# Electron-Labs/eth-lc-plonky2

Measured on AMD Instinct MI355X. Metric: lc_proofs_per_hour, higher is better.
Workload: dtype u64

## Files before the change

### eth-lc-plonky2_amd/binding.py

```python
import ctypes
import os

import numpy as np

from . import build as _build

u64p = ctypes.POINTER(ctypes.c_uint64)
u32p = ctypes.POINTER(ctypes.c_uint32)
u8p = ctypes.POINTER(ctypes.c_uint8)
MEM_HOST, MEM_DEVICE = 0, 1
VERIFY_HEADS = {"host": 0, "device": 1}
E_UNSAT = -5
SECTION_OPENINGS, SECTION_FRI_CAP0, SECTION_AFTER_CAPS = 0, 1, 2

K_INTT, K_LDE, K_LEAF_HASH, K_MERKLE, K_PERM_Z, K_QUOTIENT, K_OPENINGS, K_FRI, K_POW, K_SHA256, K_OTHER = range(11)
KERNEL_FAMILIES = ["intt", "lde", "leaf_hash", "merkle", "perm_z", "quotient", "openings", "fri", "pow", "sha256", "other"]

GOLDILOCKS_P = 0xFFFFFFFF00000001


class Lcp2Error(RuntimeError):
    def __init__(self, status, message):
        super().__init__(f"lcp2 status {status}: {message}")
        self.status = status


class Params(ctypes.Structure):
    _fields_ = [(n, ctypes.c_uint32) for n in (
        "degree_bits", "num_wires", "num_routed_wires", "num_constants", "rate_bits", "cap_height",
        "num_challenges", "quotient_degree_factor", "proof_of_work_bits", "num_query_rounds", "num_fri_layers")]
    _fields_.append(("fri_arity_bits", ctypes.c_uint32 * 8))


class CircuitDesc(ctypes.Structure):
    _fields_ = [("params", Params), ("constants_sigmas", ctypes.c_void_p), ("constants_sigmas_mem", ctypes.c_int),
                ("k_is", ctypes.c_void_p), ("num_selectors", ctypes.c_uint32), ("num_gates", ctypes.c_uint32),
                ("gates", ctypes.c_void_p), ("code", ctypes.c_void_p), ("code_words", ctypes.c_size_t),
                ("imm", ctypes.c_void_p), ("num_imm", ctypes.c_size_t), ("num_public_inputs", ctypes.c_uint32),
                ("num_regs", ctypes.c_uint32)]


class CircuitRows(ctypes.Structure):
    _fields_ = [("gate_of_row", ctypes.c_void_p), ("num_rows", ctypes.c_size_t), ("pad_gate", ctypes.c_uint32), ("row_constants", ctypes.c_void_p),
                ("bindings", ctypes.c_void_p), ("num_bindings", ctypes.c_size_t), ("bindings_mem", ctypes.c_int), ("num_classes", ctypes.c_uint32)]


BINDING_DTYPE = np.dtype([("row", "<u4"), ("col", "<u4"), ("cls", "<u4")])
assert BINDING_DTYPE.itemsize == 12


class ProofLayout(ctypes.Structure):
    _fields_ = ([(n, ctypes.c_uint64) for n in ("cap_words", "wires_cap", "zs_cap", "quot_cap", "op_constants", "op_sigmas", "op_wires", "op_zs",
                                                "op_zs_next", "op_partial_products", "op_quotient", "fri_caps", "queries", "query_words")]
                + [("q_init_off", ctypes.c_uint64 * 4), ("q_init_cols", ctypes.c_uint64 * 4), ("q_init_sib", ctypes.c_uint64),
                   ("q_step_off", ctypes.c_uint64 * 8), ("q_step_sib", ctypes.c_uint64 * 8)]
                + [(n, ctypes.c_uint64) for n in ("final_poly", "final_len", "pow_witness", "total")])


class U32Job(ctypes.Structure):
    _fields_ = [("row", ctypes.c_uint32), ("kind", ctypes.c_uint16), ("op", ctypes.c_uint16), ("inputs", ctypes.c_uint32 * 4)]


U32_ARITHMETIC, U32_ADD_MANY, U32_SUBTRACTION, U32_RANGE_CHECK, U32_COMPARISON = range(5)
U32_JOB_DTYPE = np.dtype([("row", "<u4"), ("kind", "<u2"), ("op", "<u2"), ("in", "<u4", (4,))])
assert U32_JOB_DTYPE.itemsize == ctypes.sizeof(U32Job) == 24
POSEIDON_ROW_DTYPE = np.dtype([("row", "<u4"), ("swap", "<u4"), ("in", "<u8", (12,))])
assert POSEIDON_ROW_DTYPE.itemsize == 104
SHA_JOB_DTYPE = np.dtype([("first_row", "<u4"), ("in_src", "<i4", (16,))])
CELL_DTYPE = np.dtype([("row", "<u4"), ("col", "<u4"), ("value", "<u8")])
CELL_REF_DTYPE = np.dtype([("row", "<u4"), ("col", "<u4")])
assert SHA_JOB_DTYPE.itemsize == 68 and CELL_DTYPE.itemsize == 16 and CELL_REF_DTYPE.itemsize == 8
SHA_ROWS, SHA_ROW_COLUMNS = 310, 108

class RecOperand(ctypes.Structure):
    _fields_ = [("v", ctypes.c_uint64), ("col", ctypes.c_uint32), ("src", ctypes.c_uint32)]


class RecJob(ctypes.Structure):
    _fields_ = [("row", ctypes.c_uint32), ("kind", ctypes.c_uint16), ("op", ctypes.c_uint16), ("first_operand", ctypes.c_uint32),
                ("reserved", ctypes.c_uint32)]


(REC_ARITHMETIC, REC_BASE_SUM, REC_ARITHMETIC_EXT, REC_MUL_EXT, REC_REDUCING, REC_REDUCING_EXT, REC_POSEIDON_MDS, REC_RANDOM_ACCESS,
 REC_EXPONENTIATION, REC_COSET_INTERPOLATION, REC_KINDS) = range(11)
REC_IMM, REC_CELL = 0, 1
REC_OPERAND_DTYPE = np.dtype([("v", "<u8"), ("col", "<u4"), ("src", "<u4")])
REC_JOB_DTYPE = np.dtype([("row", "<u4"), ("kind", "<u2"), ("op", "<u2"), ("first_operand", "<u4"), ("reserved", "<u4")])
assert REC_OPERAND_DTYPE.itemsize == ctypes.sizeof(RecOperand) == 16 and REC_JOB_DTYPE.itemsize == ctypes.sizeof(RecJob) == 16
PLAN_IMM, PLAN_CELL, PLAN_PREV = 0, 1, 2
POS_JOB_DTYPE = np.dtype([("row", "<u4"), ("first_operand", "<u4")])
assert POS_JOB_DTYPE.itemsize == 8


class WitnessPlan(ctypes.Structure):
    _fields_ = [("rec_jobs", ctypes.c_void_p), ("nrec", ctypes.c_size_t), ("rec_level_ends", ctypes.c_void_p),
                ("pos_jobs", ctypes.c_void_p), ("npos", ctypes.c_size_t), ("chain_ends", ctypes.c_void_p), ("nchains", ctypes.c_size_t),
                ("pos_level_ends", ctypes.c_void_p), ("operands", ctypes.c_void_p), ("noperands", ctypes.c_size_t), ("nlevels", ctypes.c_size_t)]


class U32PlanJob(ctypes.Structure):
    _fields_ = [("row", ctypes.c_uint32), ("kind", ctypes.c_uint16), ("op", ctypes.c_uint16), ("first_operand", ctypes.c_uint32),
                ("reserved", ctypes.c_uint32)]


U32_PLAN_JOB_DTYPE = REC_JOB_DTYPE
U32_PLAN_OPERANDS = {U32_ARITHMETIC: 3, U32_ADD_MANY: 4, U32_SUBTRACTION: 3, U32_RANGE_CHECK: 1, U32_COMPARISON: 2}
assert ctypes.sizeof(U32PlanJob) == U32_PLAN_JOB_DTYPE.itemsize == 16


class WitnessPlanU32(ctypes.Structure):
    _fields_ = [("base", WitnessPlan), ("u32_jobs", ctypes.c_void_p), ("nu32", ctypes.c_size_t), ("u32_level_ends", ctypes.c_void_p)]


_lib = None


class WitnessReport(ctypes.Structure):
    _fields_ = [("gate_violations", ctypes.c_uint64), ("gate_row", ctypes.c_uint64), ("gate_index", ctypes.c_uint32), ("gate_constraint", ctypes.c_uint32),
                ("copy_violations", ctypes.c_uint64), ("copy_row", ctypes.c_uint64), ("copy_wire", ctypes.c_uint32),
                ("copy_to_row", ctypes.c_uint64), ("copy_to_wire", ctypes.c_uint32), ("noncanonical_cells", ctypes.c_uint64)]
    per_gate = None

    @property
    def ok(self):
        return self.gate_violations == 0 and self.copy_violations == 0

    def __repr__(self):
        return "WitnessReport(%s)" % ", ".join("%s=%d" % (f, getattr(self, f)) for f, _ in self._fields_)


class FillReport(ctypes.Structure):
    _fields_ = [(f, ctypes.c_uint64) for f in ("num_classes", "classes_set", "cells_filled", "conflicts", "conflict_index", "owner_index")]
    unsat = False
    message = ""

    def __repr__(self):
        return "FillReport(%s, unsat=%s)" % (", ".join("%s=%d" % (f, getattr(self, f)) for f, _ in self._fields_), self.unsat)


class ChallengerState(ctypes.Structure):
    _fields_ = [("sponge", ctypes.c_uint64 * 12), ("input", ctypes.c_uint64 * 8), ("output", ctypes.c_uint64 * 8),
                ("input_len", ctypes.c_uint32), ("output_len", ctypes.c_uint32)]


def _share_torch_hip_runtime():
    import importlib.util
    spec = importlib.util.find_spec("torch")
    if spec is None or not spec.submodule_search_locations:
        return
    libdir = os.path.join(list(spec.submodule_search_locations)[0], "lib")
    for name in ("libhsa-runtime64.so", "libamdhip64.so"):
        cand = os.path.join(libdir, name)
        if os.path.exists(cand):
            try:
                ctypes.CDLL(cand, mode=ctypes.RTLD_GLOBAL)
            except OSError:
                return


def load_library():
    global _lib
    if _lib is not None:
        return _lib
    path = _build.LIB
    if not os.path.exists(path):
        path = _build.build_native()
    _share_torch_hip_runtime()
    lib = ctypes.CDLL(path)
    c = ctypes
    sigs = {
        "lcp2_status_str": (c.c_char_p, [c.c_int]),
        "lcp2_abi_version": (c.c_int, []),
        "lcp2_device_count": (c.c_int, []),
        "lcp2_params_standard": (c.c_int, [c.c_uint32, c.c_uint32, c.POINTER(Params)]),
        "lcp2_params_config": (c.c_int, [c.c_uint32] * 8 + [c.POINTER(Params)]),
        "lcp2_ctx_create": (c.c_int, [c.c_int, c.c_void_p, c.POINTER(c.c_void_p)]),
        "lcp2_ctx_create_ex": (c.c_int, [c.c_int, c.c_void_p, c.c_uint32, c.POINTER(c.c_void_p)]),
        "lcp2_ctx_destroy": (None, [c.c_void_p]),
        "lcp2_ctx_sync": (c.c_int, [c.c_void_p]),
        "lcp2_ctx_stream": (c.c_void_p, [c.c_void_p]),
        "lcp2_last_error": (c.c_char_p, [c.c_void_p]),
        "lcp2_poseidon_permute_batch": (c.c_int, [c.c_void_p, c.c_void_p, c.c_void_p, c.c_size_t, c.c_int]),
        "lcp2_field_op_batch": (c.c_int, [c.c_void_p, c.c_void_p, c.c_void_p, c.c_void_p, c.c_size_t, c.c_uint32, c.c_int]),
        "lcp2_merkle_cap": (c.c_int, [c.c_void_p, c.c_void_p, c.c_size_t, c.c_size_t, c.c_uint32, c.c_int, c.c_void_p]),
        "lcp2_ntt_batch": (c.c_int, [c.c_void_p, c.c_void_p, c.c_size_t, c.c_uint32, c.c_int, c.c_uint64, c.c_int]),
        "lcp2_lde_batch": (c.c_int, [c.c_void_p, c.c_void_p, c.c_void_p, c.c_size_t, c.c_uint32, c.c_uint32, c.c_int]),
        "lcp2_sha256_tree": (c.c_int, [c.c_void_p, c.c_void_p, c.c_uint32, c.c_size_t, c.c_void_p, c.c_void_p, c.c_int]),
        "lcp2_sha256_witness": (c.c_int, [c.c_void_p, c.c_void_p, c.c_size_t, c.c_void_p, c.c_uint32, c.c_void_p, c.c_size_t, c.c_void_p, c.c_uint64, c.c_void_p]),
        "lcp2_scatter_cells": (c.c_int, [c.c_void_p, c.c_void_p, c.c_size_t, c.c_void_p, c.c_uint64]),
        "lcp2_poseidon_gate_rows": (c.c_int, [c.c_void_p, c.c_void_p, c.c_size_t, c.c_void_p, c.c_uint64]),
        "lcp2_u32_gate_rows": (c.c_int, [c.c_void_p, c.c_void_p, c.c_size_t, c.c_int, c.c_void_p, c.c_uint64]),
        "lcp2_rec_gate_rows": (c.c_int, [c.c_void_p, c.c_void_p, c.c_size_t, c.c_void_p, c.c_size_t, c.c_void_p, c.c_size_t, c.c_int, c.c_void_p,
                                         c.c_uint32, c.c_uint64]),
        "lcp2_witness_plan_rows": (c.c_int, [c.c_void_p, c.POINTER(WitnessPlan), c.c_int, c.c_void_p, c.c_uint32, c.c_uint64]),
        "lcp2_witness_plan_rows_u32": (c.c_int, [c.c_void_p, c.POINTER(WitnessPlanU32), c.c_int, c.c_void_p, c.c_uint32, c.c_uint64]),
        "lcp2_commit_wires_rows_begin": (c.c_int, [c.c_void_p, c.c_void_p]),
        "lcp2_commit_wires_chunk": (c.c_int, [c.c_void_p, c.c_void_p, c.c_uint32, c.c_uint32]),
        "lcp2_commit_wires_rows_finish": (c.c_int, [c.c_void_p, c.c_void_p]),
        "lcp2_host_register": (c.c_int, [c.c_void_p, c.c_void_p, c.c_size_t]),
        "lcp2_host_unregister": (c.c_int, [c.c_void_p, c.c_void_p]),
        "lcp2_witness_stage": (c.c_int, [c.c_void_p, c.c_void_p, c.c_uint32]),
        "lcp2_prove_staged": (c.c_int, [c.c_void_p, c.c_uint32, c.c_void_p, c.c_size_t, c.c_void_p, c.c_size_t]),
        "lcp2_buffer_alloc": (c.c_int, [c.c_void_p, c.c_size_t, c.POINTER(c.c_void_p)]),
        "lcp2_buffer_free": (c.c_int, [c.c_void_p, c.c_void_p]),
        "lcp2_buffer_zero": (c.c_int, [c.c_void_p, c.c_void_p, c.c_size_t]),
        "lcp2_buffer_read": (c.c_int, [c.c_void_p, c.c_void_p, c.c_void_p, c.c_size_t]),
        "lcp2_buffer_write": (c.c_int, [c.c_void_p, c.c_void_p, c.c_void_p, c.c_size_t]),
        "lcp2_buffer_copy": (c.c_int, [c.c_void_p, c.c_void_p, c.c_void_p, c.c_size_t]),
        "lcp2_buffer_copy_2d": (c.c_int, [c.c_void_p, c.c_void_p, c.c_size_t, c.c_void_p, c.c_size_t, c.c_size_t, c.c_size_t]),
        "lcp2_commit_values": (c.c_int, [c.c_void_p, c.c_void_p, c.c_size_t, c.c_uint32, c.c_uint32, c.c_uint32, c.c_int, c.POINTER(c.c_void_p), c.c_void_p]),
        "lcp2_commit_coeffs": (c.c_int, [c.c_void_p, c.c_void_p, c.c_size_t, c.c_uint32, c.c_uint32, c.c_uint32, c.c_int, c.POINTER(c.c_void_p), c.c_void_p]),
        "lcp2_commit_cosets": (c.c_int, [c.c_void_p, c.c_void_p, c.c_size_t, c.c_uint32, c.c_uint32, c.c_uint32, c.c_uint32, c.c_uint32, c.c_int, c.POINTER(c.c_void_p), c.c_void_p]),
        "lcp2_oracle_destroy": (None, [c.c_void_p]),
        "lcp2_oracle_open": (c.c_int, [c.c_void_p, c.c_void_p, c.c_size_t, c.c_void_p, c.c_void_p]),
        "lcp2_oracle_read": (c.c_int, [c.c_void_p, c.c_void_p, c.c_void_p]),
        "lcp2_circuit_create": (c.c_int, [c.c_void_p, c.POINTER(CircuitDesc), c.POINTER(c.c_void_p)]),
        "lcp2_circuit_rows_expand": (c.c_int, [c.c_void_p, c.POINTER(CircuitDesc), c.POINTER(CircuitRows), c.c_void_p]),
        "lcp2_circuit_create_from_rows": (c.c_int, [c.c_void_p, c.POINTER(CircuitDesc), c.POINTER(CircuitRows), c.POINTER(c.c_void_p)]),
        "lcp2_verifier_create": (c.c_int, [c.POINTER(CircuitDesc), c.c_void_p, c.c_void_p, c.POINTER(c.c_void_p)]),
        "lcp2_circuit_destroy": (None, [c.c_void_p]),
        "lcp2_circuit_digest": (c.c_int, [c.c_void_p, c.c_void_p, c.c_void_p]),
        "lcp2_proof_words": (c.c_size_t, [c.POINTER(Params)]),
        "lcp2_proof_layout_of": (c.c_int, [c.POINTER(Params), c.POINTER(ProofLayout)]),
        "lcp2_prove": (c.c_int, [c.c_void_p, c.c_void_p, c.c_int, c.c_void_p, c.c_size_t, c.c_void_p, c.c_size_t]),
        "lcp2_witness_fill_copies": (c.c_int, [c.c_void_p, c.c_void_p, c.c_size_t, c.c_int, c.c_void_p, c.POINTER(FillReport)]),
        "lcp2_circuit_copy_classes": (c.c_int, [c.c_void_p, c.c_void_p, c.POINTER(c.c_uint64)]),
        "lcp2_witness_settle_copies": (c.c_int, [c.c_void_p, c.c_void_p, c.c_size_t, c.c_int, c.c_void_p, c.POINTER(FillReport)]),
        "lcp2_check_witness": (c.c_int, [c.c_void_p, c.c_void_p, c.c_int, c.c_void_p, c.c_size_t, c.POINTER(WitnessReport), c.c_void_p, c.c_uint32]),
        "lcp2_commit_wires": (c.c_int, [c.c_void_p, c.c_void_p, c.c_int, c.c_void_p]),
        "lcp2_commit_wires_coeffs": (c.c_int, [c.c_void_p, c.c_void_p, c.c_void_p, c.c_void_p]),
        "lcp2_commit_wires_rows": (c.c_int, [c.c_void_p, c.c_void_p, c.c_void_p, c.c_void_p]),
        "lcp2_perm_zs_rows_begin": (c.c_int, [c.c_void_p, c.c_void_p, c.c_void_p, c.c_void_p]),
        "lcp2_perm_zs_rows_finish": (c.c_int, [c.c_void_p, c.c_void_p, c.POINTER(c.c_void_p), c.POINTER(c.c_size_t)]),
        "lcp2_perm_zs_commit": (c.c_int, [c.c_void_p, c.c_void_p]),
        "lcp2_perm_zs": (c.c_int, [c.c_void_p, c.c_void_p, c.c_void_p, c.c_void_p]),
        "lcp2_quotient": (c.c_int, [c.c_void_p, c.c_void_p, c.c_void_p, c.c_void_p]),
        "lcp2_fri_open": (c.c_int, [c.c_void_p, c.c_void_p, c.POINTER(ChallengerState), c.c_void_p]),
        "lcp2_fri_open_begin": (c.c_int, [c.c_void_p, c.c_void_p, c.POINTER(ChallengerState), c.c_void_p]),
        "lcp2_fri_open_commit": (c.c_int, [c.c_void_p, c.c_void_p]),
        "lcp2_fri_open_finish": (c.c_int, [c.c_void_p, c.POINTER(ChallengerState), c.c_void_p]),
        "lcp2_proof_section": (c.c_int, [c.c_void_p, c.c_int, c.POINTER(c.c_size_t), c.POINTER(c.c_size_t)]),
        "lcp2_challenger_init": (None, [c.POINTER(ChallengerState)]),
        "lcp2_challenger_observe": (c.c_int, [c.POINTER(ChallengerState), c.c_void_p, c.c_size_t]),
        "lcp2_challenger_get": (c.c_int, [c.POINTER(ChallengerState), c.c_void_p, c.c_size_t]),
        "lcp2_hash_no_pad": (c.c_int, [c.c_void_p, c.c_size_t, c.c_void_p]),
        "lcp2_circuit_create_sharded": (c.c_int, [c.c_void_p, c.POINTER(CircuitDesc), c.c_uint32, c.c_uint32, c.POINTER(c.c_void_p)]),
        "lcp2_circuit_set_constants_cap": (c.c_int, [c.c_void_p, c.c_void_p]),
        "lcp2_quotient_values": (c.c_int, [c.c_void_p, c.c_void_p, c.c_void_p]),
        "lcp2_quotient_buffer": (c.c_int, [c.c_void_p, c.POINTER(c.c_void_p), c.POINTER(c.c_size_t)]),
        "lcp2_quotient_commit": (c.c_int, [c.c_void_p, c.c_void_p]),
        "lcp2_verify": (c.c_int, [c.c_void_p, c.c_void_p, c.c_size_t, c.c_void_p, c.c_size_t, c.POINTER(c.c_int)]),
        "lcp2_verify_batch": (c.c_int, [c.c_void_p, c.c_void_p, c.c_void_p, c.c_size_t, c.c_size_t, c.c_int, c.c_void_p, c.c_size_t, c.c_void_p]),
        "lcp2_verify_batch_ex": (c.c_int, [c.c_void_p, c.c_void_p, c.c_void_p, c.c_size_t, c.c_size_t, c.c_int, c.c_void_p, c.c_size_t, c.c_void_p,
                                           c.c_uint32]),
        "lcp2_last_challenges": (c.c_int, [c.c_void_p, c.c_void_p]),
        "lcp2_gate_program_degree": (c.c_int, [c.c_void_p, c.c_size_t, c.c_uint32, c.POINTER(c.c_uint32)]),
        "lcp2_circuit_gate_tiers": (c.c_int, [c.c_void_p, c.c_uint32, c.c_void_p, c.c_void_p]),
        "lcp2_proof_bytes": (c.c_size_t, [c.POINTER(Params), c.c_size_t, c.c_uint32]),
        "lcp2_proof_to_bytes": (c.c_int, [c.POINTER(Params), c.c_void_p, c.c_size_t, c.c_void_p, c.c_size_t, c.c_uint32, c.c_void_p, c.c_size_t]),
        "lcp2_proof_from_bytes": (c.c_int, [c.POINTER(Params), c.c_void_p, c.c_size_t, c.c_uint32, c.c_void_p, c.c_size_t, c.c_void_p, c.c_size_t]),
        "lcp2_verifier_data_to_bytes": (c.c_int, [c.c_void_p, c.c_void_p, c.c_size_t]),
        "lcp2_prof_enable": (c.c_int, [c.c_void_p, c.c_int]),
        "lcp2_prof_reset": (c.c_int, [c.c_void_p]),
        "lcp2_prof_get": (c.c_int, [c.c_void_p, c.c_int, c.POINTER(c.c_double), c.POINTER(c.c_uint64), c.POINTER(c.c_double)]),
    }
    for name, (res, args) in sigs.items():
        fn = getattr(lib, name)
        fn.restype = res
        fn.argtypes = args
    _lib = lib
    return lib


EXPORTED_SYMBOLS = None


def _np_u64(a):
    a = np.ascontiguousarray(a, dtype=np.uint64)
    return a


def _ptr(a):
    return a.ctypes.data_as(ctypes.c_void_p) if a is not None else None


def standard_params(degree_bits, num_constants=4):
    lib = load_library()
    p = Params()
    rc = lib.lcp2_params_standard(degree_bits, num_constants, ctypes.byref(p))
    if rc:
        raise Lcp2Error(rc, lib.lcp2_status_str(rc).decode())
    return p


def params_config(degree_bits, num_constants=4, rate_bits=3, cap_height=4, proof_of_work_bits=16, num_query_rounds=28,
                  arity_bits=4, final_poly_bits=5):
    lib = load_library()
    p = Params()
    rc = lib.lcp2_params_config(degree_bits, num_constants, rate_bits, cap_height, proof_of_work_bits, num_query_rounds,
                                arity_bits, final_poly_bits, ctypes.byref(p))
    if rc:
        raise Lcp2Error(rc, lib.lcp2_status_str(rc).decode())
    return p


class Oracle:

    def __init__(self, ctx, handle, ncols, log_n, rate_bits, cap_height, cap):
        self.ctx, self.handle = ctx, handle
        self.ncols, self.log_n, self.rate_bits, self.cap_height = ncols, log_n, rate_bits, cap_height
        self.cap = cap
        self.block_first, self.block_count = 0, 1 << rate_bits

    def open(self, indices):
        idx = _np_u64(indices)
        k = idx.size
        nsib = self.log_n + self.rate_bits - self.cap_height
        leaves = np.zeros((k, self.ncols), dtype=np.uint64)
        sib = np.zeros((k, max(nsib, 0), 4), dtype=np.uint64)
        self.ctx._check(self.ctx.lib.lcp2_oracle_open(self.handle, _ptr(idx), k, _ptr(leaves), _ptr(sib)))
        return leaves, sib

    def read(self, coeffs=True, lde=True):
        n = 1 << self.log_n
        c = np.zeros((self.ncols, n), dtype=np.uint64) if coeffs else None
        l = np.zeros((self.ncols, n * self.block_count), dtype=np.uint64) if lde else None
        self.ctx._check(self.ctx.lib.lcp2_oracle_read(self.handle, _ptr(c), _ptr(l)))
        return c, l

    def close(self):
        if self.handle:
            self.ctx.lib.lcp2_oracle_destroy(self.handle)
            self.handle = None

    def __del__(self):
        try:
            self.close()
        except Exception:
            pass


class Context:

    def __init__(self, device=0, stream=None, order_with_default_stream=False):
        self.lib = load_library()
        h = ctypes.c_void_p()
        rc = self.lib.lcp2_ctx_create_ex(device, stream, 1 if order_with_default_stream else 0, ctypes.byref(h))
        if rc:
            raise Lcp2Error(rc, self.lib.lcp2_status_str(rc).decode())
        self.handle = h

    def _check(self, rc):
        if rc:
            msg = self.lib.lcp2_status_str(rc).decode()
            detail = self.lib.lcp2_last_error(self.handle)
            raise Lcp2Error(rc, msg + (": " + detail.decode() if detail else ""))

    def close(self):
        if getattr(self, "handle", None):
            self.lib.lcp2_ctx_destroy(self.handle)
            self.handle = None

    def __del__(self):
        try:
            self.close()
        except Exception:
            pass

    def sync(self):
        self._check(self.lib.lcp2_ctx_sync(self.handle))

    def stream_ptr(self):
        return self.lib.lcp2_ctx_stream(self.handle) or 0

    def poseidon_permute_batch(self, states):
        s = _np_u64(states).reshape(-1, 12)
        out = np.empty_like(s)
        self._check(self.lib.lcp2_poseidon_permute_batch(self.handle, _ptr(s), _ptr(out), s.shape[0], MEM_HOST))
        return out

    FIELD_OPS = {"mul": 0, "pow7": 1, "add": 2, "sub": 3, "canon": 4, "add_lazy": 5, "sub_lazy": 6, "shl32_lazy": 24, "mul_u32": 25,
                 **{"shl%d" % (12 * k): 16 + k for k in range(1, 8)}}

    def field_op_batch(self, op, a, b=None):
        a = _np_u64(a).reshape(-1)
        out = np.empty_like(a)
        if b is not None:
            b = _np_u64(b).reshape(-1)
            assert a.shape == b.shape
        self._check(self.lib.lcp2_field_op_batch(self.handle, _ptr(a), _ptr(b) if b is not None else None, _ptr(out), a.shape[0],
                                                 self.FIELD_OPS[op], MEM_HOST))
        return out

    def merkle_cap(self, leaves, cap_height):
        l = _np_u64(leaves)
        assert l.ndim == 2
        cap = np.zeros((1 << cap_height, 4), dtype=np.uint64)
        self._check(self.lib.lcp2_merkle_cap(self.handle, _ptr(l), l.shape[0], l.shape[1], cap_height, MEM_HOST, _ptr(cap)))
        return cap

    def ntt_batch(self, cols, inverse=False, shift=1):
        c = _np_u64(cols).copy()
        assert c.ndim == 2
        log_n = int(c.shape[1]).bit_length() - 1
        assert 1 << log_n == c.shape[1]
        self._check(self.lib.lcp2_ntt_batch(self.handle, _ptr(c), c.shape[0], log_n, int(inverse), shift, MEM_HOST))
        return c

    def lde_batch(self, coeffs, rate_bits=3):
        c = _np_u64(coeffs)
        log_n = int(c.shape[1]).bit_length() - 1
        out = np.zeros((c.shape[0], c.shape[1] << rate_bits), dtype=np.uint64)
        self._check(self.lib.lcp2_lde_batch(self.handle, _ptr(c), _ptr(out), c.shape[0], log_n, rate_bits, MEM_HOST))
        return out

    def sha256_tree(self, leaves, height, trees=1, trace=False):
        l = np.ascontiguousarray(leaves, dtype=np.uint8).reshape(trees, 1 << height, 32)
        nodes = np.zeros((trees, (2 << height) - 1, 32), dtype=np.uint8)
        tr = np.zeros((trees, (1 << height) - 1, 2, 176), dtype=np.uint32) if trace else None
        self._check(self.lib.lcp2_sha256_tree(self.handle, _ptr(l), height, trees, _ptr(nodes), _ptr(tr), MEM_HOST))
        return (nodes, tr) if trace else nodes

    def _commit(self, fn, cols, rate_bits, cap_height, mem, shape):
        if mem == MEM_HOST:
            c = _np_u64(cols)
            ncols, n = c.shape
            p = _ptr(c)
        else:
            ncols, n = shape
            p = ctypes.c_void_p(cols)
        log_n = int(n).bit_length() - 1
        cap = np.zeros((1 << cap_height, 4), dtype=np.uint64)
        h = ctypes.c_void_p()
        self._check(fn(self.handle, p, ncols, log_n, rate_bits, cap_height, mem, ctypes.byref(h), _ptr(cap)))
        return Oracle(self, h, ncols, log_n, rate_bits, cap_height, cap)

    def commit_values(self, cols, rate_bits=3, cap_height=4, mem=MEM_HOST, shape=None):
        return self._commit(self.lib.lcp2_commit_values, cols, rate_bits, cap_height, mem, shape)

    def commit_coeffs(self, cols, rate_bits=3, cap_height=4, mem=MEM_HOST, shape=None):
        return self._commit(self.lib.lcp2_commit_coeffs, cols, rate_bits, cap_height, mem, shape)

    def commit_cosets(self, coeffs, block_first, block_count, rate_bits=3, cap_height=4, mem=MEM_HOST, shape=None):
        if mem == MEM_HOST:
            c = _np_u64(coeffs)
            ncols, n = c.shape
            p = _ptr(c)
        else:
            ncols, n = shape
            p = ctypes.c_void_p(coeffs)
        log_n = int(n).bit_length() - 1
        cap = np.zeros((block_count << (cap_height - rate_bits), 4), dtype=np.uint64)
        h = ctypes.c_void_p()
        self._check(self.lib.lcp2_commit_cosets(self.handle, p, ncols, log_n, rate_bits, cap_height, block_first, block_count, mem,
                                                ctypes.byref(h), _ptr(cap)))
        o = Oracle(self, h, ncols, log_n, rate_bits, cap_height, cap)
        o.block_first, o.block_count = block_first, block_count
        return o

    def buffer_zero(self, dev_ptr, words):
        self._check(self.lib.lcp2_buffer_zero(self.handle, ctypes.c_void_p(dev_ptr), int(words) * 8))

    def sha256_witness(self, jobs, level_start, words_in, wires_dev, n, digests=True):
        if not isinstance(jobs, np.ndarray) or jobs.dtype != SHA_JOB_DTYPE:
            raise Lcp2Error(-1, "jobs must be an array of SHA_JOB_DTYPE records")
        j = np.ascontiguousarray(jobs).ravel()
        levels = np.ascontiguousarray(level_start, dtype=np.uint32).ravel()
        words = np.ascontiguousarray(words_in, dtype=np.uint32).ravel()
        out = np.zeros((j.size, 8), dtype=np.uint32) if digests else None
        self._check(self.lib.lcp2_sha256_witness(self.handle, _ptr(j) if j.size else None, j.size, _ptr(levels) if levels.size else None,
                                                 max(levels.size, 1) - 1, _ptr(words) if words.size else None, words.size,
                                                 ctypes.c_void_p(wires_dev), int(n), _ptr(out) if digests and j.size else None))
        return out

    def scatter_cells(self, cells, wires_dev, n):
        if not isinstance(cells, np.ndarray) or cells.dtype != CELL_DTYPE:
            raise Lcp2Error(-1, "cells must be an array of CELL_DTYPE records")
        c = np.ascontiguousarray(cells).ravel()
        self._check(self.lib.lcp2_scatter_cells(self.handle, _ptr(c) if c.size else None, c.size, ctypes.c_void_p(wires_dev), int(n)))

    def poseidon_gate_rows(self, rows, wires_dev, n):
        if not isinstance(rows, np.ndarray) or rows.dtype != POSEIDON_ROW_DTYPE:
            raise Lcp2Error(-1, "rows must be an array of POSEIDON_ROW_DTYPE records")
        r = np.ascontiguousarray(rows).ravel()
        self._check(self.lib.lcp2_poseidon_gate_rows(self.handle, _ptr(r), r.size, ctypes.c_void_p(wires_dev), n))

    def u32_gate_rows(self, jobs, wires_dev, n, njobs=None):
        if isinstance(jobs, np.ndarray):
            if jobs.dtype != U32_JOB_DTYPE:
                raise Lcp2Error(-1, "jobs must be an array of U32_JOB_DTYPE records")
            j = np.ascontiguousarray(jobs).ravel()
            count, p, mem = j.size, _ptr(j), MEM_HOST
        else:
            if njobs is None:
                raise Lcp2Error(-1, "a device job list needs njobs")
            count, p, mem = int(njobs), ctypes.c_void_p(jobs), MEM_DEVICE
        self._check(self.lib.lcp2_u32_gate_rows(self.handle, p, count, mem, ctypes.c_void_p(wires_dev), n))

    def rec_gate_rows(self, jobs, operands, level_ends, wires_dev, ncols, n, njobs=None, noperands=None):
        ends = np.ascontiguousarray(level_ends, dtype=np.uint32).ravel()
        if isinstance(jobs, np.ndarray) != isinstance(operands, np.ndarray):
            raise Lcp2Error(-1, "jobs and operands must both be host arrays or both be device pointers")
        if isinstance(jobs, np.ndarray):
            if jobs.dtype != REC_JOB_DTYPE or operands.dtype != REC_OPERAND_DTYPE:
                raise Lcp2Error(-1, "jobs / operands must be arrays of REC_JOB_DTYPE / REC_OPERAND_DTYPE records")
            j, o = np.ascontiguousarray(jobs).ravel(), np.ascontiguousarray(operands).ravel()
            nj, no, pj, po, mem = j.size, o.size, _ptr(j), _ptr(o), MEM_HOST
        else:
            if njobs is None or noperands is None:
                raise Lcp2Error(-1, "device lists need njobs and noperands")
            nj, no, pj, po, mem = int(njobs), int(noperands), ctypes.c_void_p(jobs), ctypes.c_void_p(operands), MEM_DEVICE
        self._check(self.lib.lcp2_rec_gate_rows(self.handle, pj, nj, po, no, _ptr(ends) if ends.size else None, ends.size, mem,
                                                ctypes.c_void_p(wires_dev), int(ncols), int(n)))

    def witness_plan_rows(self, rec_jobs, pos_jobs, chain_ends, operands, rec_level_ends, pos_level_ends, wires_dev, ncols, n,
                          nrec=None, npos=None, nchains=None, noperands=None):
        rends = np.ascontiguousarray(rec_level_ends, dtype=np.uint32).ravel()
        pends = np.ascontiguousarray(pos_level_ends, dtype=np.uint32).ravel()
        if rends.size != pends.size:
            raise Lcp2Error(-1, "rec_level_ends and pos_level_ends must have one entry per level each")
        lists = (rec_jobs, pos_jobs, chain_ends, operands)
        on_host = [isinstance(a, np.ndarray) for a in lists]
        if any(on_host) != all(on_host):
            raise Lcp2Error(-1, "the four lists must all be host arrays or all be device pointers")
        if all(on_host):
            if (rec_jobs.dtype, pos_jobs.dtype, chain_ends.dtype, operands.dtype) != (REC_JOB_DTYPE, POS_JOB_DTYPE, np.dtype(np.uint32), REC_OPERAND_DTYPE):
                raise Lcp2Error(-1, "the lists must be arrays of REC_JOB_DTYPE / POS_JOB_DTYPE / uint32 / REC_OPERAND_DTYPE records")
            keep = [np.ascontiguousarray(a).ravel() for a in lists]
            counts, ptrs, mem = [a.size for a in keep], [a.ctypes.data if a.size else None for a in keep], MEM_HOST
        else:
            if None in (nrec, npos, nchains, noperands):
                raise Lcp2Error(-1, "device lists need nrec, npos, nchains and noperands")
            counts, ptrs, mem = [int(nrec), int(npos), int(nchains), int(noperands)], [a or None for a in lists], MEM_DEVICE
        plan = WitnessPlan(ptrs[0], counts[0], rends.ctypes.data if rends.size else None, ptrs[1], counts[1], ptrs[2], counts[2],
                           pends.ctypes.data if pends.size else None, ptrs[3], counts[3], rends.size)
        self._check(self.lib.lcp2_witness_plan_rows(self.handle, ctypes.byref(plan), mem, ctypes.c_void_p(wires_dev), int(ncols), int(n)))

    def witness_plan_rows_u32(self, u32_jobs, rec_jobs, pos_jobs, chain_ends, operands, u32_level_ends, rec_level_ends, pos_level_ends,
                              wires_dev, ncols, n, nu32=None, nrec=None, npos=None, nchains=None, noperands=None):
        ends = [np.ascontiguousarray(e, dtype=np.uint32).ravel() for e in (u32_level_ends, rec_level_ends, pos_level_ends)]
        if len({e.size for e in ends}) != 1:
            raise Lcp2Error(-1, "u32_level_ends, rec_level_ends and pos_level_ends must have one entry per level each")
        lists = (u32_jobs, rec_jobs, pos_jobs, chain_ends, operands)
        on_host = [isinstance(a, np.ndarray) for a in lists]
        if any(on_host) != all(on_host):
            raise Lcp2Error(-1, "the five lists must all be host arrays or all be device pointers")
        if all(on_host):
            if [a.dtype for a in lists] != [U32_PLAN_JOB_DTYPE, REC_JOB_DTYPE, POS_JOB_DTYPE, np.dtype(np.uint32), REC_OPERAND_DTYPE]:
                raise Lcp2Error(-1, "the lists must be arrays of U32_PLAN_JOB_DTYPE / REC_JOB_DTYPE / POS_JOB_DTYPE / uint32 / REC_OPERAND_DTYPE records")
            keep = [np.ascontiguousarray(a).ravel() for a in lists]
            counts, ptrs, mem = [a.size for a in keep], [a.ctypes.data if a.size else None for a in keep], MEM_HOST
        else:
            if None in (nu32, nrec, npos, nchains, noperands):
                raise Lcp2Error(-1, "device lists need nu32, nrec, npos, nchains and noperands")
            counts, ptrs, mem = [int(nu32), int(nrec), int(npos), int(nchains), int(noperands)], [a or None for a in lists], MEM_DEVICE
        end_ptrs = [e.ctypes.data if e.size else None for e in ends]
        base = WitnessPlan(ptrs[1], counts[1], end_ptrs[1], ptrs[2], counts[2], ptrs[3], counts[3], end_ptrs[2], ptrs[4], counts[4], ends[0].size)
        plan = WitnessPlanU32(base, ptrs[0], counts[0], end_ptrs[0])
        self._check(self.lib.lcp2_witness_plan_rows_u32(self.handle, ctypes.byref(plan), mem, ctypes.c_void_p(wires_dev), int(ncols), int(n)))

    def verify_batch(self, circuit_data, proofs, public_inputs, mem=MEM_HOST, count=None, head="host"):
        if head not in VERIFY_HEADS:
            raise Lcp2Error(-1, "head is 'host' or 'device'")
        words = circuit_data.proof_words
        if mem == MEM_HOST:
            pr = _np_u64(proofs)
            if pr.size % words:
                raise Lcp2Error(-1, "proofs is not a whole number of this circuit's proofs")
            count, ptr = pr.size // words, _ptr(pr)
        else:
            if count is None:
                raise Lcp2Error(-1, "device proofs need count")
            ptr = ctypes.c_void_p(proofs)
        if count == 0:
            return np.zeros(0, dtype=np.int32)
        pis = _np_u64(public_inputs).ravel()
        npi = pis.size // count
        if npi * count != pis.size:
            raise Lcp2Error(-1, "public_inputs is not count rows")
        checks = np.zeros(count, dtype=np.int32)
        if head == "host":
            rc = self.lib.lcp2_verify_batch(self.handle, circuit_data.handle, ptr, words, count, mem, _ptr(pis), npi, _ptr(checks))
        else:
            rc = self.lib.lcp2_verify_batch_ex(self.handle, circuit_data.handle, ptr, words, count, mem, _ptr(pis), npi, _ptr(checks), VERIFY_HEADS[head])
        if rc != -7:
            self._check(rc)
        return checks

    def expand_rows(self, circ, rows, bindings_ptr=None, num_bindings=None):
        d, keep = _describe(circ, 0)
        r, keep_rows = _describe_rows(rows, bindings_ptr, num_bindings)
        shape = (circ.params.num_constants + circ.params.num_routed_wires, 1 << circ.params.degree_bits)
        ptr = self.buffer_alloc(shape[0] * shape[1])
        try:
            self._check(self.lib.lcp2_circuit_rows_expand(self.handle, ctypes.byref(d), ctypes.byref(r), ctypes.c_void_p(ptr)))
            return self.buffer_read(ptr, shape[0] * shape[1]).reshape(shape)
        finally:
            self.buffer_free(ptr)

    def buffer_alloc(self, words):
        p = ctypes.c_void_p()
        self._check(self.lib.lcp2_buffer_alloc(self.handle, int(words) * 8, ctypes.byref(p)))
        return p.value

    def buffer_free(self, dev_ptr):
        self._check(self.lib.lcp2_buffer_free(self.handle, ctypes.c_void_p(dev_ptr)))

    def buffer_read(self, dev_ptr, words):
        out = np.zeros(words, dtype=np.uint64)
        self._check(self.lib.lcp2_buffer_read(self.handle, _ptr(out), ctypes.c_void_p(dev_ptr), words * 8))
        return out

    def buffer_write(self, dev_ptr, arr):
        a = _np_u64(arr)
        self._check(self.lib.lcp2_buffer_write(self.handle, ctypes.c_void_p(dev_ptr), _ptr(a), a.size * 8))

    def buffer_copy(self, dst_ptr, src_ptr, words):
        self._check(self.lib.lcp2_buffer_copy(self.handle, ctypes.c_void_p(dst_ptr), ctypes.c_void_p(src_ptr), words * 8))

    def buffer_copy_2d(self, dst_ptr, dst_pitch_words, src_ptr, src_pitch_words, width_words, height):
        self._check(self.lib.lcp2_buffer_copy_2d(self.handle, ctypes.c_void_p(dst_ptr), dst_pitch_words * 8, ctypes.c_void_p(src_ptr),
                                                 src_pitch_words * 8, width_words * 8, height))

    def prof_enable(self, on=True):
        self._check(self.lib.lcp2_prof_enable(self.handle, int(on)))

    def prof_reset(self):
        self._check(self.lib.lcp2_prof_reset(self.handle))

    def prof_get(self):
        out = {}
        for i, name in enumerate(KERNEL_FAMILIES):
            ms, n, b = ctypes.c_double(), ctypes.c_uint64(), ctypes.c_double()
            self._check(self.lib.lcp2_prof_get(self.handle, i, ctypes.byref(ms), ctypes.byref(n), ctypes.byref(b)))
            out[name] = {"ms": ms.value, "launches": n.value, "bytes": b.value}
        return out


class Challenger:

    def __init__(self):
        self.lib = load_library()
        self.state = ChallengerState()
        self.lib.lcp2_challenger_init(ctypes.byref(self.state))

    def observe(self, values):
        v = np.ascontiguousarray(np.asarray(values, dtype=np.uint64).ravel())
        rc = self.lib.lcp2_challenger_observe(ctypes.byref(self.state), _ptr(v), v.size)
        if rc:
            raise Lcp2Error(rc, self.lib.lcp2_status_str(rc).decode())

    def get(self, count=1):
        out = np.zeros(count, dtype=np.uint64)
        rc = self.lib.lcp2_challenger_get(ctypes.byref(self.state), _ptr(out), count)
        if rc:
            raise Lcp2Error(rc, self.lib.lcp2_status_str(rc).decode())
        return out


def hash_no_pad(values):
    lib = load_library()
    v = np.ascontiguousarray(np.asarray(values, dtype=np.uint64).ravel())
    out = np.zeros(4, dtype=np.uint64)
    rc = lib.lcp2_hash_no_pad(_ptr(v) if v.size else None, v.size, _ptr(out))
    if rc:
        raise Lcp2Error(rc, lib.lcp2_status_str(rc).decode())
    return out


SER_PUBLIC_INPUT_COUNT = 1


def proof_layout(params):
    lib, out = load_library(), ProofLayout()
    rc = lib.lcp2_proof_layout_of(ctypes.byref(params), ctypes.byref(out))
    if rc:
        raise Lcp2Error(rc, lib.lcp2_status_str(rc).decode())
    return out


def proof_to_bytes(params, proof, public_inputs, flags=SER_PUBLIC_INPUT_COUNT):
    lib = load_library()
    pr, pis = _np_u64(proof).ravel(), _np_u64(public_inputs).ravel()
    out = np.zeros(lib.lcp2_proof_bytes(ctypes.byref(params), pis.size, flags), dtype=np.uint8)
    rc = lib.lcp2_proof_to_bytes(ctypes.byref(params), _ptr(pr), pr.size, _ptr(pis), pis.size, flags, _ptr(out), out.size)
    if rc:
        raise Lcp2Error(rc, lib.lcp2_status_str(rc).decode())
    return out.tobytes()


def proof_from_bytes(params, data, num_public_inputs, flags=SER_PUBLIC_INPUT_COUNT):
    lib = load_library()
    buf = np.frombuffer(bytes(data), dtype=np.uint8)
    proof = np.zeros(lib.lcp2_proof_words(ctypes.byref(params)), dtype=np.uint64)
    pis = np.zeros(num_public_inputs, dtype=np.uint64)
    rc = lib.lcp2_proof_from_bytes(ctypes.byref(params), _ptr(buf) if buf.size else None, buf.size, flags, _ptr(proof), proof.size, _ptr(pis), pis.size)
    if rc:
        raise Lcp2Error(rc, lib.lcp2_status_str(rc).decode())
    return proof, pis


class ProofRejected(Lcp2Error):

    def __init__(self, check):
        super().__init__(-7, f"proof rejected (check {check})")
        self.check = check


def _describe(circ, constants_sigmas_ptr=None, mem=MEM_HOST):
    gs = circ.gateset
    gates = circ.gates_array
    d = CircuitDesc()
    d.params = circ.params
    d.constants_sigmas = constants_sigmas_ptr if constants_sigmas_ptr is not None else circ.constants_sigmas.ctypes.data
    d.constants_sigmas_mem = mem
    d.k_is = circ.k_is.ctypes.data
    d.num_selectors, d.num_gates = gs.num_selectors, len(gs.gates)
    d.gates = ctypes.cast(gates, ctypes.c_void_p)
    d.code, d.code_words = gs.code.ctypes.data, gs.code_len
    d.imm, d.num_imm = gs.imm.ctypes.data, gs.imm.size
    d.num_public_inputs, d.num_regs = circ.num_public_inputs, gs.max_regs
    return d, (gates, gs, circ)


def _describe_rows(rows, bindings_ptr=None, num_bindings=None):
    gate_of_row = np.ascontiguousarray(rows.gate_of_row, dtype=np.uint32).ravel()
    consts = None if rows.row_constants is None else np.ascontiguousarray(rows.row_constants, dtype=np.uint64)
    r = CircuitRows()
    r.gate_of_row, r.num_rows, r.pad_gate = (gate_of_row.ctypes.data if gate_of_row.size else None), gate_of_row.size, rows.pad_gate
    r.row_constants = consts.ctypes.data if consts is not None and consts.size else None
    r.num_classes = rows.num_classes
    if bindings_ptr is not None:
        r.bindings, r.num_bindings, r.bindings_mem, b = bindings_ptr, int(num_bindings), MEM_DEVICE, None
    else:
        if not isinstance(rows.bindings, np.ndarray) or rows.bindings.dtype != BINDING_DTYPE:
            raise Lcp2Error(-1, "bindings must be an array of BINDING_DTYPE records")
        b = np.ascontiguousarray(rows.bindings).ravel()
        r.bindings, r.num_bindings, r.bindings_mem = (b.ctypes.data if b.size else None), b.size, MEM_HOST
    return r, (gate_of_row, consts, b)


class CircuitData:

    def __init__(self, ctx, circ, handle, keep):
        self.ctx, self.circ, self.handle, self._keep = ctx, circ, handle, keep
        self.lib = load_library()
        self.proof_words = self.lib.lcp2_proof_words(ctypes.byref(circ.params))

    @classmethod
    def build(cls, ctx, circ, constants_sigmas_ptr=None, mem=MEM_HOST):
        d, keep = _describe(circ, constants_sigmas_ptr, mem)
        h = ctypes.c_void_p()
        ctx._check(ctx.lib.lcp2_circuit_create(ctx.handle, ctypes.byref(d), ctypes.byref(h)))
        return cls(ctx, circ, h, keep)

    @classmethod
    def build_from_rows(cls, ctx, circ, rows, bindings_ptr=None, num_bindings=None):
        d, keep = _describe(circ, 0)
        r, keep_rows = _describe_rows(rows, bindings_ptr, num_bindings)
        h = ctypes.c_void_p()
        ctx._check(ctx.lib.lcp2_circuit_create_from_rows(ctx.handle, ctypes.byref(d), ctypes.byref(r), ctypes.byref(h)))
        return cls(ctx, circ, h, keep)

    @classmethod
    def build_sharded(cls, ctx, circ, block_first, block_count, constants_sigmas_ptr=None, mem=MEM_HOST):
        d, keep = _describe(circ, constants_sigmas_ptr, mem)
        h = ctypes.c_void_p()
        ctx._check(ctx.lib.lcp2_circuit_create_sharded(ctx.handle, ctypes.byref(d), block_first, block_count, ctypes.byref(h)))
        return cls(ctx, circ, h, keep)

    def set_constants_cap(self, cap):
        cp = _np_u64(cap)
        self._check(self.lib.lcp2_circuit_set_constants_cap(self.handle, _ptr(cp)))

    def quotient_values(self, alphas, public_inputs_hash):
        a, h = _np_u64(alphas), _np_u64(public_inputs_hash)
        assert h.size == 4
        self._check(self.lib.lcp2_quotient_values(self.handle, _ptr(a), _ptr(h)))

    def quotient_buffer(self):
        ptr, words = ctypes.c_void_p(), ctypes.c_size_t()
        self._check(self.lib.lcp2_quotient_buffer(self.handle, ctypes.byref(ptr), ctypes.byref(words)))
        return ptr.value, words.value

    def quotient_commit(self):
        cap = self._cap()
        self._check(self.lib.lcp2_quotient_commit(self.handle, _ptr(cap)))
        return cap

    @classmethod
    def verifier_only(cls, circ, digest, cap):
        lib = load_library()
        d, keep = _describe(circ, 0)
        h = ctypes.c_void_p()
        dg, cp = _np_u64(digest), _np_u64(cap)
        rc = lib.lcp2_verifier_create(ctypes.byref(d), _ptr(dg), _ptr(cp), ctypes.byref(h))
        if rc:
            raise Lcp2Error(rc, lib.lcp2_status_str(rc).decode())
        return cls(None, circ, h, keep)

    def _check(self, rc):
        if rc:
            if self.ctx is not None:
                self.ctx._check(rc)
            raise Lcp2Error(rc, self.lib.lcp2_status_str(rc).decode())

    def digest(self):
        d = np.zeros(4, dtype=np.uint64)
        cap = np.zeros((1 << self.circ.params.cap_height, 4), dtype=np.uint64)
        self._check(self.lib.lcp2_circuit_digest(self.handle, _ptr(d), _ptr(cap)))
        return d, cap

    def prove(self, wires, public_inputs, mem=MEM_HOST):
        pis = _np_u64(public_inputs).ravel()
        proof = np.zeros(self.proof_words, dtype=np.uint64)
        if mem == MEM_HOST:
            w = _np_u64(wires)
            if w.shape != (self.circ.params.num_wires, 1 << self.circ.params.degree_bits):
                raise Lcp2Error(-1, "witness must be [num_wires][n]")
            wp = _ptr(w)
        else:
            wp = ctypes.c_void_p(wires)
        self._check(self.lib.lcp2_prove(self.handle, wp, mem, _ptr(pis), pis.size, _ptr(proof), proof.size))
        return proof

    def check_witness(self, wires, public_inputs, per_gate=False, mem=MEM_HOST):
        pis = _np_u64(public_inputs).ravel()
        if mem == MEM_HOST:
            w = _np_u64(wires)
            if w.shape != (self.circ.params.num_wires, 1 << self.circ.params.degree_bits):
                raise Lcp2Error(-1, "witness must be [num_wires][n]")
            wp = _ptr(w)
        else:
            wp = ctypes.c_void_p(wires)
        report = WitnessReport()
        ng = len(self.circ.gateset.gates)
        counts = np.zeros(ng, dtype=np.uint64) if per_gate else None
        self._check(self.lib.lcp2_check_witness(self.handle, wp, mem, _ptr(pis), pis.size, ctypes.byref(report), _ptr(counts), ng))
        report.per_gate = counts
        return report

    def fill_copies(self, cells, wires_ptr, mem=MEM_HOST, ncells=None):
        return self._copies_call(self.lib.lcp2_witness_fill_copies, cells, CELL_DTYPE, "cells must be an array of CELL_DTYPE records", wires_ptr, mem, ncells)

    def settle_copies(self, sources, wires_ptr, mem=MEM_HOST, nsources=None):
        return self._copies_call(self.lib.lcp2_witness_settle_copies, sources, CELL_REF_DTYPE, "sources must be an array of CELL_REF_DTYPE records", wires_ptr, mem,
                                 nsources)

    def _copies_call(self, call, records, dtype, dtype_message, wires_ptr, mem, count):
        if mem == MEM_HOST:
            if not isinstance(records, np.ndarray) or records.dtype != dtype:
                raise Lcp2Error(-1, dtype_message)
            c = np.ascontiguousarray(records).ravel()
            p, count = (_ptr(c) if c.size else None), c.size
        else:
            p, count = ctypes.c_void_p(records), int(count)
        report = FillReport()
        rc = call(self.handle, p, count, mem, ctypes.c_void_p(wires_ptr), ctypes.byref(report))
        if rc == E_UNSAT:
            report.unsat = True
            report.message = self.lib.lcp2_last_error(self.ctx.handle).decode()
        else:
            self._check(rc)
        return report

    def copy_classes(self):
        NR, n = self.circ.params.num_routed_wires, 1 << self.circ.params.degree_bits
        class_of, count = np.zeros((NR, n), dtype=np.uint32), ctypes.c_uint64()
        self._check(self.lib.lcp2_circuit_copy_classes(self.handle, _ptr(class_of), ctypes.byref(count)))
        return class_of, count.value

    def stage_witness(self, wires, slot):
        w = _np_u64(wires)
        if w.shape != (self.circ.params.num_wires, 1 << self.circ.params.degree_bits):
            raise Lcp2Error(-1, "witness must be [num_wires][n]")
        if not hasattr(self, "_staged"):
            self._staged = {}
        self._staged[slot] = w
        self._check(self.lib.lcp2_witness_stage(self.handle, _ptr(w), slot))

    def prove_staged(self, slot, public_inputs):
        pis = _np_u64(public_inputs).ravel()
        proof = np.zeros(self.proof_words, dtype=np.uint64)
        self._check(self.lib.lcp2_prove_staged(self.handle, slot, _ptr(pis), pis.size, _ptr(proof), proof.size))
        self._staged.pop(slot, None)
        return proof

    def host_witness_benchmark(self, wires, public_inputs, steps=4, reference_proof=None):
        import time
        ctx = self.ctx
        bufs = [np.ascontiguousarray(wires, dtype=np.uint64), np.array(wires, dtype=np.uint64, order="C")]
        for b in bufs:
            ctx._check(ctx.lib.lcp2_host_register(ctx.handle, _ptr(b), b.nbytes))
        try:
            ctx.sync()
            t0 = time.perf_counter()
            plain = self.prove(bufs[0], public_inputs, mem=MEM_HOST)
            t_plain = time.perf_counter() - t0
            self.stage_witness(bufs[0], 0)
            times = []
            for i in range(steps):
                t0 = time.perf_counter()
                if i + 1 < steps:
                    self.stage_witness(bufs[(i + 1) % 2], (i + 1) % 2)
                proof = self.prove_staged(i % 2, public_inputs)
                times.append(time.perf_counter() - t0)
            ok = bool((proof == plain).all()) and (reference_proof is None or bool((proof == reference_proof).all()))
        finally:
            ctx.sync()
            for b in bufs:
                ctx.lib.lcp2_host_unregister(ctx.handle, _ptr(b))
        steady = times[1:-1] if len(times) > 2 else times
        return {"workload": "lcp2_prove from HOST witnesses (%.2f GB each, pinned with lcp2_host_register): upload of witness i + 1 on the copy stream while "
                            "proof i runs (lcp2_witness_stage / lcp2_prove_staged)" % (bufs[0].nbytes / 1e9),
                "ms_per_proof_steady_state": 1e3 * min(steady), "ms_per_proof_all": [round(1e3 * t, 2) for t in times],
                "ms_plain_host_prove": 1e3 * t_plain, "proofs_equal_device_resident_proof": ok}

    def _cap(self):
        return np.zeros((1 << self.circ.params.cap_height, 4), dtype=np.uint64)

    def commit_wires(self, wires, mem=MEM_HOST):
        cap = self._cap()
        if mem == MEM_HOST:
            self._staged_wires = _np_u64(wires)
            wp = _ptr(self._staged_wires)
        else:
            wp = ctypes.c_void_p(wires)
        self._check(self.lib.lcp2_commit_wires(self.handle, wp, mem, _ptr(cap)))
        return cap

    def commit_wires_coeffs(self, wires_ptr, coeffs_ptr):
        cap = self._cap()
        self._check(self.lib.lcp2_commit_wires_coeffs(self.handle, ctypes.c_void_p(wires_ptr), ctypes.c_void_p(coeffs_ptr), _ptr(cap)))
        return cap

    def commit_wires_rows(self, rows_ptr, coeffs_ptr):
        cap = self._cap()
        self._check(self.lib.lcp2_commit_wires_rows(self.handle, ctypes.c_void_p(rows_ptr), ctypes.c_void_p(coeffs_ptr), _ptr(cap)))
        return cap

    def commit_wires_rows_begin(self, rows_ptr):
        self._check(self.lib.lcp2_commit_wires_rows_begin(self.handle, ctypes.c_void_p(rows_ptr)))

    def commit_wires_chunk(self, coeffs_ptr, first_col, ncols):
        self._check(self.lib.lcp2_commit_wires_chunk(self.handle, ctypes.c_void_p(coeffs_ptr), first_col, ncols))

    def commit_wires_rows_finish(self):
        cap = self._cap()
        self._check(self.lib.lcp2_commit_wires_rows_finish(self.handle, _ptr(cap)))
        return cap

    def perm_zs_rows_begin(self, betas, gammas, world):
        out, b, g = np.zeros(world * self.circ.params.num_challenges, dtype=np.uint64), _np_u64(betas), _np_u64(gammas)
        self._check(self.lib.lcp2_perm_zs_rows_begin(self.handle, _ptr(b), _ptr(g), _ptr(out)))
        return out

    def perm_zs_rows_finish(self, block_products):
        bp = _np_u64(block_products)
        ptr, words = ctypes.c_void_p(), ctypes.c_size_t()
        self._check(self.lib.lcp2_perm_zs_rows_finish(self.handle, _ptr(bp), ctypes.byref(ptr), ctypes.byref(words)))
        return ptr.value, words.value

    def perm_zs_commit(self):
        cap = self._cap()
        self._check(self.lib.lcp2_perm_zs_commit(self.handle, _ptr(cap)))
        return cap

    def perm_zs(self, betas, gammas):
        cap, b, g = self._cap(), _np_u64(betas), _np_u64(gammas)
        self._check(self.lib.lcp2_perm_zs(self.handle, _ptr(b), _ptr(g), _ptr(cap)))
        return cap

    def quotient(self, alphas, public_inputs_hash):
        cap, a, h = self._cap(), _np_u64(alphas), _np_u64(public_inputs_hash)
        assert h.size == 4
        self._check(self.lib.lcp2_quotient(self.handle, _ptr(a), _ptr(h), _ptr(cap)))
        return cap

    def fri_open(self, zeta, challenger_state, proof):
        z = _np_u64(zeta)
        assert proof.dtype == np.uint64 and proof.size == self.proof_words and proof.flags.c_contiguous
        self._check(self.lib.lcp2_fri_open(self.handle, _ptr(z), ctypes.byref(challenger_state), _ptr(proof)))

    def fri_open_begin(self, zeta, challenger_state, proof):
        z = _np_u64(zeta)
        assert proof.dtype == np.uint64 and proof.size == self.proof_words and proof.flags.c_contiguous
        self._check(self.lib.lcp2_fri_open_begin(self.handle, _ptr(z), ctypes.byref(challenger_state), _ptr(proof)))

    def fri_open_commit(self, proof):
        assert proof.dtype == np.uint64 and proof.size == self.proof_words and proof.flags.c_contiguous
        self._check(self.lib.lcp2_fri_open_commit(self.handle, _ptr(proof)))

    def fri_open_finish(self, proof, challenger_state=None):
        assert proof.dtype == np.uint64 and proof.size == self.proof_words and proof.flags.c_contiguous
        self._check(self.lib.lcp2_fri_open_finish(self.handle, ctypes.byref(challenger_state) if challenger_state is not None else None, _ptr(proof)))

    def proof_section(self, section):
        first, count = ctypes.c_size_t(0), ctypes.c_size_t(0)
        self._check(self.lib.lcp2_proof_section(self.handle, section, ctypes.byref(first), ctypes.byref(count)))
        return first.value, count.value

    def verify(self, proof, public_inputs):
        failed = ctypes.c_int(0)
        pr, pis = _np_u64(proof).ravel(), _np_u64(public_inputs).ravel()
        rc = self.lib.lcp2_verify(self.handle, _ptr(pr), pr.size, _ptr(pis), pis.size, ctypes.byref(failed))
        if rc == -7:
            raise ProofRejected(failed.value)
        self._check(rc)

    def verifier_data_bytes(self):
        out = np.zeros(((4 << self.circ.params.cap_height) + 4) * 8, dtype=np.uint8)
        self._check(self.lib.lcp2_verifier_data_to_bytes(self.handle, _ptr(out), out.size))
        return out.tobytes()

    def last_challenges(self):
        out = np.zeros(97, dtype=np.uint64)
        self._check(self.lib.lcp2_last_challenges(self.handle, _ptr(out)))
        return {"betas": out[0:4], "gammas": out[4:8], "alphas": out[8:12], "zeta": out[12:14], "fri_alpha": out[14:16],
                "fri_betas": out[16:32].reshape(8, 2), "pow_witness": int(out[32]), "query_indices": out[33:97]}

    def gate_tiers(self):
        ng = len(self.circ.gateset.gates)
        deg, bun = np.zeros(ng, dtype=np.uint32), np.zeros(ng, dtype=np.int32)
        self._check(self.lib.lcp2_circuit_gate_tiers(self.handle, ng, _ptr(deg), _ptr(bun)))
        return deg, bun

    def close(self):
        if self.handle:
            self.lib.lcp2_circuit_destroy(self.handle)
            self.handle = None

    def __del__(self):
        try:
            self.close()
        except Exception:
            pass
```

### eth-lc-plonky2_amd/csrc/kernels_gates.hpp

```cpp
#pragma once
#include <utility>
#include "quotient_common.hpp"

namespace lcp2 {

enum GeneratedMode : u32 { GEN_QUOTIENT = 0, GEN_ROW_CHECK = 1, GEN_CLAIM_CHECK = 2 };

#if defined(__HIP_DEVICE_COMPILE__)
template <u32 K> struct QGenerated {
  static __device__ __forceinline__ void run(const QuotientArgs &a, const GateDev &, u64 i, u64 *, u32, u32, QEmit &emit) { q_generated<K>(a, i, emit); }
};
#else
template <u32 K> struct QGenerated;
#endif

template <u32 K, bool CHECK>
__global__ __launch_bounds__(QUOTIENT_THREADS, Q_GENERATED_WAVES[K]) void k_q_gen(QuotientArgs a, u32 g, u32 accumulate, unsigned long long *flag) {
#if defined(__HIP_DEVICE_COMPILE__)
  extern __shared__ __attribute__((aligned(16))) u64 lds[];
  const u32 T = QUOTIENT_THREADS, tid = threadIdx.x;
  u64 i;
  const bool live = q_point<CHECK>(a, i);
  q_stage_limbs(a, lds, T, tid);
  if (!live) return;
  const GateDev G = q_load_gate(a, g);
  if (!q_wave_holds<CHECK>(a, G, i)) return;
  u64 val[QUOTIENT_MAX_CH];
  q_gate_value<QGenerated<K>>(a, g, G, i, lds, T, tid, val);
  q_gate_store<CHECK>(a, i, val, accumulate, flag);
#endif
}

template <class EVAL>
__global__ __launch_bounds__(QUOTIENT_THREADS, 2) void k_claim_check(QuotientArgs a, u32 g, unsigned long long *flag) {
  extern __shared__ __attribute__((aligned(16))) u64 lds[];
  const u32 T = QUOTIENT_THREADS, tid = threadIdx.x;
  const u64 i = (u64)blockIdx.x * T + tid;
  q_stage_limbs(a, lds, T, tid);
  if (i >= a.count) return;
  q_claim_check<EVAL>(a, g, i, lds, T, tid, flag);
}
template <class EVAL>
void launch_claim_check(hipStream_t s, const QuotientArgs &a, u32 g, unsigned long long *flag) {
  QuotientArgs ag = a;
  ag.limbs_lds_word = (a.num_regs + QUOTIENT_STAGE) * QUOTIENT_THREADS;
  hipLaunchKernelGGL((k_claim_check<EVAL>), q_grid(a), dim3(QUOTIENT_THREADS), q_interp_lds_bytes(a) + Q_LIMB_WORDS32 * 4, s, ag, g, flag);
}

template <u32 K>
void launch_generated_one(hipStream_t s, const QuotientArgs &a, u32 g, u32 accumulate, unsigned long long *flag, u32 mode) {
  if (mode == GEN_CLAIM_CHECK) { launch_claim_check<QGenerated<K>>(s, a, g, flag); return; }
  const dim3 block(QUOTIENT_THREADS);
  const size_t limbs = Q_LIMB_WORDS32 * 4;
  QuotientArgs ag = a;
  ag.limbs_lds_word = 0;
  if (mode == GEN_ROW_CHECK) hipLaunchKernelGGL((k_q_gen<K, true>), q_grid(a), block, limbs, s, ag, g, accumulate, flag);
  else hipLaunchKernelGGL((k_q_gen<K, false>), q_grid(a), block, limbs, s, ag, g, accumulate, flag);
}

template <u32 FIRST, size_t... I>
bool launch_generated_unit(std::index_sequence<I...>, hipStream_t s, const QuotientArgs &a, u32 k, u32 g, u32 accumulate, unsigned long long *flag, u32 mode) {
  bool hit = false;
  ((k == FIRST + I ? (launch_generated_one<FIRST + (u32)I>(s, a, g, accumulate, flag, mode), hit = true) : false), ...);
  return hit;
}

#define LCP2_DEFINE_GENERATED_UNIT(name, FIRST, COUNT)                                                                                          \
  bool launch_generated_##name(hipStream_t s, const QuotientArgs &a, u32 k, u32 g, u32 accumulate, unsigned long long *flag, u32 mode) {       \
    return launch_generated_unit<FIRST>(std::make_index_sequence<COUNT>{}, s, a, k, g, accumulate, flag, mode);                                 \
  }

bool launch_generated_sha(hipStream_t s, const QuotientArgs &a, u32 k, u32 g, u32 accumulate, unsigned long long *flag, u32 mode);
bool launch_generated_u32a(hipStream_t s, const QuotientArgs &a, u32 k, u32 g, u32 accumulate, unsigned long long *flag, u32 mode);
bool launch_generated_u32b(hipStream_t s, const QuotientArgs &a, u32 k, u32 g, u32 accumulate, unsigned long long *flag, u32 mode);
bool launch_generated_reca(hipStream_t s, const QuotientArgs &a, u32 k, u32 g, u32 accumulate, unsigned long long *flag, u32 mode);
bool launch_generated_recb(hipStream_t s, const QuotientArgs &a, u32 k, u32 g, u32 accumulate, unsigned long long *flag, u32 mode);

}
```

### eth-lc-plonky2_amd/csrc/kernels_quotient.hip

```cpp
#include <algorithm>
#include "gate_program.hpp"
#include "kernels_gates.hpp"
#include "light_gates.hpp"

namespace lcp2 {

void stage_gate_programs(const std::vector<uint32_t> &code, std::vector<GateDev> &gates, u32 num_wires, u32 num_selectors,
                         std::vector<uint32_t> &out, std::vector<uint32_t> &lists) {
  stage_programs(code, gates, num_wires, num_selectors, out, lists);
}

#if defined(__HIP_DEVICE_COMPILE__)
__device__ __forceinline__ void q_poseidon_native(const QuotientArgs &a, u64 i, u64 *lds, u32 T, u32 tid, QEmit &emit) {
  const_as<u64> rc = konst(a.rc);
  QEmit &E = emit;
  E.begin_terms();
  auto emit_term = [&](u64 x) { E.term(a, E.emitted++, x); };
  const u64 *W = a.wires + i;
  const u64 st = a.stride;
  u64 in[12], dl[4], swap;
#pragma unroll
  for (int j = 0; j < 12; j++) in[j] = W[(u64)j * st];
  swap = W[24 * st];
#pragma unroll
  for (int j = 0; j < 4; j++) dl[j] = W[(u64)(25 + j) * st];
  emit_term(gl_mul_nc(swap, gl_sub(swap, 1)));
#pragma unroll
  for (int j = 0; j < 4; j++) emit_term(gl_sub_nc(gl_mul_nc(swap, gl_sub(in[j + 4], in[j])), dl[j]));
  u32 lo[12], hi[12];
#pragma unroll
  for (int j = 0; j < 12; j++) {
    u64 v = j < 4 ? gl_add(in[j], dl[j]) : j < 8 ? gl_sub(in[j], dl[j - 4]) : in[j];
    v = gl_add_nc(v, rc[j]);
    lo[j] = (u32)v; hi[j] = (u32)(v >> 32);
  }
  auto constrain12 = [&](u32 first_wire) {
    u64 w[12];
#pragma unroll
    for (int j = 0; j < 12; j++) w[j] = W[(u64)(first_wire + j) * st];
#pragma unroll
    for (int j = 0; j < 12; j++) {
      emit_term(gl_sub_nc(((u64)hi[j] << 32) | lo[j], w[j]));
      lo[j] = (u32)w[j]; hi[j] = (u32)(w[j] >> 32);
    }
  };
  u32 round = 0;
#pragma unroll 1
  for (u32 r = 0; r < POS_FULL_HALF; r++, round++) {
    if (r) constrain12(29 + 12 * (r - 1));
#pragma unroll
    for (int j = 0; j < 12; j++) pos_sbox_h(lo[j], hi[j]);
    u64 nxt[12];
#pragma unroll
    for (int j = 0; j < 12; j++) nxt[j] = rc[(round + 1) * 12 + j];
    pos_mds_h(lo, hi, nxt);
  }
  static_assert(QUOTIENT_STAGE % POS_GROUP == 0, "a group of partial rounds must not straddle two staging batches");
  auto stage_sbox_wires = [&](u32 r) {
    u64 pw[QUOTIENT_STAGE];
#pragma unroll
    for (u32 j = 0; j < QUOTIENT_STAGE; j++) pw[j] = W[(u64)(65 + min(r + j, (u32)POS_PARTIAL - 1)) * st];
#pragma unroll
    for (u32 j = 0; j < QUOTIENT_STAGE; j++) lds[j * T + tid] = pw[j];
  };
  auto constrain0 = [&](u32 r, u32 &ul, u32 &uh) {
    const u64 w = lds[(r % QUOTIENT_STAGE) * T + tid];
    emit_term(gl_sub_nc(((u64)uh << 32) | ul, w));
    ul = (u32)w; uh = (u32)(w >> 32);
  };
  u32 r = 0;
#pragma unroll 1
  for (u32 g = 0; g < POS_GROUPS; g++, r += POS_GROUP, round += POS_GROUP) {
    if (r % QUOTIENT_STAGE == 0) stage_sbox_wires(r);
    constrain0(r, lo[0], hi[0]);
    pos_partial3_core(lo, hi, &rc[POS_ROUNDS * POS_W + POS_GROUP_CONSTS * g], [&](int i, u32 &ul, u32 &uh) {
      constrain0(r + i, ul, uh);
      pos_sbox_h(ul, uh);
    });
  }
#pragma unroll 1
  for (; r < POS_PARTIAL; r++, round++) {
    if (r % QUOTIENT_STAGE == 0) stage_sbox_wires(r);
    constrain0(r, lo[0], hi[0]);
    pos_sbox_h(lo[0], hi[0]);
    u64 nxt[12];
#pragma unroll
    for (int j = 0; j < 12; j++) nxt[j] = rc[(round + 1) * 12 + j];
    pos_mds_h(lo, hi, nxt);
  }
#pragma unroll 1
  for (u32 r = 0; r < POS_FULL_HALF; r++, round++) {
    constrain12(87 + 12 * r);
#pragma unroll
    for (int j = 0; j < 12; j++) pos_sbox_h(lo[j], hi[j]);
    u64 nxt[12];
#pragma unroll
    for (int j = 0; j < 12; j++) nxt[j] = round + 1 < POS_ROUNDS ? rc[(round + 1) * 12 + j] : 0;
    pos_mds_h(lo, hi, nxt);
  }
  u64 out[12];
#pragma unroll
  for (int j = 0; j < 12; j++) out[j] = W[(u64)(12 + j) * st];
#pragma unroll
  for (int j = 0; j < 12; j++) emit_term(gl_sub_nc(((u64)hi[j] << 32) | lo[j], out[j]));
  E.finish_terms();
}
#endif

#if defined(__HIP_DEVICE_COMPILE__)
struct QPoseidon {
  static __device__ __forceinline__ void run(const QuotientArgs &a, const GateDev &, u64 i, u64 *lds, u32 T, u32 tid, QEmit &emit) { q_poseidon_native(a, i, lds, T, tid, emit); }
};
struct QArithmetic {
  static __device__ __forceinline__ void run(const QuotientArgs &a, const GateDev &G, u64 i, u64 *, u32, u32, QEmit &emit) { q_arith_base_walk<true, false>(a, i, G.num_constraints, 0, emit, emit); }
};
struct QBaseSum2 {
  static __device__ __forceinline__ void run(const QuotientArgs &a, const GateDev &G, u64 i, u64 *, u32, u32, QEmit &emit) { q_arith_base_walk<false, true>(a, i, 0, G.num_constraints - 1, emit, emit); }
};
__device__ __forceinline__ void q_pair_values(const QuotientArgs &a, u32 gA, u32 gB, const GateDev &GA, const GateDev &GB, u64 i, u64 valA[QUOTIENT_MAX_CH], u64 valB[QUOTIENT_MAX_CH]) {
  QEmit eA, eB;
  q_emit_begin(a, GA, eA); q_emit_begin(a, GB, eB);
  q_arith_base_walk<true, true>(a, i, GA.num_constraints, GB.num_constraints - 1, eA, eB);
  q_gate_finish(a, gA, GA, i, eA, valA); q_gate_finish(a, gB, GB, i, eB, valB);
}
#else
struct QPoseidon; struct QArithmetic; struct QBaseSum2;
#endif
struct QArithBasePair;
template <>
__device__ __forceinline__ void q_claim_check<QArithBasePair>(const QuotientArgs &a, u32 g, u64 i, u64 *lds, u32 T, u32 tid, unsigned long long *flag) {
#if defined(__HIP_DEVICE_COMPILE__)
  const u32 gA = g & 0xFFFFu, gB = g >> 16;
  const GateDev GA = q_load_gate(a, gA), GB = q_load_gate(a, gB);
  u64 pA[QUOTIENT_MAX_CH], pB[QUOTIENT_MAX_CH], vA[QUOTIENT_MAX_CH], vB[QUOTIENT_MAX_CH];
  q_gate_value<QInterpreted>(a, gA, GA, i, lds, T, tid, pA); q_gate_value<QInterpreted>(a, gB, GB, i, lds, T, tid, pB);
  q_pair_values(a, gA, gB, GA, GB, i, vA, vB);
  q_claim_compare(a, i, pA, vA, flag); q_claim_compare(a, i, pB, vB, flag);
#endif
}

template <u32 NATIVE, bool CHECK>
__global__ __launch_bounds__(QUOTIENT_THREADS, 2) void k_q_gate(QuotientArgs a, u32 g, u32 accumulate, unsigned long long *flag) {
  static_assert(NATIVE == LCP2_GATE_NATIVE_POSEIDON, "k_q_gate is the PoseidonGate kernel");
#if defined(__HIP_DEVICE_COMPILE__)
  extern __shared__ __attribute__((aligned(16))) u64 lds[];
  u64 i;
  if (!q_point<CHECK>(a, i)) return;
  const GateDev G = q_load_gate(a, g);
  if (!q_wave_holds<CHECK>(a, G, i)) return;
  u64 val[QUOTIENT_MAX_CH];
  q_gate_value<QPoseidon>(a, g, G, i, lds, QUOTIENT_THREADS, threadIdx.x, val);
  q_gate_store<CHECK>(a, i, val, accumulate, flag);
#endif
}

__device__ __forceinline__ u64 q_mul7_nc(u64 x) {
#if defined(__HIP_DEVICE_COMPILE__)
  const u64 p0 = (u64)(u32)x * 7u, p1 = (u64)(u32)(x >> 32) * 7u + (p0 >> 32);
  u64 lo = (p1 << 32) | (u32)p0;
  const u32 hi = (u32)(p1 >> 32);
  u32 c;
  asm("v_mad_u64_u32 %0, vcc, %2, -1, %0\n\t"
      "s_nop 1\n\t"
      "v_cndmask_b32_e64 %1, 0, 1, vcc\n\t"
      "v_mad_u64_u32 %0, vcc, %1, -1, %0"
      : "+v"(lo), "=&v"(c) : "v"(hi) : "vcc");
  return lo;
#else
  return gl_mul_u32_nc(x, 7u);
#endif
}

__global__ __launch_bounds__(QUOTIENT_THREADS, 2) void k_q_perm(QuotientArgs a, u32 have_gates) {
  const u32 T = QUOTIENT_THREADS, tid = threadIdx.x;
  const u64 i = (u64)blockIdx.x * T + tid;
  if (i >= a.count) return;
  const u64 ig = a.leaf0 + i;
  const u32 CH = a.num_challenges;
  u64 res[QUOTIENT_MAX_CH];
#pragma unroll
  for (u32 c = 0; c < QUOTIENT_MAX_CH; c++) res[c] = (c < CH && have_gates) ? a.out[(u64)c * a.N + ig] : 0;

  const u32 lgN = a.lgN;
  const u64 jnat = bitrev32((u32)ig, lgN);
  const u64 x = two_level(a.points, jnat);
  const u64 inext = bitrev32((u32)((jnat + (1u << a.rate_bits)) & (a.N - 1)), lgN) - a.leaf0;
  const u32 npp = a.nchunks - 1;
  u64 beta[QUOTIENT_MAX_CH], gamma[QUOTIENT_MAX_CH], bx[QUOTIENT_MAX_CH], prev[QUOTIENT_MAX_CH], z0[QUOTIENT_MAX_CH];
  u64 bxk[QUOTIENT_MAX_CH];
  u64 hh[QUOTIENT_MAX_CH][QUOTIENT_MAX_CH];
  u64 ainv[QUOTIENT_MAX_CH];
#pragma unroll
  for (u32 c = 0; c < QUOTIENT_MAX_CH; c++) {
    beta[c] = c < CH ? konst(a.betas)[c] : 0; gamma[c] = c < CH ? konst(a.gammas)[c] : 0;
    ainv[c] = c < CH ? konst(a.alpha_inv)[c] : 0;
    bx[c] = gl_mul(beta[c], x);
    bxk[c] = bx[c];
    z0[c] = c < CH ? a.zs[(u64)c * a.stride + i] : 0;
    prev[c] = z0[c];
#pragma unroll
    for (u32 d = 0; d < QUOTIENT_MAX_CH; d++) hh[c][d] = 0;
  }
  for (u32 k = 0; k < a.nchunks; k++) {
    u64 pn[QUOTIENT_MAX_CH], pd[QUOTIENT_MAX_CH], nx[QUOTIENT_MAX_CH];
#pragma unroll
    for (u32 c = 0; c < QUOTIENT_MAX_CH; c++) {
      pn[c] = 1; pd[c] = 1;
      nx[c] = c < CH ? (k < npp ? a.zs[((u64)CH + (u64)c * npp + k) * a.stride + i] : a.zs[(u64)c * a.stride + inext]) : 0;
    }
    const u32 jend = min((k + 1) * a.chunk, a.num_routed);
    for (u32 j0 = k * a.chunk; j0 < jend; j0 += 8) {
      u64 w[8], sg[8];
#pragma unroll
      for (u32 jj = 0; jj < 8; jj++) {
        const u32 j = min(j0 + jj, jend - 1);
        w[jj] = a.wires[(u64)j * a.stride + i];
        sg[jj] = a.consts[(u64)(a.num_constants + j) * a.stride + i];
      }
#pragma unroll
      for (u32 jj = 0; jj < 8; jj++) {
        if (j0 + jj < jend) {
          const u64 kj = konst(a.k_is)[j0 + jj];
#pragma unroll
          for (u32 c = 0; c < QUOTIENT_MAX_CH; c++)
            if (c < CH) {
              const u64 wg = gl_add(w[jj], gamma[c]);
              const u64 bk = a.kis_pow7 ? bxk[c] : gl_mul_nc(bx[c], kj);
              if (a.kis_pow7) bxk[c] = q_mul7_nc(bxk[c]);
              pn[c] = gl_mul_nc(pn[c], gl_add_nc(bk, wg));
              pd[c] = gl_mul_nc(pd[c], gl_add_nc(gl_mul_nc(beta[c], sg[jj]), wg));
            }
        }
      }
    }
#pragma unroll
    for (u32 c2 = 0; c2 < QUOTIENT_MAX_CH; c2++)
      if (c2 < CH) {
        const u64 term = gl_sub(gl_mul(prev[c2], pn[c2]), gl_mul(nx[c2], pd[c2]));
        prev[c2] = nx[c2];
#pragma unroll
        for (u32 c = 0; c < QUOTIENT_MAX_CH; c++)
          if (c < CH) hh[c2][c] = gl_add(gl_mul(hh[c2][c], ainv[c]), term);
      }
  }
  const u64 l0 = a.l0[ig];
#pragma unroll
  for (u32 c = 0; c < QUOTIENT_MAX_CH; c++)
    if (c < CH) {
      const_as<u64> pw = konst(a.alpha_pow) + c * QUOTIENT_ALPHA_POWS;
      u64 l0t[QUOTIENT_MAX_CH];
#pragma unroll
      for (u32 c2 = 0; c2 < QUOTIENT_MAX_CH; c2++) l0t[c2] = c2 < CH ? gl_mul(l0, gl_sub(z0[c2], 1)) : 0;
      if (ainv[c] == 0) { res[c] = l0t[0]; continue; }
      u64 r = gl_mul(res[c], pw[CH + CH * a.nchunks]);
#pragma unroll
      for (u32 c2 = 0; c2 < QUOTIENT_MAX_CH; c2++)
        if (c2 < CH) {
          r = gl_add(r, gl_mul(hh[c2][c], pw[CH + c2 * a.nchunks + a.nchunks - 1]));
          r = gl_add(r, gl_mul(l0t[c2], pw[c2]));
        }
      res[c] = r;
    }
  const u64 zhi = a.zh_inv[ig >> (lgN - a.rate_bits)];
#pragma unroll
  for (u32 c = 0; c < QUOTIENT_MAX_CH; c++)
    if (c < CH) a.out[(u64)c * a.N + ig] = gl_mul(res[c], zhi);
}

constexpr u32 LIGHT_NO_PAIR = ~0u;
struct LightGates { u32 count; u32 g[8]; u32 pair_a, pair_b; };
template <bool CHECK>
__global__ __launch_bounds__(QUOTIENT_THREADS, 2) void k_q_light(QuotientArgs a, LightGates L, u32 accumulate, unsigned long long *flag) {
#if defined(__HIP_DEVICE_COMPILE__)
  extern __shared__ __attribute__((aligned(16))) u64 lds[];
  const u32 T = QUOTIENT_THREADS, tid = threadIdx.x;
  u64 i;
  if (!q_point<CHECK>(a, i)) return;
  u64 sum[QUOTIENT_MAX_CH];
#pragma unroll
  for (u32 c = 0; c < QUOTIENT_MAX_CH; c++) sum[c] = 0;
  const u32 ka = L.pair_a, kb = L.pair_b;
  const bool pair = ka != LIGHT_NO_PAIR;
  if (pair) {
    const GateDev GA = q_load_gate(a, L.g[ka]), GB = q_load_gate(a, L.g[kb]);
    if (q_wave_holds<CHECK>(a, GA, i) || q_wave_holds<CHECK>(a, GB, i)) {
      u64 va[QUOTIENT_MAX_CH], vb[QUOTIENT_MAX_CH];
      q_pair_values(a, L.g[ka], L.g[kb], GA, GB, i, va, vb);
#pragma unroll
      for (u32 c = 0; c < QUOTIENT_MAX_CH; c++)
        if (c < a.num_challenges) sum[c] = gl_add(va[c], vb[c]);
    }
  }
  for (u32 k = 0; k < L.count; k++) {
    if (pair && (k == ka || k == kb)) continue;
    const u32 g = L.g[k];
    const GateDev G = q_load_gate(a, g);
    if (!q_wave_holds<CHECK>(a, G, i)) continue;
    u64 val[QUOTIENT_MAX_CH];
    switch (G.flags & LCP2_GATE_NATIVE_MASK) {
      case LCP2_GATE_NATIVE_ARITHMETIC: q_gate_value<QArithmetic>(a, g, G, i, lds, T, tid, val); break;
      case LCP2_GATE_NATIVE_BASE_SUM2: q_gate_value<QBaseSum2>(a, g, G, i, lds, T, tid, val); break;
      default: q_gate_value<QInterpreted>(a, g, G, i, lds, T, tid, val); break;
    }
#pragma unroll
    for (u32 c = 0; c < QUOTIENT_MAX_CH; c++)
      if (c < a.num_challenges) sum[c] = gl_add(sum[c], val[c]);
  }
  q_gate_store<CHECK>(a, i, sum, accumulate, flag);
#endif
}

static bool launch_generated(hipStream_t s, const QuotientArgs &a, u32 k, u32 g, u32 accumulate, unsigned long long *flag, u32 mode) {
  return launch_generated_sha(s, a, k, g, accumulate, flag, mode) || launch_generated_u32a(s, a, k, g, accumulate, flag, mode) ||
         launch_generated_u32b(s, a, k, g, accumulate, flag, mode) || launch_generated_reca(s, a, k, g, accumulate, flag, mode) ||
         launch_generated_recb(s, a, k, g, accumulate, flag, mode);
}
namespace {
template <bool CHECK>
void launch_gate(hipStream_t s, const QuotientArgs &a, const GateDev &G, u32 g, u32 accumulate, unsigned long long *flag) {
  const u32 kind = G.flags & LCP2_GATE_NATIVE_MASK;
  if (kind & 0x8000u) {
    launch_generated(s, a, (kind >> 8) & 0x7Fu, g, accumulate, flag, CHECK ? GEN_ROW_CHECK : GEN_QUOTIENT);
    return;
  }
  const size_t stage = (size_t)QUOTIENT_STAGE * QUOTIENT_THREADS * sizeof(u64);
  hipLaunchKernelGGL((k_q_gate<LCP2_GATE_NATIVE_POSEIDON, CHECK>), q_grid(a), dim3(QUOTIENT_THREADS), stage, s, a, g, accumulate, flag);
}
bool is_light(const GateDev &G) {
  const u32 k = G.flags & LCP2_GATE_NATIVE_MASK;
  return k == 0 || k == LCP2_GATE_NATIVE_ARITHMETIC || k == LCP2_GATE_NATIVE_BASE_SUM2;
}
bool pairable(u32 g) { return g < (1u << 16); }
template <bool CHECK>
u32 launch_gates(hipStream_t s, const QuotientArgs &a, const std::vector<GateDev> &host_gates, unsigned long long *flag, const int *tier = nullptr, int want = -1) {
  u32 launched = 0;
  const LightGates none{0, {}, LIGHT_NO_PAIR, LIGHT_NO_PAIR};
  LightGates L = none;
  auto flush = [&] {
    if (!L.count) return;
    if (L.pair_a == LIGHT_NO_PAIR || L.pair_b == LIGHT_NO_PAIR) L.pair_a = L.pair_b = LIGHT_NO_PAIR;
    hipLaunchKernelGGL((k_q_light<CHECK>), q_grid(a), dim3(QUOTIENT_THREADS), q_interp_lds_bytes(a), s, a, L, launched ? 1u : 0u, flag);
    launched++;
    L = none;
  };
  for (u32 g = 0; g < host_gates.size(); g++) {
    if (host_gates[g].num_constraints == 0 || (tier && tier[g] != want)) continue;
    if (is_light(host_gates[g])) {
      const u32 kind = host_gates[g].flags & LCP2_GATE_NATIVE_MASK;
      if (kind == LCP2_GATE_NATIVE_ARITHMETIC && L.pair_a == LIGHT_NO_PAIR && pairable(g)) L.pair_a = L.count;
      if (kind == LCP2_GATE_NATIVE_BASE_SUM2 && L.pair_b == LIGHT_NO_PAIR && pairable(g)) L.pair_b = L.count;
      L.g[L.count++] = g;
      if (L.count == 8) flush();
      continue;
    }
    launch_gate<CHECK>(s, a, host_gates[g], g, launched ? 1u : 0u, flag);
    launched++;
  }
  flush();
  return launched;
}
}

void launch_quotient(hipStream_t s, const QuotientArgs &a, const std::vector<GateDev> &host_gates) {
  const u32 launched = launch_gates<false>(s, a, host_gates, nullptr);
  launch_quotient_perm(s, a, launched ? 1u : 0u);
}
void launch_quotient_perm(hipStream_t s, const QuotientArgs &a, u32 have_gates) {
  hipLaunchKernelGGL(k_q_perm, q_grid(a), dim3(QUOTIENT_THREADS), 0, s, a, have_gates);
}
u32 launch_quotient_full_tier(hipStream_t s, const QuotientArgs &a, const std::vector<GateDev> &host_gates, const QuotientTiers &t) {
  return launch_gates<false>(s, a, host_gates, nullptr, t.bundle_of.data(), -1);
}
void launch_quotient_half_tier(hipStream_t s, const QuotientArgs &a, const std::vector<GateDev> &host_gates, const QuotientTiers &t, u64 *planes) {
  for (size_t b = 0; b < t.bundles.size(); b++) {
    QuotientArgs ab = a;
    ab.out = planes + (u64)b * a.num_challenges * a.N;
    launch_gates<false>(s, ab, host_gates, nullptr, t.bundle_of.data(), (int)b);
  }
}

struct TierCombine { u32 count; u32 selector_index[8], group_start[8], group_end[8]; u64 mask[8]; };
__global__ __launch_bounds__(256) void k_q_tier_combine(QuotientArgs a, const u64 *__restrict__ planes, TierCombine T, u32 accumulate) {
  const u64 i = (u64)blockIdx.x * 256 + threadIdx.x;
  if (i >= a.count) return;
  const u32 CH = a.num_challenges;
  const u64 ig = a.leaf0 + i;
  u64 acc[QUOTIENT_MAX_CH];
#pragma unroll
  for (u32 c = 0; c < QUOTIENT_MAX_CH; c++) acc[c] = (c < CH && accumulate) ? a.out[(u64)c * a.N + ig] : 0;
  for (u32 b = 0; b < T.count; b++) {
    const u32 gs = T.group_start[b], ge = T.group_end[b];
    const u64 mask = T.mask[b];
    const u64 s = a.consts[(u64)T.selector_index[b] * a.stride + i];
    u64 v[QUOTIENT_MAX_CH];
#pragma unroll
    for (u32 c = 0; c < QUOTIENT_MAX_CH; c++) v[c] = c < CH ? planes[((u64)b * CH + c) * a.N + ig] : 0;
    u64 f = 1;
    for (u32 j = gs; j < ge; j++) {
      const bool in_bundle = (mask >> ((j - gs) & 63)) & 1;
      if (!in_bundle) f = gl_mul(f, gl_sub((u64)j, s));
    }
    if (a.num_selectors > 1) f = gl_mul(f, gl_sub(0xFFFFFFFFull, s));
#pragma unroll
    for (u32 c = 0; c < QUOTIENT_MAX_CH; c++)
      if (c < CH) acc[c] = gl_add(acc[c], gl_mul(f, v[c]));
  }
#pragma unroll
  for (u32 c = 0; c < QUOTIENT_MAX_CH; c++)
    if (c < CH) a.out[(u64)c * a.N + ig] = acc[c];
}
void launch_tier_combine(hipStream_t s, const QuotientArgs &a, const QuotientTiers &t, const u64 *planes, u32 accumulate) {
  for (size_t b0 = 0; b0 < t.bundles.size(); b0 += 8) {
    TierCombine T{};
    T.count = (u32)std::min<size_t>(8, t.bundles.size() - b0);
    for (u32 k = 0; k < T.count; k++) {
      const QuotientBundle &B = t.bundles[b0 + k];
      T.selector_index[k] = B.selector_index; T.group_start[k] = B.group_start; T.group_end[k] = B.group_end; T.mask[k] = B.mask;
    }
    hipLaunchKernelGGL(k_q_tier_combine, dim3((unsigned)((a.count + 255) / 256)), dim3(256), 0, s, a, planes + (u64)b0 * a.num_challenges * a.N, T, b0 ? 1u : accumulate);
  }
}
void launch_gate_check(hipStream_t s, const QuotientArgs &a, const std::vector<GateDev> &host_gates, unsigned long long *flag) {
  launch_gates<true>(s, a, host_gates, flag);
}
void launch_native_check(hipStream_t s, const QuotientArgs &a, const std::vector<GateDev> &host_gates, unsigned long long *flag) {
  auto kind_of = [&](u32 g) { return host_gates[g].flags & LCP2_GATE_NATIVE_MASK; };
  for (u32 g = 0; g < host_gates.size(); g++) {
    const u32 kind = kind_of(g);
    if (kind & 0x8000u) { launch_generated(s, a, (kind >> 8) & 0x7Fu, g, 0, flag, GEN_CLAIM_CHECK); continue; }
    switch (kind) {
      case LCP2_GATE_NATIVE_POSEIDON: launch_claim_check<QPoseidon>(s, a, g, flag); break;
      case LCP2_GATE_NATIVE_ARITHMETIC: launch_claim_check<QArithmetic>(s, a, g, flag);
        for (u32 gB = 0; gB < host_gates.size() && pairable(g) && pairable(gB); gB++)
          if (kind_of(gB) == LCP2_GATE_NATIVE_BASE_SUM2) launch_claim_check<QArithBasePair>(s, a, g | gB << 16, flag);
        break;
      case LCP2_GATE_NATIVE_BASE_SUM2: launch_claim_check<QBaseSum2>(s, a, g, flag); break;
      default: break;
    }
  }
}

__global__ __launch_bounds__(256) void k_quotient_setup(QuotientSetupArgs a) {
  const u32 t = threadIdx.x, CH = a.num_challenges;
  if (t < QUOTIENT_TERM_POWS) {
    for (u32 c = 0; c < QUOTIENT_MAX_CH; c++) {
      const u64 pw = c < CH ? gl_pow(a.alphas[c], t) : 0;
      u32 *w = a.limbs + ((size_t)c * QUOTIENT_TERM_POWS + t) * 4;
      w[0] = (u32)(pw & 0x3FFFFF); w[1] = (u32)((pw >> 22) & 0x3FFFFF); w[2] = (u32)(pw >> 44); w[3] = 0;
      if (t < QUOTIENT_ALPHA_POWS) a.small[SMALL_ALPHA_POW + (size_t)c * QUOTIENT_ALPHA_POWS + t] = pw;
    }
  } else if (t < 255) {
    for (u32 g = t - QUOTIENT_TERM_POWS; g < a.num_gates; g += 255 - QUOTIENT_TERM_POWS) {
      const u32 m = konst((const u32 *)a.gates)[(size_t)g * GW_WORDS + GW_NUM_CONSTRAINTS];
      for (u32 c = 0; c < QUOTIENT_MAX_CH; c++) a.small[SMALL_GATE_SCALE + (size_t)g * QUOTIENT_MAX_CH + c] = c < CH ? (m ? gl_pow(a.alphas[c], m - 1) : 1) : 0;
    }
  } else {
    for (u32 c = 0; c < 4; c++) {
      const u64 al = c < CH ? a.alphas[c] : 0;
      a.small[SMALL_ALPHAS + c] = al;
      a.small[SMALL_ALPHA_INV + c] = al ? gl_inv(al) : 0;
      a.small[SMALL_PI_HASH + c] = a.pi_hash[c];
    }
    a.small[SMALL_CHECK] = ~0ull;
  }
}
void launch_quotient_setup(hipStream_t s, const QuotientSetupArgs &a) {
  static_assert(QUOTIENT_TERM_POWS < 255 && QUOTIENT_MAX_CH <= 4 && QUOTIENT_ALPHA_POWS <= QUOTIENT_TERM_POWS, "k_quotient_setup's thread map");
  hipLaunchKernelGGL(k_quotient_setup, dim3(1), dim3(256), 0, s, a);
}

__global__ __launch_bounds__(256) void k_quotient_combine(const u64 *__restrict__ in, u64 *__restrict__ out, const u64 *__restrict__ m, u64 n, u32 R, u64 plane) {
  const u64 l = (u64)blockIdx.x * 256 + threadIdx.x;
  if (l >= n) return;
  const u64 base = (u64)blockIdx.y * plane + l;
  u64 r[8];
#pragma unroll
  for (u32 b = 0; b < 8; b++) r[b] = b < R ? in[base + (u64)b * n] : 0;
  for (u32 k = 0; k < R; k++) {
    u64 acc = 0;
#pragma unroll
    for (u32 b = 0; b < 8; b++)
      if (b < R) acc = gl_add(acc, gl_mul(m[k * R + b], r[b]));
    out[base + (u64)k * n] = acc;
  }
}
void launch_quotient_combine(hipStream_t s, const u64 *in, u64 *out, const u64 *m, u64 n, u32 R, u64 plane, u32 num_challenges) {
  hipLaunchKernelGGL(k_quotient_combine, dim3((unsigned)((n + 255) / 256), num_challenges), dim3(256), 0, s, in, out, m, n, R, plane);
}
}
```

### eth-lc-plonky2_amd/csrc/prover_build.hip

```cpp
#include <algorithm>
#include <cstdlib>
#include "circuit_state.hpp"
#include "gate_program.hpp"

using namespace lcp2;
namespace gp = gate_program;

namespace lcp2 {
const char *params_problem(const lcp2_params &p, bool *unsupported) {
  *unsupported = false;
  if (p.degree_bits < 1 || p.rate_bits < 1 || p.rate_bits > 8 || p.degree_bits + p.rate_bits > 30) return "degree_bits / rate_bits out of range";
  if (p.num_wires == 0 || p.num_wires > 65535 || p.num_constants > 65535) return "bad column counts";
  if (p.num_routed_wires > p.num_wires || p.num_routed_wires == 0) return "bad routed wire count";
  if (p.cap_height > p.degree_bits + p.rate_bits) return "cap_height exceeds the LDE tree";
  *unsupported = true;
  if (p.quotient_degree_factor < 2 || p.quotient_degree_factor > (1u << p.rate_bits)) return "quotient_degree_factor must lie in [2, 2^rate_bits]";
  if (p.num_challenges < 1 || p.num_challenges > QUOTIENT_MAX_CH) return "num_challenges must be 1 or 2";
  if ((p.num_routed_wires + p.quotient_degree_factor - 1) / p.quotient_degree_factor > PERM_MAX_CHUNKS) return "too many routed wires";
  if (p.num_query_rounds > 64 || p.num_fri_layers > LCP2_MAX_FRI_LAYERS) return "too many queries / layers";
  if (p.proof_of_work_bits < 1 || p.proof_of_work_bits > 40) return "proof_of_work_bits out of range";
  *unsupported = false;
  u32 lg = p.degree_bits + p.rate_bits, d = p.degree_bits;
  for (u32 l = 0; l < p.num_fri_layers; l++) {
    u32 ab = p.fri_arity_bits[l];
    if (ab < 1 || ab > 5 || ab > d || lg - ab < p.cap_height) return "bad FRI arity schedule";
    lg -= ab; d -= ab;
  }
  return nullptr;
}
}

namespace {
static_assert(QUOTIENT_TERM_POWS == 128, "the limit LIGHT_GATE_LIMIT names");
const char *const LIGHT_GATE_LIMIT = "LCP2_GATE_NATIVE_ARITHMETIC / LCP2_GATE_NATIVE_BASE_SUM2: at most 128 constraints (the alpha power table holds 128 weights)";
const char *validate_programs(const lcp2_circuit_desc *d) {
  const lcp2_params &p = d->params;
  if (d->num_regs > 64 || d->num_selectors > p.num_constants) return "bad gate set";
  const gp::Limits limits{std::max(d->num_regs, 1u), p.num_wires, p.num_constants - d->num_selectors, d->num_imm, 4};
  for (u32 g = 0; g < d->num_gates; g++) {
    const lcp2_gate &G = d->gates[g];
    if (G.selector_index >= d->num_selectors || ((size_t)G.code_offset + (size_t)G.code_len) * 2 > d->code_words || G.group_end < G.group_start ||
        (G.flags & ~(LCP2_GATE_EMIT_FORWARD | LCP2_GATE_NATIVE_MASK)))
      return "gate descriptor out of range";
    switch (G.flags & LCP2_GATE_NATIVE_MASK) {
      case 0: break;
      case LCP2_GATE_NATIVE_POSEIDON:
        if (!(G.flags & LCP2_GATE_EMIT_FORWARD) || G.num_constraints != 123 || p.num_wires < 135) return "LCP2_GATE_NATIVE_POSEIDON needs 135 wires, 123 forward-emitted constraints";
        break;
      case LCP2_GATE_NATIVE_ARITHMETIC:
        if ((G.flags & LCP2_GATE_EMIT_FORWARD) || G.num_constraints == 0 || 4 * (size_t)G.num_constraints > p.num_wires || p.num_constants - d->num_selectors < 2)
          return "LCP2_GATE_NATIVE_ARITHMETIC needs 4 wires per operation and 2 gate constants";
        if (G.num_constraints > QUOTIENT_TERM_POWS) return LIGHT_GATE_LIMIT;
        break;
      case LCP2_GATE_NATIVE_BASE_SUM2:
        if ((G.flags & LCP2_GATE_EMIT_FORWARD) || G.num_constraints < 2 || G.num_constraints > p.num_wires) return "LCP2_GATE_NATIVE_BASE_SUM2 needs num_limbs + 1 wires";
        if (G.num_constraints > QUOTIENT_TERM_POWS) return LIGHT_GATE_LIMIT;
        break;
      default:
        if (!(G.flags & 0x8000u) || ((G.flags >> 8) & 0x7Fu) >= QUOTIENT_GENERATED_GATES || G.num_constraints > QUOTIENT_TERM_POWS) return "unknown native gate id";
        break;
    }
    size_t emits_seen = 0;
    for (size_t pc = G.code_offset; pc < (size_t)G.code_offset + G.code_len; pc++) {
      const gp::Insn in(d->code[2 * pc], d->code[2 * pc + 1]);
      if (const char *why = gp::insn_problem(in, limits)) return why;
      emits_seen += in.emits();
    }
    if (emits_seen != G.num_constraints) return "num_constraints does not match the program";
  }
  return nullptr;
}

constexpr u32 DEGREE_CAP = 1u << 20;
struct DegreeAlg {
  using V = u32; using S = u32;
  V wire(u32) { return 1; }    V gate_const(u32) { return 1; }    V imm(u64) { return 0; }    V pi(u32) { return 0; }    S scalar(u64) { return 0; }
  V add(V a, V b) { return std::max(a, b); }    V sub(V a, V b) { return std::max(a, b); }    V mul(V a, V b) { return std::min(a + b, DEGREE_CAP); }
  V mul_add(V a, V b, V acc) { return std::max(acc, mul(a, b)); }
  V scale_add(V x, S, V acc) { return std::max(x, acc); }
};
u32 program_degree(const uint32_t *code, size_t first, size_t len, size_t nregs) {
  std::vector<u32> reg(std::max<size_t>(nregs, 1), 0);
  DegreeAlg A;
  u32 deg = 0;
  gp::walk_program(A, code, first, len, (const u64 *)nullptr, reg.data(), [&](u32 d) { deg = std::max(deg, d); });
  return deg;
}

void form_bundles(lcp2_circuit *c) {
  QuotientTiers &t = c->tiers;
  t.bundles.clear();
  t.bundle_of.assign(c->gates.size(), -1);
  const u32 qb = c->qbits();
  if (qb == 0) return;
  const u32 half = 1u << (qb - 1);
  std::vector<u32> order;
  for (u32 g = 0; g < c->gates.size(); g++) {
    const lcp2_gate &G = c->gates[g];
    if (G.num_constraints == 0 || c->gate_degree[g] > half) continue;
    if (G.selector_value < G.group_start || G.selector_value >= G.group_end || G.group_end - G.group_start > 64) continue;
    order.push_back(g);
  }
  std::stable_sort(order.begin(), order.end(), [&](u32 x, u32 y) { return c->gate_degree[x] > c->gate_degree[y]; });
  std::vector<u32> maxdeg;
  for (u32 g : order) {
    const lcp2_gate &G = c->gates[g];
    size_t b = 0;
    for (; b < t.bundles.size(); b++) {
      const QuotientBundle &B = t.bundles[b];
      if (B.selector_index == G.selector_index && B.group_start == G.group_start && B.group_end == G.group_end &&
          maxdeg[b] + B.gates.size() <= half && !((B.mask >> (G.selector_value - G.group_start)) & 1))
        break;
    }
    if (b == t.bundles.size()) {
      t.bundles.push_back(QuotientBundle{G.selector_index, G.group_start, G.group_end, 0, {}});
      maxdeg.push_back(c->gate_degree[g]);
    }
    t.bundles[b].gates.push_back(g);
    t.bundles[b].mask |= 1ull << (G.selector_value - G.group_start);
    t.bundle_of[g] = (int)b;
  }
}

void circuit_digest(const std::vector<u64> &cs_cap, u32 degree_bits, u64 digest[4]) {
  std::vector<u64> buf(cs_cap);
  const u64 empty_padded[8] = {1, 0, 0, 0, 0, 0, 0, 1};
  u64 ds[4];
  HostPoseidon::get().hash_no_pad(empty_padded, 8, ds);
  buf.insert(buf.end(), ds, ds + 4);
  buf.push_back(degree_bits);
  HostPoseidon::get().hash_no_pad(buf.data(), buf.size(), digest);
}

int check_native_gates(lcp2_circuit *c) {
  lcp2_ctx *ctx = c->ctx;
  bool any = false;
  for (const lcp2_gate &G : c->gates) any = any || (G.flags & LCP2_GATE_NATIVE_MASK);
  if (!any) return LCP2_OK;
  const lcp2_params &p = c->p;
  const u64 cnt = 256;
  u64 seed = 0x9E3779B97F4A7C15ull;
  auto rnd = [&]() { seed += 0x9E3779B97F4A7C15ull; u64 z = seed; z = (z ^ (z >> 30)) * 0xBF58476D1CE4E5B9ull; z = (z ^ (z >> 27)) * 0x94D049BB133111EBull; return gl_canon(z ^ (z >> 31)); };
  std::vector<u64> hw((size_t)p.num_wires * cnt), hc((size_t)p.num_constants * cnt);
  for (auto &v : hw) v = rnd();
  for (auto &v : hc) v = rnd();
  DevBuf dw, dc;
  LCP2_TRY(upload(ctx, dw, hw.data(), hw.size() * 8));
  LCP2_TRY(upload(ctx, dc, hc.data(), hc.size() * 8));
  LCP2_HIP(ctx, c->alpha_limbs.ensure((size_t)QUOTIENT_MAX_CH * QUOTIENT_TERM_POWS * 16));
  u64 *d_small = c->small.u();
  QuotientSetupArgs qs{};
  for (u32 i = 0; i < 4; i++) qs.pi_hash[i] = rnd();
  qs.num_challenges = p.num_challenges; qs.num_gates = (u32)c->gates.size(); qs.gates = (const GateDev *)c->d_gates.p; qs.small = d_small;
  qs.limbs = (u32 *)c->alpha_limbs.p;
  QuotientArgs a{};
  a.wires = dw.u(); a.consts = dc.u(); a.stride = cnt; a.count = cnt;
  a.alphas = d_small + SMALL_ALPHAS; a.alpha_inv = d_small + SMALL_ALPHA_INV; a.pis = d_small + SMALL_PI_HASH; a.gate_scale = d_small + SMALL_GATE_SCALE;
  a.alpha_limbs = (const u32 *)c->alpha_limbs.p;
  a.imm = c->d_imm.u(); a.code = (const u32 *)c->d_code.p; a.gates = (const GateDev *)c->d_gates.p; a.stage_list = (const u32 *)c->d_stage.p;
  a.num_wires = p.num_wires; a.num_gates = (u32)c->gates.size(); a.num_selectors = c->num_selectors; a.num_constants = p.num_constants;
  a.num_challenges = p.num_challenges; a.num_regs = c->num_regs; a.rc = ctx->d_rc;
  u64 bad = ~0ull;
  for (int zero_alpha = 0; zero_alpha < 2 && bad == ~0ull; zero_alpha++) {
    for (u32 k = 0; k < p.num_challenges; k++) qs.alphas[k] = zero_alpha ? 0 : gl_canon(rnd() | 1);
    launch_quotient_setup(ctx->stream, qs);
    launch_native_check(ctx->stream, a, c->dev_gates, (unsigned long long *)(d_small + SMALL_CHECK));
    LCP2_HIP(ctx, hipGetLastError());
    LCP2_TRY(download(ctx, &bad, d_small + SMALL_CHECK, 8));
  }
  if (bad != ~0ull) return ctx->fail(LCP2_E_INVALID, "a gate flagged LCP2_GATE_NATIVE_* does not compute what its program computes");
  return LCP2_OK;
}

void copy_description(lcp2_circuit *c, const lcp2_circuit_desc *d) {
  const lcp2_params &p = d->params;
  c->p = p; c->npi = d->num_public_inputs; c->num_selectors = d->num_selectors; c->num_regs = std::max(d->num_regs, 1u);
  c->gates.assign(d->gates, d->gates + d->num_gates);
  c->code.assign(d->code, d->code + d->code_words);
  c->imm.resize(std::max<size_t>(d->num_imm, 1), 0);
  for (size_t i = 0; i < d->num_imm; i++) c->imm[i] = gl_canon(d->imm[i]);
  c->k_is.resize(p.num_routed_wires);
  for (u32 i = 0; i < p.num_routed_wires; i++) c->k_is[i] = gl_canon(d->k_is[i]);
  c->gate_degree.resize(c->gates.size());
  for (size_t g = 0; g < c->gates.size(); g++) c->gate_degree[g] = program_degree(c->code.data(), c->gates[g].code_offset, c->gates[g].code_len, c->num_regs);
  c->tiers.bundle_of.assign(c->gates.size(), -1);
}

int circuit_create(lcp2_ctx *ctx, const lcp2_circuit_desc *d, uint32_t bf, uint32_t bc, lcp2_circuit **out) {
  if (!ctx || !d || !out) return LCP2_E_INVALID;
  *out = nullptr;
  if (!d->constants_sigmas || !d->k_is || !d->gates || !d->code || (d->num_imm && !d->imm)) return ctx->fail(LCP2_E_INVALID, "null description field");
  LCP2_TRY(check_params(ctx, d->params));
  const lcp2_params &p = d->params;
  if (d->num_selectors > p.num_constants || d->num_regs > 64 || d->num_gates == 0) return ctx->fail(LCP2_E_INVALID, "bad gate set");
  if (d->num_public_inputs > (1u << 20)) return ctx->fail(LCP2_E_UNSUPPORTED, "too many public inputs");
  if (const char *why = validate_programs(d)) return ctx->fail(LCP2_E_INVALID, why);
  LCP2_HIP(ctx, hipSetDevice(ctx->device));
  std::unique_ptr<lcp2_circuit> c(new lcp2_circuit());
  c->ctx = ctx;
  if (bc) {
    if (p.quotient_degree_factor != (1u << p.rate_bits)) return ctx->fail(LCP2_E_UNSUPPORTED, "sharded circuit: needs quotient_degree_factor = 2^rate_bits");
    if (p.cap_height < p.rate_bits) return ctx->fail(LCP2_E_INVALID, "sharded circuit: needs cap_height >= rate_bits");
    if ((bc & (bc - 1)) || bf % bc || bf + bc > (1u << p.rate_bits)) return ctx->fail(LCP2_E_INVALID, "sharded circuit: block range must be an aligned power of two");
    c->bf = bf; c->bc = bc; c->cap_final = false;
    for (lcp2_oracle *o : c->oracles()) { o->block_first = bf; o->block_count = bc; }
  }
  copy_description(c.get(), d);
  const u64 n = 1ull << p.degree_bits, N = n << p.rate_bits;
  const u32 ncs = p.num_constants + p.num_routed_wires, CH = p.num_challenges, npp = npp_of(p), nchunks = npp + 1;
  {
    static_assert(sizeof(GateDev) == sizeof(lcp2_gate), "GateDev mirrors lcp2_gate");
    std::vector<GateDev> &dev_gates = c->dev_gates;
    dev_gates.resize(c->gates.size());
    memcpy(dev_gates.data(), c->gates.data(), c->gates.size() * sizeof(lcp2_gate));
    std::vector<uint32_t> staged, lists;
    stage_gate_programs(c->code, dev_gates, p.num_wires, c->num_selectors, staged, lists);
    c->dev_regs = 1;
    for (const lcp2_gate &G : c->gates) {
      if (G.flags & LCP2_GATE_NATIVE_MASK) continue;
      for (size_t pc = G.code_offset; pc < (size_t)G.code_offset + G.code_len; pc++)
        c->dev_regs = std::max(c->dev_regs, gp::Insn(c->code[2 * pc], c->code[2 * pc + 1]).top_reg());
    }
    staged.resize(staged.size() + 4, 0);
    LCP2_TRY(upload(ctx, c->d_gates, dev_gates.data(), dev_gates.size() * sizeof(GateDev)));
    LCP2_TRY(upload(ctx, c->d_code, staged.data(), staged.size() * 4));
    LCP2_TRY(upload(ctx, c->d_stage, lists.data(), lists.size() * 4));
    LCP2_HIP(ctx, hipStreamSynchronize(ctx->stream));
  }
  LCP2_TRY(upload(ctx, c->d_imm, c->imm.data(), c->imm.size() * 8));
  LCP2_TRY(upload(ctx, c->d_kis, c->k_is.data(), c->k_is.size() * 8));
  LCP2_HIP(ctx, c->cs_values.alloc((size_t)ncs * n * 8));
  LCP2_HIP(ctx, hipMemcpyAsync(c->cs_values.p, d->constants_sigmas, (size_t)ncs * n * 8,
                               d->constants_sigmas_mem == LCP2_MEM_DEVICE ? hipMemcpyDeviceToDevice : hipMemcpyHostToDevice, ctx->stream));
  LCP2_TRY(commit_values_dev(ctx, c->cs_values.u(), ncs, p.degree_bits, p.rate_bits, p.cap_height, &c->cs));
  const size_t capw = (size_t)4 << p.cap_height;
  c->cs_cap.resize(capw);
  {
    Download dl(ctx);
    LCP2_TRY(queue_cap(dl, c.get(), c->cs.cap_dev(), c->cs_cap.data()));
    LCP2_TRY(dl.wait());
  }
  if (!c->sharded()) circuit_digest(c->cs_cap, p.degree_bits, c->digest);
  {
    DevBuf ones;
    LCP2_HIP(ctx, ones.alloc(n * 8));
    launch_fill(ctx->stream, ones.u(), n, gl_inv(n % GL_P));
    LCP2_HIP(ctx, c->d_l0.alloc(N * 8));
    DeviceNttBackend be{ctx};
    NttHost<DeviceNttBackend> ntt(be);
    ntt.forward(ones.u(), n, c->d_l0.u(), N, p.degree_bits, 1, GL_GENERATOR, p.rate_bits);
    if (be.status) return be.status;
    LCP2_HIP(ctx, hipStreamSynchronize(ctx->stream));
  }
  const u32 qb = c->qbits();
  const u64 NQ = n << qb;
  {
    std::vector<u64> t(1u << qb);
    u64 shift_n = gl_pow(GL_GENERATOR, n), wr = gl_root_of_unity(qb);
    for (u32 top = 0; top < (1u << qb); top++) {
      u32 r = bitrev32(top, qb);
      t[top] = gl_inv(gl_sub(gl_mul(shift_n, gl_pow(wr, r)), 1));
    }
    LCP2_TRY(upload(ctx, c->d_zh_inv, t.data(), t.size() * 8));
  }
  LCP2_HIP(ctx, c->zs_vals.alloc((size_t)CH * (1 + npp) * n * 8));
  LCP2_HIP(ctx, c->chunk_q.alloc((size_t)CH * nchunks * n * 8));
  LCP2_HIP(ctx, c->row_tot.alloc((size_t)CH * n * 8));
  LCP2_HIP(ctx, c->scan_tmp.alloc(std::max(scan_scratch_words(n, 4), (u64)16) * 8));
  LCP2_HIP(ctx, c->qvals.alloc((size_t)CH * NQ * 8));
  {
    const char *sw = getenv("LCP2_QUOTIENT_TIERS");
    if (!c->sharded() && !(sw && sw[0] == '0' && !sw[1])) form_bundles(c.get());
    if (c->tiers.on()) {
      std::vector<u64> masks(c->gates.size(), 0);
      for (const QuotientBundle &B : c->tiers.bundles)
        for (u32 g : B.gates) masks[g] = B.mask;
      LCP2_TRY(upload(ctx, c->d_half_mask, masks.data(), masks.size() * 8));
      LCP2_HIP(ctx, hipStreamSynchronize(ctx->stream));
      LCP2_HIP(ctx, c->tier_planes.alloc(c->tiers.bundles.size() * (size_t)CH * NQ * 8));
      LCP2_HIP(ctx, hipMemsetAsync(c->tier_planes.p, 0, c->tiers.bundles.size() * (size_t)CH * NQ * 8, ctx->stream));
      DeviceNttBackend be{ctx};
      NttHost<DeviceNttBackend> ntt(be);
      LCP2_TRY(tier_extend(c.get(), ntt));
      if (be.status) return be.status;
      LCP2_HIP(ctx, hipStreamSynchronize(ctx->stream));
    }
  }
  LCP2_HIP(ctx, c->planes.alloc((size_t)4 * n * 8));
  LCP2_HIP(ctx, c->small.alloc((SMALL_GATE_SCALE + (size_t)QUOTIENT_MAX_CH * d->num_gates + 8) * 8));
  {
    u32 maxcols = std::max(std::max(ncs, p.num_wires), std::max(CH * (1 + npp), CH * p.quotient_degree_factor));
    u64 nchk = (n + EVAL_CHUNK - 1) / EVAL_CHUNK;
    LCP2_HIP(ctx, c->partial.alloc((size_t)maxcols * nchk * 16 + (size_t)maxcols * 16));
  }
  LCP2_HIP(ctx, c->tables.alloc(((size_t)8 * ((1ull << ((p.degree_bits + 1) / 2)) + (n >> ((p.degree_bits + 1) / 2)) + 2) + 4 * 1024 + 2 * (ncs + p.num_wires + 64) + 64) * 16));
  LCP2_HIP(ctx, c->fri_c[0].alloc((size_t)2 * n * 8));
  LCP2_HIP(ctx, c->fri_c[1].alloc((size_t)2 * n * 8));
  {
    u64 m = n;
    c->fri_vals.resize(p.num_fri_layers); c->fri_dig.resize(p.num_fri_layers);
    c->fri_level_off.resize(p.num_fri_layers); c->fri_d_level_off.resize(p.num_fri_layers);
    for (u32 l = 0; l < p.num_fri_layers; l++) {
      u64 nvals = m << p.rate_bits, nleaves = nvals >> p.fri_arity_bits[l];
      u32 h = 0;
      while ((1ull << h) < nleaves) h++;
      u32 nlev = h - p.cap_height + 1;
      if (l == 0 && c->sharded()) {
        nvals = (u64)c->bc * m;
        nleaves = nvals >> p.fri_arity_bits[0];
      }
      LCP2_HIP(ctx, c->fri_vals[l].alloc((size_t)2 * nvals * 8));
      c->fri_level_off[l].resize(nlev);
      u64 tot = 0;
      for (u32 k = 0; k < nlev; k++) { c->fri_level_off[l][k] = tot; tot += nleaves >> k; }
      LCP2_HIP(ctx, c->fri_dig[l].alloc(tot * 32));
      LCP2_TRY(upload(ctx, c->fri_d_level_off[l], c->fri_level_off[l].data(), nlev * 8));
      m >>= p.fri_arity_bits[l];
    }
  }
  LCP2_HIP(ctx, c->q_idx.alloc(64 * 8 * (3 + LCP2_MAX_FRI_LAYERS)));
  LCP2_HIP(ctx, c->q_buf.alloc((size_t)64 * (ncs + p.num_wires + CH * (1 + npp) + CH * p.quotient_degree_factor + 4 * 4 * 32 + LCP2_MAX_FRI_LAYERS * (64 + 4 * 32)) * 8));
  LCP2_HIP(ctx, hipStreamSynchronize(ctx->stream));
  LCP2_TRY(check_native_gates(c.get()));
  *out = c.release();
  return LCP2_OK;
}
}

extern "C" int lcp2_circuit_create(lcp2_ctx *ctx, const lcp2_circuit_desc *d, lcp2_circuit **out) { return circuit_create(ctx, d, 0, 0, out); }
extern "C" int lcp2_circuit_create_sharded(lcp2_ctx *ctx, const lcp2_circuit_desc *d, uint32_t block_first, uint32_t block_count,
                                           lcp2_circuit **out) {
  if (block_count == 0) return LCP2_E_INVALID;
  return circuit_create(ctx, d, block_first, block_count, out);
}
extern "C" int lcp2_circuit_set_constants_cap(lcp2_circuit *c, const uint64_t *cap) {
  if (!c || !cap) return LCP2_E_INVALID;
  if (!c->sharded()) return LCP2_E_INVALID;
  const lcp2_circuit::Range mine = c->cap_share();
  if (memcmp(cap + mine.first, c->cs_cap.data() + mine.first, mine.count * 8) != 0)
    return c->ctx->fail(LCP2_E_INVALID, "constants cap does not contain this shard's entries");
  c->cs_cap.assign((const u64 *)cap, (const u64 *)cap + c->cs_cap.size());
  circuit_digest(c->cs_cap, c->p.degree_bits, c->digest);
  c->cap_final = true;
  return LCP2_OK;
}

extern "C" int lcp2_verifier_create(const lcp2_circuit_desc *d, const uint64_t digest[4], const uint64_t *cap, lcp2_circuit **out) {
  if (!d || !digest || !cap || !out || !d->k_is || !d->gates || !d->code) return LCP2_E_INVALID;
  *out = nullptr;
  const lcp2_params &p = d->params;
  bool unsupported;
  if (params_problem(p, &unsupported)) return unsupported ? LCP2_E_UNSUPPORTED : LCP2_E_INVALID;
  if (d->num_selectors > p.num_constants || d->num_gates == 0 || (d->num_imm && !d->imm)) return LCP2_E_INVALID;
  if (validate_programs(d)) return LCP2_E_INVALID;
  lcp2_circuit *c = new lcp2_circuit();
  copy_description(c, d);
  memcpy(c->digest, digest, 32);
  c->cs_cap.assign((const u64 *)cap, (const u64 *)cap + ((size_t)4 << p.cap_height));
  *out = c;
  return LCP2_OK;
}

extern "C" void lcp2_circuit_destroy(lcp2_circuit *c) {
  if (!c) return;
  if (c->ctx) { (void)hipSetDevice(c->ctx->device); (void)hipStreamSynchronize(c->ctx->stream); }
  delete c;
}
extern "C" int lcp2_circuit_digest(const lcp2_circuit *c, uint64_t digest[4], uint64_t *cap) {
  if (!c || !digest) return LCP2_E_INVALID;
  memcpy(digest, c->digest, 32);
  if (cap) memcpy(cap, c->cs_cap.data(), c->cs_cap.size() * 8);
  return LCP2_OK;
}
extern "C" size_t lcp2_proof_words(const lcp2_params *p) {
  bool unsupported;
  if (!p || params_problem(*p, &unsupported)) return 0;
  return ProofLayout(*p).total;
}
extern "C" int lcp2_gate_program_degree(const uint32_t *code, size_t num_instructions, uint32_t num_regs, uint32_t *degree) {
  if (!code || !degree || num_regs > 64) return LCP2_E_INVALID;
  const gp::Limits registers_only{std::max(num_regs, 1u)};
  for (size_t pc = 0; pc < num_instructions; pc++)
    if (gp::insn_problem(gp::Insn(code[2 * pc], code[2 * pc + 1]), registers_only)) return LCP2_E_INVALID;
  *degree = program_degree(code, 0, num_instructions, registers_only.regs);
  return LCP2_OK;
}
extern "C" int lcp2_circuit_gate_tiers(const lcp2_circuit *c, uint32_t num_gates, uint32_t *degrees, int32_t *bundles) {
  if (!c || num_gates != c->gates.size()) return LCP2_E_INVALID;
  for (uint32_t g = 0; g < num_gates; g++) {
    if (degrees) degrees[g] = c->gate_degree[g];
    if (bundles) bundles[g] = c->tiers.bundle_of[g];
  }
  return LCP2_OK;
}
extern "C" int lcp2_last_challenges(const lcp2_circuit *c, uint64_t out[97]) {
  if (!c || !out) return LCP2_E_INVALID;
  memcpy(out, c->last_challenges, sizeof c->last_challenges);
  return LCP2_OK;
}

namespace lcp2 {
VerifierView verifier_view(const lcp2_circuit *c) {
  VerifierView v;
  v.p = &c->p; v.npi = c->npi; v.num_selectors = c->num_selectors;
  v.gates = c->gates.data(); v.num_gates = (u32)c->gates.size(); v.code = c->code.data(); v.imm = c->imm.data();
  v.k_is = c->k_is.data(); v.digest = c->digest; v.cs_cap = c->cs_cap.data();
  v.code_words = c->code.size(); v.num_imm = c->imm.size(); v.num_regs = c->num_regs;
  return v;
}
}
```

### eth-lc-plonky2_amd/csrc/prover_kernels.hpp

```cpp
#pragma once
#include <hip/hip_runtime.h>
#include <cstddef>
#include <vector>
#include "gate_staging.hpp"
#include "gl64.hpp"
#include "ntt.hpp"

namespace lcp2 {

constexpr u32 PERM_MAX_CHUNKS = 10;
constexpr u32 QUOTIENT_THREADS = 128;
constexpr u32 QUOTIENT_MAX_CH = 2;
constexpr u32 QUOTIENT_ALPHA_POWS = 32;
constexpr u32 QUOTIENT_TERM_POWS = 128;
constexpr u32 QUOTIENT_GENERATED_GATES = 17;
constexpr u32 EVAL_CHUNK = 4096;

constexpr size_t SMALL_BETAS = 0, SMALL_GAMMAS = 4, SMALL_ALPHAS = 8, SMALL_ALPHA_INV = 12, SMALL_PI_HASH = 16, SMALL_POW = 20,
                 SMALL_CHECK = 21, SMALL_NONCANON = 22, SMALL_TRIM = 23, SMALL_PERM_PREFIX = 24, SMALL_ALPHA_POW = 32, SMALL_GATE_SCALE = SMALL_ALPHA_POW + QUOTIENT_MAX_CH * QUOTIENT_ALPHA_POWS;

struct GateDev {
  u32 selector_index, selector_value, group_start, group_end, code_offset, code_len, num_constraints, flags;
};
constexpr u32 GW_NUM_CONSTRAINTS = 6, GW_FLAGS = 7, GW_WORDS = 8;
static_assert(sizeof(GateDev) == 4 * GW_WORDS && offsetof(GateDev, num_constraints) == 4 * GW_NUM_CONSTRAINTS && offsetof(GateDev, flags) == 4 * GW_FLAGS, "GateDev's words");

struct PermArgs {
  const u64 *wires;
  const u64 *sigmas;
  const u64 *k_is;
  TwoLevelTable subgroup;
  const u64 *betas, *gammas;
  const u64 *prefix;
  u64 *chunk_q;
  u64 *row_tot;
  u64 *zs_out;
  u64 n, row0;
  u64 wires_stride, sigma_stride;
  u32 num_routed, chunk, nchunks, num_challenges;
};

struct QuotientArgs {
  const u64 *wires;
  const u64 *consts;
  const u64 *zs;
  const u64 *l0;
  const u64 *zh_inv;
  TwoLevelTable points;
  const u64 *k_is, *betas, *gammas, *alphas, *pis, *imm;
  u32 kis_pow7;
  const u32 *stage_list;
  u32 num_wires;
  const u64 *rc;
  const u64 *alpha_pow;
  u32 limbs_lds_word;
  const u32 *alpha_limbs;
  const u64 *alpha_inv;
  const u64 *gate_scale;
  const u32 *code;
  const GateDev *gates;
  const u64 *half_mask;
  u64 *out;
  u64 N;
  u64 leaf0, count, stride;
  u32 lgN, rate_bits, num_gates, num_selectors, num_constants, num_routed, chunk, nchunks, num_challenges, num_regs;
};

struct EvalArgs {
  const u64 *coeffs;
  u64 col_stride;
  u32 chunk_len, items, nchunks;
  u64 zstep[2];
  const u64 *zpow_t;
  const u64 *zpow_chunk;
  u64 *partial;
};

struct ComposeArgs {
  const u64 *coeffs[4];
  u32 ncols[4];
  u32 num_challenges;
  u64 n;
  const u64 *alpha_pows;
  const u64 *z0_lo, *z0_hi, *z1_lo, *z1_hi;
  const u64 *zi0_lo, *zi0_hi, *zi1_lo, *zi1_hi;
  u32 zh;
  u64 zmask;
  u64 alpha_shift[2];
  u64 *planes;
};

struct PowArgs {
  u64 state[12];
  u32 pos, bits;
  u64 start;
  const u64 *rc;
  u64 *result;
};

void launch_scan(hipStream_t s, bool mul, const u64 *in, u64 *out, u64 *block_tot, u64 n, bool reverse, u32 batches, u64 batch_stride);
u64 scan_scratch_words(u64 n, u32 batches);
void launch_quotient_combine(hipStream_t s, const u64 *in, u64 *out, const u64 *m, u64 n, u32 R, u64 plane, u32 num_challenges);
void launch_perm_chunks(hipStream_t s, const PermArgs &a);
void launch_perm_finalize(hipStream_t s, const PermArgs &a);
void launch_quotient(hipStream_t s, const QuotientArgs &a, const std::vector<GateDev> &host_gates);
struct QuotientBundle {
  u32 selector_index, group_start, group_end;
  u64 mask;
  std::vector<u32> gates;
};
struct QuotientTiers {
  std::vector<QuotientBundle> bundles;
  std::vector<int> bundle_of;
  bool on() const { return !bundles.empty(); }
};
u32 launch_quotient_full_tier(hipStream_t s, const QuotientArgs &a, const std::vector<GateDev> &host_gates, const QuotientTiers &t);
void launch_quotient_half_tier(hipStream_t s, const QuotientArgs &a, const std::vector<GateDev> &host_gates, const QuotientTiers &t, u64 *planes);
void launch_tier_combine(hipStream_t s, const QuotientArgs &a, const QuotientTiers &t, const u64 *planes, u32 accumulate);
void launch_quotient_perm(hipStream_t s, const QuotientArgs &a, u32 have_gates);
void stage_gate_programs(const std::vector<uint32_t> &code, std::vector<GateDev> &gates, u32 num_wires, u32 num_selectors,
                         std::vector<uint32_t> &staged_code, std::vector<uint32_t> &stage_list);
void launch_gate_check(hipStream_t s, const QuotientArgs &a, const std::vector<GateDev> &host_gates, unsigned long long *flag);
void launch_native_check(hipStream_t s, const QuotientArgs &a, const std::vector<GateDev> &host_gates, unsigned long long *flag);
void launch_eval_polys(hipStream_t s, const EvalArgs &a, u32 npolys, u64 *out);
void launch_compose(hipStream_t s, const ComposeArgs &a);
void launch_divide_finalize(hipStream_t s, const ComposeArgs &a, u64 *out0, u64 *out1);
void launch_fri_fold(hipStream_t s, const u64 *c0, const u64 *c1, u64 *o0, u64 *o1, u64 nout, u32 arity, u64 b0, u64 b1);
void launch_gather_ext_leaves(hipStream_t s, const u64 *p0, const u64 *p1, u32 arity, const u64 *leaf_idx, u32 k, u64 *out);
void launch_pow_search(hipStream_t s, const PowArgs &a, u64 count);
void launch_fill(hipStream_t s, u64 *p, u64 n, u64 v);
struct U32JobDev;
void launch_u32_gate_rows(hipStream_t s, const U32JobDev *jobs, u64 njobs, u64 *wires, u64 n, u64 *flag);
struct RecJobDev;
struct RecOperandDev;
void launch_rec_gate_rows(hipStream_t s, const RecJobDev *jobs, u64 base, u64 begin, u64 end, const RecOperandDev *operands, u64 noperands,
                          u64 *wires, u32 ncols, u64 n, u64 *flag, bool check_structure);
struct PosJobDev;
void launch_pos_plan_chains(hipStream_t s, const PosJobDev *jobs, u64 npos, const u32 *chain_ends, u64 chain_begin, u64 chain_end,
                            const RecOperandDev *operands, u64 noperands, u64 *wires, u32 ncols, u64 n, const u64 *rc, u64 *flags, u64 gate,
                            u64 marker);
struct U32PlanJobDev;
void launch_u32_plan_rows(hipStream_t s, const U32PlanJobDev *jobs, u64 base, u64 begin, u64 end, const RecOperandDev *operands, u64 noperands,
                          u64 *wires, u32 ncols, u64 n, u64 *flags, u64 gate, u64 marker);
void launch_any_nonzero(hipStream_t s, const u64 *p, u64 pitch, u64 width, u32 rows, unsigned long long *flag);

struct SmallWords { u64 v[16]; };
void launch_set_words(hipStream_t s, u64 *dst, const SmallWords &w, u32 n);
struct QuotientSetupArgs {
  u64 alphas[QUOTIENT_MAX_CH], pi_hash[4];
  u32 num_challenges, num_gates;
  const GateDev *gates;
  u64 *small;
  u32 *limbs;
};
void launch_quotient_setup(hipStream_t s, const QuotientSetupArgs &a);
void launch_eval_tables(hipStream_t s, u64 z0, u64 z1, u32 chunk_len, u32 nchunks, u64 *tab);
void launch_compose_tables(hipStream_t s, u64 a0, u64 a1, u64 z0, u64 z1, u64 g, u32 total_polys, u32 h, u64 hi_count, u64 *T);

}
```

### eth-lc-plonky2_amd/csrc/quotient_common.hpp

```cpp
#pragma once
#include "internal.hpp"
#include "poseidon.hpp"
#include "prover_kernels.hpp"
#include "gate_helpers.hpp"

namespace lcp2 {

template <class T> using const_as = const T __attribute__((address_space(4))) *;
template <class T> __device__ __forceinline__ const_as<T> konst(const T *p) { return (const_as<T>)(unsigned long long)p; }

__device__ __forceinline__ u64 q_operand(const QuotientArgs &a, u32 kind, u32 idx, const u64 *lds, u32 T, u32 tid, u64 i) {
  switch (kind) {
    case 0: return lds[idx * T + tid];
    case 1: return a.wires[(u64)idx * a.stride + i];
    case 2: return a.consts[(u64)(a.num_selectors + idx) * a.stride + i];
    case 3: return konst(a.imm)[idx];
    case 4: return konst(a.pis)[idx];
    default: return lds[(a.num_regs + idx) * T + tid];
  }
}

__device__ __forceinline__ void q_stage(const QuotientArgs &a, u32 cnt, const_as<u32> lst, u64 *lds, u32 T, u32 tid, u64 i) {
  u64 v[QUOTIENT_STAGE];
#pragma unroll
  for (u32 j = 0; j < QUOTIENT_STAGE; j++) {
    const u32 e = lst[j < cnt ? j : 0];
    const u64 *col = e < a.num_wires ? a.wires + (u64)e * a.stride : a.consts + (u64)(e - a.num_wires) * a.stride;
    v[j] = col[i];
  }
#pragma unroll
  for (u32 j = 0; j < QUOTIENT_STAGE; j++)
    if (j < cnt) lds[(a.num_regs + j) * T + tid] = v[j];
}

#if defined(__HIP_DEVICE_COMPILE__)
__device__ __forceinline__ void q_pmds(u64 *lds, u32 T, u32 tid, u32 dst, u32 src, const_as<u64> add) {
  u32 lo[12], hi[12];
  u64 rc[12];
#pragma unroll
  for (int j = 0; j < 12; j++) rc[j] = add[j];
#pragma unroll
  for (int j = 0; j < 12; j++) { const u64 v = lds[(src + j) * T + tid]; lo[j] = (u32)v; hi[j] = (u32)(v >> 32); }
  pos_mds_h(lo, hi, rc);
#pragma unroll
  for (int j = 0; j < 12; j++) lds[(dst + j) * T + tid] = gl_canon(((u64)hi[j] << 32) | lo[j]);
}
__device__ __forceinline__ u64 q_sbox(u64 x) {
  u32 x0 = (u32)x, x1 = (u32)(x >> 32);
  pos_sbox_h(x0, x1);
  return gl_canon(((u64)x1 << 32) | x0);
}
#else
__device__ void q_pmds(u64 *lds, u32 T, u32 tid, u32 dst, u32 src, const_as<u64> add);
__device__ u64 q_sbox(u64 x);
#endif

#if defined(__HIP_DEVICE_COMPILE__)
struct QTermCols {
  u64 col[QUOTIENT_MAX_CH][6];
  __device__ __forceinline__ void clear() {
#pragma unroll
    for (u32 c = 0; c < QUOTIENT_MAX_CH; c++)
#pragma unroll
      for (u32 l = 0; l < 6; l++) col[c][l] = 0;
  }
  __device__ __forceinline__ void fold(u64 out[QUOTIENT_MAX_CH], u32 ch) const {
#pragma unroll
    for (u32 c = 0; c < QUOTIENT_MAX_CH; c++) {
      if (c < ch) {
        u64 v[3];
#pragma unroll
        for (u32 l = 0; l < 3; l++) {
          const u64 lo = col[c][l] + (col[c][3 + l] << 32);
          const u64 hi = (col[c][3 + l] >> 32) + (lo < col[c][l] ? 1 : 0);
          v[l] = gl_reduce128(lo, hi);
        }
        out[c] = gl_add(v[0], gl_add(gl_shl<22>(v[1]), gl_shl<44>(v[2])));
      }
    }
  }
};
struct QTerms : QTermCols {
  u32 CH;
  __device__ __forceinline__ void init(u32 ch) { CH = ch; clear(); }
  template <u32 E>
  __device__ __forceinline__ void add(const QuotientArgs &a, u64 x) {
    static_assert(E < QUOTIENT_TERM_POWS, "too many constraints for the alpha power table");
    add(a, E, x);
  }
  __device__ __forceinline__ void add(const QuotientArgs &a, u32 e , u64 x) {
    const u32 x0 = (u32)x, x1 = (u32)(x >> 32);
#pragma unroll
    for (u32 c = 0; c < QUOTIENT_MAX_CH; c++) {
      if (c < CH) {
        const_as<u32> L = konst(a.alpha_limbs) + ((size_t)c * QUOTIENT_TERM_POWS + e) * 4;
#pragma unroll
        for (u32 l = 0; l < 3; l++) {
          const u32 w = L[l];
          col[c][l] += (u64)x0 * w;
          col[c][3 + l] += (u64)x1 * w;
        }
      }
    }
  }
  __device__ __forceinline__ void fold(u64 out[QUOTIENT_MAX_CH]) const { QTermCols::fold(out, CH); }
};
typedef const __attribute__((address_space(3))) u32 *lds_u32_ptr;
struct QTermsLds : QTermCols {
  lds_u32_ptr limbs;
  __device__ __forceinline__ void init() { clear(); }
  __device__ __forceinline__ void pin() {
#pragma unroll
    for (u32 c = 0; c < QUOTIENT_MAX_CH; c++)
#pragma unroll
      for (u32 l = 0; l < 6; l++) asm volatile("" : "+v"(col[c][l]));
  }
  template <u32 E>
  __device__ __forceinline__ void add(u64 x) {
    static_assert(E < QUOTIENT_TERM_POWS, "too many constraints for the alpha power table");
    const u32 x0 = (u32)x, x1 = (u32)(x >> 32);
#pragma unroll
    for (u32 c = 0; c < QUOTIENT_MAX_CH; c++) {
      lds_u32_ptr L = limbs + ((size_t)c * QUOTIENT_TERM_POWS + E) * 4;
#pragma unroll
      for (u32 l = 0; l < 3; l++) {
        const u32 w = L[l];
        col[c][l] += (u64)x0 * w;
        col[c][3 + l] += (u64)x1 * w;
      }
    }
  }
  __device__ __forceinline__ void fold(u64 out[QUOTIENT_MAX_CH]) const { QTermCols::fold(out, QUOTIENT_MAX_CH); }
};
struct QEmit {
  u64 acc[QUOTIENT_MAX_CH], step[QUOTIENT_MAX_CH];
  u32 CH, emitted;
  bool weighted = false;
  QTerms t;
  QTermsLds tl;
  __device__ __forceinline__ void begin_terms_lds() { tl.init(); }
  __device__ __forceinline__ void finish_terms_lds() { tl.fold(acc); weighted = true; }
  __device__ __forceinline__ void begin_terms() { t.init(CH); }
  __device__ __forceinline__ void term(const QuotientArgs &a, u32 e, u64 x) { t.add(a, e, x); }
  __device__ __forceinline__ void finish_terms() { t.fold(acc); weighted = true; }
  __device__ __forceinline__ void operator()(u64 x) {
#pragma unroll
    for (u32 c = 0; c < QUOTIENT_MAX_CH; c++)
      if (c < CH) acc[c] = step[c] == 0 ? (emitted ? acc[c] : x) : gl_add_nc(gl_mul_nc(acc[c], step[c]), x);
    emitted++;
  }
  __device__ __forceinline__ void horner(u64 x) {
#pragma unroll
    for (u32 c = 0; c < QUOTIENT_MAX_CH; c++)
      if (c < CH) acc[c] = gl_add_nc(gl_mul_nc(acc[c], step[c]), x);
  }
};
#endif

}

#define Q_PIN(x) asm volatile("" : "+v"(x))
#define Q_WINDOW_BARRIER() do { asm volatile("" ::: "memory"); __builtin_amdgcn_sched_barrier(0); } while (0)
#include "generated_gates.hpp"

namespace lcp2 {
static_assert(Q_GENERATED_COUNT == QUOTIENT_GENERATED_GATES, "prover_kernels.hpp and generated_gates.hpp disagree");
#if defined(__HIP_DEVICE_COMPILE__)
template <u32 K> __device__ __forceinline__ void q_generated(const QuotientArgs &a, u64 i, QEmit &emit);
#endif

constexpr u32 Q_LIMB_WORDS32 = QUOTIENT_MAX_CH * QUOTIENT_TERM_POWS * 4;
__device__ __forceinline__ void q_stage_limbs(const QuotientArgs &a, u64 *lds, u32 T, u32 tid) {
#if defined(__HIP_DEVICE_COMPILE__)
  u32 *dst = (u32 *)(lds + a.limbs_lds_word);
  for (u32 j = tid; j < Q_LIMB_WORDS32; j += T) dst[j] = konst(a.alpha_limbs)[j];
  __syncthreads();
#endif
}

#if defined(__HIP_DEVICE_COMPILE__)
__device__ __forceinline__ void q_emit_begin(const QuotientArgs &a, const GateDev &G, QEmit &emit) {
  const u32 CH = a.num_challenges;
  const bool fwd = (G.flags & LCP2_GATE_EMIT_FORWARD) != 0;
  emit.CH = CH; emit.emitted = 0;
#pragma unroll
  for (u32 c = 0; c < QUOTIENT_MAX_CH; c++) { emit.acc[c] = 0; emit.step[c] = c < CH ? (fwd ? konst(a.alpha_inv)[c] : konst(a.alphas)[c]) : 0; }
}
__device__ __forceinline__ void q_interpret(const QuotientArgs &a, const GateDev &G, u64 i, u64 *lds, u32 T, u32 tid, QEmit &emit) {
  const bool fwd = (G.flags & LCP2_GATE_EMIT_FORWARD) != 0;
  const_as<u64> code2 = konst((const u64 *)a.code);
  u64 nxt = code2[G.code_offset];
  for (u32 pc = G.code_offset; pc < G.code_offset + G.code_len; pc++) {
    const u32 w0 = (u32)nxt, w1 = (u32)(nxt >> 32);
    nxt = code2[pc + 1];
    const u32 op = w0 & 0xF, dst = (w0 >> 8) & 0xFF, ka = (w0 >> 16) & 0xF, kb = (w0 >> 20) & 0xF, ia = w1 & 0xFFFF, ib = w1 >> 16;
    if (op == QOP_LDG) { q_stage(a, dst, konst(a.stage_list) + w1, lds, T, tid, i); continue; }
    if (op == LCP2_OP_PMDS) { q_pmds(lds, T, tid, dst, ia, konst(a.imm) + ib); continue; }
    u64 x = q_operand(a, ka, ia, lds, T, tid, i);
    if (op == LCP2_OP_EMIT || op == LCP2_OP_EMITBOOL) {
      if (op == LCP2_OP_EMITBOOL) x = gl_sub(gl_mul(x, x), x);
      if (fwd) emit(x); else emit.horner(x);
      continue;
    }
    if (op == LCP2_OP_SBOX) { lds[dst * T + tid] = q_sbox(x); continue; }
    u64 y = q_operand(a, kb, ib, lds, T, tid, i);
    u64 r;
    switch (op) {
      case LCP2_OP_ADD: r = gl_add(x, y); break;
      case LCP2_OP_SUB: r = gl_sub(x, y); break;
      case LCP2_OP_MUL: r = gl_mul(x, y); break;
      case LCP2_OP_XOR: { const u64 xy = gl_mul(x, y); r = gl_sub(gl_sub(gl_add(x, y), xy), xy); break; }
      case LCP2_OP_DBLADD: r = gl_add(gl_add(x, x), y); break;
      default: r = gl_add(lds[dst * T + tid], gl_mul(x, y)); break;
    }
    lds[dst * T + tid] = r;
  }
}
__device__ __forceinline__ u64 q_filter(const QuotientArgs &a, u32 g, const GateDev &G, u64 i) {
  const u64 s = a.consts[(u64)G.selector_index * a.stride + i];
  const bool half = a.half_mask != nullptr;
  const u64 keep = half ? konst(a.half_mask)[g] : ~0ull;
  u64 f = 1;
  for (u32 j = G.group_start; j < G.group_end; j++)
    if (j != G.selector_value && ((keep >> ((j - G.group_start) & 63)) & 1)) f = gl_mul(f, gl_sub((u64)j, s));
  if (a.num_selectors > 1 && !half) f = gl_mul(f, gl_sub(0xFFFFFFFFull, s));
  return f;
}
__device__ __forceinline__ void q_gate_finish(const QuotientArgs &a, u32 g, const GateDev &G, u64 i, const QEmit &emit, u64 val[QUOTIENT_MAX_CH]) {
  const u32 CH = a.num_challenges;
  const bool fwd = (G.flags & LCP2_GATE_EMIT_FORWARD) != 0;
  const u64 f = q_filter(a, g, G, i);
#pragma unroll
  for (u32 c = 0; c < QUOTIENT_MAX_CH; c++)
    if (c < CH) {
      const u64 sum = (fwd && !emit.weighted && emit.step[c] != 0) ? gl_mul(emit.acc[c], konst(a.gate_scale)[g * QUOTIENT_MAX_CH + c]) : emit.acc[c];
      val[c] = gl_mul(f, sum);
    }
}
struct QInterpreted {
  static __device__ __forceinline__ void run(const QuotientArgs &a, const GateDev &G, u64 i, u64 *lds, u32 T, u32 tid, QEmit &emit) { q_interpret(a, G, i, lds, T, tid, emit); }
};
template <class EVAL>
__device__ __forceinline__ void q_gate_value(const QuotientArgs &a, u32 g, const GateDev &G, u64 i, u64 *lds, u32 T, u32 tid, u64 val[QUOTIENT_MAX_CH]) {
  QEmit emit;
  q_emit_begin(a, G, emit);
  emit.tl.limbs = (lds_u32_ptr)(lds + a.limbs_lds_word);
  EVAL::run(a, G, i, lds, T, tid, emit);
  q_gate_finish(a, g, G, i, emit, val);
}
#endif
__device__ __forceinline__ GateDev q_load_gate(const QuotientArgs &a, u32 g) {
  GateDev G;
  const_as<u32> gw = konst((const u32 *)a.gates) + (size_t)g * GW_WORDS;
  G.selector_index = gw[0]; G.selector_value = gw[1]; G.group_start = gw[2]; G.group_end = gw[3];
  G.code_offset = gw[4]; G.code_len = gw[5]; G.num_constraints = gw[GW_NUM_CONSTRAINTS]; G.flags = gw[GW_FLAGS];
  return G;
}

template <bool CHECK>
__device__ __forceinline__ bool q_point(const QuotientArgs &a, u64 &i) {
  const u64 i0 = (u64)blockIdx.x * QUOTIENT_THREADS + threadIdx.x;
  i = !CHECK || i0 < a.count ? i0 : a.count - 1;
  return CHECK || i0 < a.count;
}
template <bool CHECK>
__device__ __forceinline__ bool q_wave_holds(const QuotientArgs &a, const GateDev &G, u64 i) {
  if (!CHECK) return true;
  const u64 sel = a.consts[(u64)G.selector_index * a.stride + i];
  return __any(sel == G.selector_value);
}
template <bool CHECK>
__device__ __forceinline__ void q_gate_store(const QuotientArgs &a, u64 i, const u64 (&val)[QUOTIENT_MAX_CH], u32 accumulate, unsigned long long *flag) {
  if (CHECK) {
    bool bad = false;
#pragma unroll
    for (u32 c = 0; c < QUOTIENT_MAX_CH; c++)
      if (c < a.num_challenges && val[c] != 0) bad = true;
    if (bad) atomicMin(flag, (unsigned long long)i + 1);
  } else {
    const u64 ig = a.leaf0 + i;
#pragma unroll
    for (u32 c = 0; c < QUOTIENT_MAX_CH; c++)
      if (c < a.num_challenges) a.out[(u64)c * a.N + ig] = accumulate ? gl_add(a.out[(u64)c * a.N + ig], val[c]) : val[c];
  }
}
__device__ __forceinline__ void q_claim_compare(const QuotientArgs &a, u64 i, const u64 (&r0)[QUOTIENT_MAX_CH], const u64 (&r1)[QUOTIENT_MAX_CH], unsigned long long *flag) {
  bool bad = false;
#pragma unroll
  for (u32 c = 0; c < QUOTIENT_MAX_CH; c++)
    if (c < a.num_challenges && r0[c] != r1[c]) bad = true;
  if (bad) atomicMin(flag, (unsigned long long)i + 1);
}
template <class EVAL>
__device__ __forceinline__ void q_claim_check(const QuotientArgs &a, u32 g, u64 i, u64 *lds, u32 T, u32 tid, unsigned long long *flag) {
#if defined(__HIP_DEVICE_COMPILE__)
  const GateDev G = q_load_gate(a, g);
  u64 r0[QUOTIENT_MAX_CH], r1[QUOTIENT_MAX_CH];
  q_gate_value<QInterpreted>(a, g, G, i, lds, T, tid, r0);
  q_gate_value<EVAL>(a, g, G, i, lds, T, tid, r1);
  q_claim_compare(a, i, r0, r1, flag);
#endif
}

inline dim3 q_grid(const QuotientArgs &a) { return dim3((unsigned)((a.count + QUOTIENT_THREADS - 1) / QUOTIENT_THREADS)); }
inline size_t q_interp_lds_bytes(const QuotientArgs &a) { return (size_t)(a.num_regs + QUOTIENT_STAGE) * QUOTIENT_THREADS * sizeof(u64); }
}
```

### include/lcp2.h

```cpp
#ifndef LCP2_H
#define LCP2_H
#include <stddef.h>
#include <stdint.h>

#ifdef __cplusplus
extern "C" {
#endif

#define LCP2_ABI_VERSION 2

typedef enum {
  LCP2_OK = 0,
  LCP2_E_INVALID = -1,
  LCP2_E_NODEVICE = -2,
  LCP2_E_HIP = -3,
  LCP2_E_OOM = -4,
  LCP2_E_UNSAT = -5,
  LCP2_E_UNSUPPORTED = -6,
  LCP2_E_VERIFY = -7
} lcp2_status;

typedef enum { LCP2_MEM_HOST = 0, LCP2_MEM_DEVICE = 1 } lcp2_mem;

#define LCP2_MAX_FRI_LAYERS 8
typedef struct {
  uint32_t degree_bits;
  uint32_t num_wires;
  uint32_t num_routed_wires;
  uint32_t num_constants;
  uint32_t rate_bits;
  uint32_t cap_height;
  uint32_t num_challenges;
  uint32_t quotient_degree_factor;
  uint32_t proof_of_work_bits;
  uint32_t num_query_rounds;
  uint32_t num_fri_layers;
  uint32_t fri_arity_bits[LCP2_MAX_FRI_LAYERS];
} lcp2_params;

int lcp2_params_standard(uint32_t degree_bits, uint32_t num_constants, lcp2_params *p);
int lcp2_params_config(uint32_t degree_bits, uint32_t num_constants, uint32_t rate_bits, uint32_t cap_height,
                       uint32_t proof_of_work_bits, uint32_t num_query_rounds, uint32_t arity_bits, uint32_t final_poly_bits,
                       lcp2_params *p);

typedef struct lcp2_ctx lcp2_ctx;
typedef struct lcp2_oracle lcp2_oracle;

const char *lcp2_status_str(int status);
int lcp2_abi_version(void);
int lcp2_device_count(void);

int lcp2_ctx_create(int device, void *stream, lcp2_ctx **out);
#define LCP2_CTX_ORDER_WITH_DEFAULT_STREAM 1u
int lcp2_ctx_create_ex(int device, void *stream, uint32_t flags, lcp2_ctx **out);
void lcp2_ctx_destroy(lcp2_ctx *ctx);
int lcp2_ctx_sync(lcp2_ctx *ctx);
void *lcp2_ctx_stream(lcp2_ctx *ctx);
const char *lcp2_last_error(lcp2_ctx *ctx);


int lcp2_poseidon_permute_batch(lcp2_ctx *ctx, const uint64_t *in, uint64_t *out, size_t count, lcp2_mem mem);

enum {
  LCP2_FIELD_MUL = 0,
  LCP2_FIELD_POW7 = 1,
  LCP2_FIELD_ADD = 2,
  LCP2_FIELD_SUB = 3,
  LCP2_FIELD_CANON = 4,
  LCP2_FIELD_ADD_LAZY = 5,
  LCP2_FIELD_SUB_LAZY = 6,
  LCP2_FIELD_SHL = 16
};
int lcp2_field_op_batch(lcp2_ctx *ctx, const uint64_t *a, const uint64_t *b, uint64_t *out, size_t count, uint32_t op, lcp2_mem mem);

int lcp2_merkle_cap(lcp2_ctx *ctx, const uint64_t *leaves, size_t nleaves, size_t leaf_len,
                    uint32_t cap_height, lcp2_mem mem, uint64_t *cap );

int lcp2_ntt_batch(lcp2_ctx *ctx, uint64_t *data, size_t ncols, uint32_t log_n, int inverse,
                   uint64_t shift, lcp2_mem mem);

int lcp2_lde_batch(lcp2_ctx *ctx, const uint64_t *coeffs, uint64_t *out, size_t ncols, uint32_t log_n,
                   uint32_t rate_bits, lcp2_mem mem);

int lcp2_sha256_tree(lcp2_ctx *ctx, const uint8_t *leaves, uint32_t height, size_t trees,
                     uint8_t *nodes, uint32_t *round_trace, lcp2_mem mem);

typedef struct {
  uint32_t first_row;
  int32_t in_src[16];
} lcp2_sha_job;
typedef struct {
  uint32_t row, col;
  uint64_t value;
} lcp2_cell;
int lcp2_sha256_witness(lcp2_ctx *ctx, const lcp2_sha_job *jobs, size_t njobs, const uint32_t *level_start, uint32_t nlevels,
                        const uint32_t *words_in, size_t nwords, uint64_t *wires, uint64_t n, uint32_t *digests);
int lcp2_scatter_cells(lcp2_ctx *ctx, const lcp2_cell *cells, size_t ncells, uint64_t *wires, uint64_t n);
typedef struct {
  uint32_t row;
  uint32_t swap;
  uint64_t in[12];
} lcp2_poseidon_row;
int lcp2_poseidon_gate_rows(lcp2_ctx *ctx, const lcp2_poseidon_row *rows, size_t nrows, uint64_t *wires, uint64_t n);
enum { LCP2_U32_ARITHMETIC = 0, LCP2_U32_ADD_MANY = 1, LCP2_U32_SUBTRACTION = 2, LCP2_U32_RANGE_CHECK = 3, LCP2_U32_COMPARISON = 4 };
typedef struct {
  uint32_t row;
  uint16_t kind;
  uint16_t op;
  uint32_t in[4];
} lcp2_u32_job;
int lcp2_u32_gate_rows(lcp2_ctx *ctx, const lcp2_u32_job *jobs, size_t njobs, lcp2_mem jobs_mem,
                       uint64_t *wires , uint64_t n);

enum { LCP2_REC_ARITHMETIC = 0, LCP2_REC_BASE_SUM, LCP2_REC_ARITHMETIC_EXT, LCP2_REC_MUL_EXT, LCP2_REC_REDUCING,
       LCP2_REC_REDUCING_EXT, LCP2_REC_POSEIDON_MDS, LCP2_REC_RANDOM_ACCESS, LCP2_REC_EXPONENTIATION,
       LCP2_REC_COSET_INTERPOLATION, LCP2_REC_KINDS };
enum { LCP2_REC_IMM = 0, LCP2_REC_CELL = 1 };
typedef struct {
  uint64_t v;
  uint32_t col;
  uint32_t src;
} lcp2_rec_operand;
typedef struct {
  uint32_t row;
  uint16_t kind;
  uint16_t op;
  uint32_t first_operand, reserved;
} lcp2_rec_job;
int lcp2_rec_gate_rows(lcp2_ctx *ctx, const lcp2_rec_job *jobs, size_t njobs,
                       const lcp2_rec_operand *operands, size_t noperands,
                       const uint32_t *level_ends , size_t nlevels,
                       lcp2_mem lists_mem ,
                       uint64_t *wires , uint32_t ncols, uint64_t n);

enum { LCP2_PLAN_IMM = 0, LCP2_PLAN_CELL = 1, LCP2_PLAN_PREV = 2 };
typedef struct { uint32_t row, first_operand; } lcp2_pos_job;
typedef struct {
  const lcp2_rec_job *rec_jobs;  size_t nrec;    const uint32_t *rec_level_ends;
  const lcp2_pos_job *pos_jobs;  size_t npos;
  const uint32_t *chain_ends;    size_t nchains;
  const uint32_t *pos_level_ends;
  const lcp2_rec_operand *operands; size_t noperands;
  size_t nlevels;
} lcp2_witness_plan;
int lcp2_witness_plan_rows(lcp2_ctx *ctx, const lcp2_witness_plan *plan, lcp2_mem lists_mem,
                           uint64_t *wires , uint32_t ncols, uint64_t n);

typedef struct { uint32_t row; uint16_t kind , op; uint32_t first_operand, reserved; } lcp2_u32_plan_job;
typedef struct {
  lcp2_witness_plan base;
  const lcp2_u32_plan_job *u32_jobs; size_t nu32;
  const uint32_t *u32_level_ends;
} lcp2_witness_plan_u32;
int lcp2_witness_plan_rows_u32(lcp2_ctx *ctx, const lcp2_witness_plan_u32 *plan, lcp2_mem lists_mem,
                               uint64_t *wires , uint32_t ncols, uint64_t n);

int lcp2_buffer_alloc(lcp2_ctx *ctx, size_t bytes, void **dev);
int lcp2_buffer_free(lcp2_ctx *ctx, void *dev);
int lcp2_buffer_zero(lcp2_ctx *ctx, void *dev, size_t bytes);
int lcp2_buffer_read(lcp2_ctx *ctx, void *host_dst, const void *dev_src, size_t bytes);
int lcp2_buffer_write(lcp2_ctx *ctx, void *dev_dst, const void *host_src, size_t bytes);
int lcp2_buffer_copy(lcp2_ctx *ctx, void *dev_dst, const void *dev_src, size_t bytes);
int lcp2_buffer_copy_2d(lcp2_ctx *ctx, void *dev_dst, size_t dst_pitch, const void *dev_src, size_t src_pitch, size_t width, size_t height);

int lcp2_commit_values(lcp2_ctx *ctx, const uint64_t *cols, size_t ncols, uint32_t log_n, uint32_t rate_bits,
                       uint32_t cap_height, lcp2_mem mem, lcp2_oracle **out, uint64_t *cap);
int lcp2_commit_coeffs(lcp2_ctx *ctx, const uint64_t *coeffs, size_t ncols, uint32_t log_n, uint32_t rate_bits,
                       uint32_t cap_height, lcp2_mem mem, lcp2_oracle **out, uint64_t *cap);
int lcp2_commit_cosets(lcp2_ctx *ctx, const uint64_t *coeffs, size_t ncols, uint32_t log_n, uint32_t rate_bits, uint32_t cap_height,
                       uint32_t block_first, uint32_t block_count, lcp2_mem mem, lcp2_oracle **out, uint64_t *cap_part);
void lcp2_oracle_destroy(lcp2_oracle *o);
int lcp2_oracle_open(lcp2_oracle *o, const uint64_t *indices, size_t k, uint64_t *leaves, uint64_t *siblings);
int lcp2_oracle_read(lcp2_oracle *o, uint64_t *coeffs , uint64_t *lde );

enum { LCP2_OP_ADD = 0, LCP2_OP_SUB = 1, LCP2_OP_MUL = 2, LCP2_OP_EMIT = 3, LCP2_OP_XOR = 4, LCP2_OP_DBLADD = 5,
       LCP2_OP_EMITBOOL = 6, LCP2_OP_MULADD = 7, LCP2_OP_SBOX = 8, LCP2_OP_PMDS = 9 };
#define LCP2_GATE_EMIT_FORWARD 1u
#define LCP2_GATE_NATIVE_MASK 0xFF00u
#define LCP2_GATE_NATIVE_POSEIDON 0x0100u
#define LCP2_GATE_NATIVE_ARITHMETIC 0x0200u
#define LCP2_GATE_NATIVE_BASE_SUM2 0x0300u
#define LCP2_GATE_NATIVE_GENERATED(k) (0x8000u | ((uint32_t)(k) << 8))
typedef struct {
  uint32_t selector_index, selector_value, group_start, group_end;
  uint32_t code_offset, code_len;
  uint32_t num_constraints;
  uint32_t flags;
} lcp2_gate;

typedef struct {
  lcp2_params params;
  const uint64_t *constants_sigmas;
  lcp2_mem constants_sigmas_mem;
  const uint64_t *k_is;
  uint32_t num_selectors;
  uint32_t num_gates;
  const lcp2_gate *gates;
  const uint32_t *code;
  size_t code_words;
  const uint64_t *imm;
  size_t num_imm;
  uint32_t num_public_inputs;
  uint32_t num_regs;
} lcp2_circuit_desc;

typedef struct lcp2_circuit lcp2_circuit;

int lcp2_circuit_create(lcp2_ctx *ctx, const lcp2_circuit_desc *desc, lcp2_circuit **out);
void lcp2_circuit_destroy(lcp2_circuit *c);
int lcp2_circuit_digest(const lcp2_circuit *c, uint64_t digest[4], uint64_t *cap);

typedef struct { uint32_t row, col, cls; } lcp2_copy_binding;
typedef struct {
  const uint32_t *gate_of_row; size_t num_rows;
  uint32_t pad_gate;
  const uint64_t *row_constants;
  const lcp2_copy_binding *bindings; size_t num_bindings; lcp2_mem bindings_mem;
  uint32_t num_classes;
} lcp2_circuit_rows;
int lcp2_circuit_rows_expand(lcp2_ctx *ctx, const lcp2_circuit_desc *desc, const lcp2_circuit_rows *rows, uint64_t *out);
int lcp2_circuit_create_from_rows(lcp2_ctx *ctx, const lcp2_circuit_desc *desc, const lcp2_circuit_rows *rows, lcp2_circuit **out);

size_t lcp2_proof_words(const lcp2_params *p);

typedef struct {
  uint64_t cap_words, wires_cap, zs_cap, quot_cap;
  uint64_t op_constants, op_sigmas, op_wires, op_zs, op_zs_next, op_partial_products, op_quotient;
  uint64_t fri_caps, queries, query_words;
  uint64_t q_init_off[4], q_init_cols[4], q_init_sib;
  uint64_t q_step_off[LCP2_MAX_FRI_LAYERS], q_step_sib[LCP2_MAX_FRI_LAYERS];
  uint64_t final_poly, final_len, pow_witness, total;
} lcp2_proof_layout;
int lcp2_proof_layout_of(const lcp2_params *p, lcp2_proof_layout *out);

int lcp2_prove(lcp2_circuit *c, const uint64_t *wires, lcp2_mem wires_mem, const uint64_t *public_inputs, size_t num_public_inputs,
               uint64_t *proof, size_t proof_words);

typedef struct {
  uint64_t gate_violations;
  uint64_t gate_row;
  uint32_t gate_index;
  uint32_t gate_constraint;
  uint64_t copy_violations;
  uint64_t copy_row;
  uint32_t copy_wire;
  uint64_t copy_to_row;
  uint32_t copy_to_wire;
  uint64_t noncanonical_cells;
} lcp2_witness_report;
int lcp2_check_witness(lcp2_circuit *c, const uint64_t *wires, lcp2_mem wires_mem, const uint64_t *public_inputs, size_t num_public_inputs,
                       lcp2_witness_report *report, uint64_t *per_gate, uint32_t num_gates);

typedef struct {
  uint64_t num_classes;
  uint64_t classes_set;
  uint64_t cells_filled;
  uint64_t conflicts;
  uint64_t conflict_index;
  uint64_t owner_index;
} lcp2_fill_report;
int lcp2_witness_fill_copies(lcp2_circuit *c, const lcp2_cell *cells, size_t ncells, lcp2_mem cells_mem,
                             uint64_t *wires , lcp2_fill_report *report );
int lcp2_circuit_copy_classes(lcp2_circuit *c, uint32_t *class_of, uint64_t *num_classes);

typedef struct {
  uint32_t row, col;
} lcp2_cell_ref;
int lcp2_witness_settle_copies(lcp2_circuit *c, const lcp2_cell_ref *sources, size_t nsources, lcp2_mem sources_mem,
                               uint64_t *wires , lcp2_fill_report *report );

int lcp2_host_register(lcp2_ctx *ctx, void *host, size_t bytes);
int lcp2_host_unregister(lcp2_ctx *ctx, void *host);
int lcp2_witness_stage(lcp2_circuit *c, const uint64_t *wires, uint32_t slot);
int lcp2_prove_staged(lcp2_circuit *c, uint32_t slot, const uint64_t *public_inputs, size_t num_public_inputs, uint64_t *proof, size_t proof_words);

int lcp2_commit_wires(lcp2_circuit *c, const uint64_t *wires, lcp2_mem wires_mem, uint64_t *cap);
int lcp2_perm_zs(lcp2_circuit *c, const uint64_t *betas, const uint64_t *gammas, uint64_t *cap);
int lcp2_quotient(lcp2_circuit *c, const uint64_t *alphas, const uint64_t public_inputs_hash[4], uint64_t *cap);
typedef struct {
  uint64_t sponge[12];
  uint64_t input[8];
  uint64_t output[8];
  uint32_t input_len, output_len;
} lcp2_challenger;
int lcp2_fri_open(lcp2_circuit *c, const uint64_t zeta[2], lcp2_challenger *ch, uint64_t *proof);

enum { LCP2_SECTION_OPENINGS = 0, LCP2_SECTION_FRI_CAP0 = 1, LCP2_SECTION_AFTER_CAPS = 2 };
int lcp2_fri_open_begin(lcp2_circuit *c, const uint64_t zeta[2], const lcp2_challenger *ch, uint64_t *proof);
int lcp2_fri_open_commit(lcp2_circuit *c, uint64_t *proof);
int lcp2_fri_open_finish(lcp2_circuit *c, lcp2_challenger *ch, uint64_t *proof);
int lcp2_proof_section(const lcp2_circuit *c, int section, size_t *first_word, size_t *num_words);

void lcp2_challenger_init(lcp2_challenger *ch);
int lcp2_challenger_observe(lcp2_challenger *ch, const uint64_t *values, size_t count);
int lcp2_challenger_get(lcp2_challenger *ch, uint64_t *out, size_t count);
int lcp2_hash_no_pad(const uint64_t *values, size_t count, uint64_t out[4]);

int lcp2_circuit_create_sharded(lcp2_ctx *ctx, const lcp2_circuit_desc *desc, uint32_t block_first, uint32_t block_count,
                                lcp2_circuit **out);
int lcp2_circuit_set_constants_cap(lcp2_circuit *c, const uint64_t *cap);
int lcp2_commit_wires_coeffs(lcp2_circuit *c, const uint64_t *wires, const uint64_t *coeffs, uint64_t *cap);
int lcp2_commit_wires_rows(lcp2_circuit *c, const uint64_t *wire_rows, const uint64_t *coeffs, uint64_t *cap);
int lcp2_commit_wires_rows_begin(lcp2_circuit *c, const uint64_t *wire_rows);
int lcp2_commit_wires_chunk(lcp2_circuit *c, const uint64_t *coeffs, uint32_t first_col, uint32_t ncols);
int lcp2_commit_wires_rows_finish(lcp2_circuit *c, uint64_t *cap);
int lcp2_perm_zs_rows_begin(lcp2_circuit *c, const uint64_t *betas, const uint64_t *gammas, uint64_t *block_products);
int lcp2_perm_zs_rows_finish(lcp2_circuit *c, const uint64_t *block_products, uint64_t **device_ptr, size_t *words);
int lcp2_perm_zs_commit(lcp2_circuit *c, uint64_t *cap);
int lcp2_quotient_values(lcp2_circuit *c, const uint64_t *alphas, const uint64_t public_inputs_hash[4]);
int lcp2_quotient_buffer(lcp2_circuit *c, uint64_t **device_ptr, size_t *words);
int lcp2_quotient_commit(lcp2_circuit *c, uint64_t *cap);

int lcp2_verify(const lcp2_circuit *c, const uint64_t *proof, size_t proof_words, const uint64_t *public_inputs,
                size_t num_public_inputs, int *failed_check);

int lcp2_verify_batch(lcp2_ctx *ctx, const lcp2_circuit *c, const uint64_t *proofs, size_t proof_words, size_t count, lcp2_mem proofs_mem,
                      const uint64_t *public_inputs, size_t num_public_inputs, int32_t *failed_checks);

#define LCP2_VERIFY_HEAD_HOST   0u
#define LCP2_VERIFY_HEAD_DEVICE 1u
int lcp2_verify_batch_ex(lcp2_ctx *ctx, const lcp2_circuit *c, const uint64_t *proofs, size_t proof_words, size_t count, lcp2_mem proofs_mem,
                         const uint64_t *public_inputs, size_t num_public_inputs, int32_t *failed_checks, uint32_t flags);

#define LCP2_SER_PUBLIC_INPUT_COUNT 1u
size_t lcp2_proof_bytes(const lcp2_params *p, size_t num_public_inputs, uint32_t flags);
int lcp2_proof_to_bytes(const lcp2_params *p, const uint64_t *proof, size_t proof_words, const uint64_t *public_inputs,
                        size_t num_public_inputs, uint32_t flags, uint8_t *out, size_t out_len);
int lcp2_proof_from_bytes(const lcp2_params *p, const uint8_t *bytes, size_t len, uint32_t flags, uint64_t *proof, size_t proof_words,
                          uint64_t *public_inputs, size_t num_public_inputs);
int lcp2_verifier_data_to_bytes(const lcp2_circuit *c, uint8_t *out, size_t out_len);

int lcp2_verifier_create(const lcp2_circuit_desc *desc, const uint64_t digest[4], const uint64_t *cap, lcp2_circuit **out);

int lcp2_last_challenges(const lcp2_circuit *c, uint64_t out[97]);
int lcp2_gate_program_degree(const uint32_t *code, size_t num_instructions, uint32_t num_regs, uint32_t *degree);
int lcp2_circuit_gate_tiers(const lcp2_circuit *c, uint32_t num_gates, uint32_t *degrees, int32_t *bundles);

typedef enum {
  LCP2_K_INTT = 0,
  LCP2_K_LDE = 1,
  LCP2_K_LEAF_HASH = 2,
  LCP2_K_MERKLE = 3,
  LCP2_K_PERM_Z = 4,
  LCP2_K_QUOTIENT = 5,
  LCP2_K_OPENINGS = 6,
  LCP2_K_FRI = 7,
  LCP2_K_POW = 8,
  LCP2_K_SHA256 = 9,
  LCP2_K_OTHER = 10,
  LCP2_K_COUNT = 11
} lcp2_kernel_family;
int lcp2_prof_enable(lcp2_ctx *ctx, int on);
int lcp2_prof_reset(lcp2_ctx *ctx);
int lcp2_prof_get(lcp2_ctx *ctx, int family, double *total_ms, uint64_t *launches, double *algorithmic_bytes);

#ifdef __cplusplus
}
#endif
#endif
```

Before: 9391.

## Fold light gate lists into generated-gate host kernels to share the quotient walk

Light gates (arithmetic, base-sum, interpreted) that used to get their own k_q_light launches per bundle can now ride inside a chosen generated-gate kernel as a guest. The guest evaluates at the same points and either adds into the host's output or writes to its bundle plane. A host-side planner picks the host gate per bundle under an LDS budget, and an env var can turn it off. This removes separate launches and repeated passes over point data, but the host kernel now needs the interpreter LDS staging area, which may lower occupancy.

```diff
diff --git a/eth-lc-plonky2_amd/binding.py b/eth-lc-plonky2_amd/binding.py
--- a/eth-lc-plonky2_amd/binding.py
+++ b/eth-lc-plonky2_amd/binding.py
@@ -256,6 +256,8 @@
         "lcp2_last_challenges": (c.c_int, [c.c_void_p, c.c_void_p]),
         "lcp2_gate_program_degree": (c.c_int, [c.c_void_p, c.c_size_t, c.c_uint32, c.POINTER(c.c_uint32)]),
         "lcp2_circuit_gate_tiers": (c.c_int, [c.c_void_p, c.c_uint32, c.c_void_p, c.c_void_p]),
+        "lcp2_shared_walk_plan": (c.c_int, [c.c_void_p, c.c_uint32, c.c_void_p, c.c_uint32, c.c_uint32, c.c_void_p]),
+        "lcp2_circuit_shared_walk": (c.c_int, [c.c_void_p, c.c_uint32, c.c_void_p]),
         "lcp2_proof_bytes": (c.c_size_t, [c.POINTER(Params), c.c_size_t, c.c_uint32]),
         "lcp2_proof_to_bytes": (c.c_int, [c.POINTER(Params), c.c_void_p, c.c_size_t, c.c_void_p, c.c_size_t, c.c_uint32, c.c_void_p, c.c_size_t]),
         "lcp2_proof_from_bytes": (c.c_int, [c.POINTER(Params), c.c_void_p, c.c_size_t, c.c_uint32, c.c_void_p, c.c_size_t, c.c_void_p, c.c_size_t]),
@@ -1025,6 +1027,12 @@
         self._check(self.lib.lcp2_circuit_gate_tiers(self.handle, ng, _ptr(deg), _ptr(bun)))
         return deg, bun
 
+    def shared_walk(self):
+        ng = len(self.circ.gateset.gates)
+        hosts = np.zeros(ng, dtype=np.int32)
+        self._check(self.lib.lcp2_circuit_shared_walk(self.handle, ng, _ptr(hosts)))
+        return hosts
+
     def close(self):
         if self.handle:
             self.lib.lcp2_circuit_destroy(self.handle)
diff --git a/eth-lc-plonky2_amd/csrc/kernels_gates.hpp b/eth-lc-plonky2_amd/csrc/kernels_gates.hpp
--- a/eth-lc-plonky2_amd/csrc/kernels_gates.hpp
+++ b/eth-lc-plonky2_amd/csrc/kernels_gates.hpp
@@ -1,6 +1,7 @@
 #pragma once
 #include <utility>
 #include "quotient_common.hpp"
+#include "light_list.hpp"
 
 namespace lcp2 {
 
@@ -14,8 +15,8 @@
 template <u32 K> struct QGenerated;
 #endif
 
-template <u32 K, bool CHECK>
-__global__ __launch_bounds__(QUOTIENT_THREADS, Q_GENERATED_WAVES[K]) void k_q_gen(QuotientArgs a, u32 g, u32 accumulate, unsigned long long *flag) {
+template <u32 K, bool CHECK, class GUEST>
+__device__ __forceinline__ void q_gen_kernel(const QuotientArgs &a, u32 g, u32 accumulate, unsigned long long *flag, const GUEST &guest) {
 #if defined(__HIP_DEVICE_COMPILE__)
   extern __shared__ __attribute__((aligned(16))) u64 lds[];
   const u32 T = QUOTIENT_THREADS, tid = threadIdx.x;
@@ -27,8 +28,17 @@
   if (!q_wave_holds<CHECK>(a, G, i)) return;
   u64 val[QUOTIENT_MAX_CH];
   q_gate_value<QGenerated<K>>(a, g, G, i, lds, T, tid, val);
+  q_guest_ride(a, guest, i, lds, T, tid, val);
   q_gate_store<CHECK>(a, i, val, accumulate, flag);
 #endif
+}
+template <u32 K, bool CHECK>
+__global__ __launch_bounds__(QUOTIENT_THREADS, Q_GENERATED_WAVES[K]) void k_q_gen(QuotientArgs a, u32 g, u32 accumulate, unsigned long long *flag) {
+  q_gen_kernel<K, CHECK>(a, g, accumulate, flag, QNoGuest{});
+}
+template <u32 K>
+__global__ __launch_bounds__(QUOTIENT_THREADS, Q_GENERATED_WAVES[K]) void k_q_gen_shared(QuotientArgs a, u32 g, u32 accumulate, LightGuest guest) {
+  q_gen_kernel<K, false>(a, g, accumulate, nullptr, guest);
 }
 
 template <class EVAL>
@@ -48,32 +58,39 @@
 }
 
 template <u32 K>
-void launch_generated_one(hipStream_t s, const QuotientArgs &a, u32 g, u32 accumulate, unsigned long long *flag, u32 mode) {
+void launch_generated_one(hipStream_t s, const QuotientArgs &a, u32 g, u32 accumulate, unsigned long long *flag, u32 mode, const LightGuest *guest) {
   if (mode == GEN_CLAIM_CHECK) { launch_claim_check<QGenerated<K>>(s, a, g, flag); return; }
   const dim3 block(QUOTIENT_THREADS);
   const size_t limbs = Q_LIMB_WORDS32 * 4;
   QuotientArgs ag = a;
   ag.limbs_lds_word = 0;
+  if constexpr (Q_GUEST_HOSTS[K]) {
+    if (guest && mode == GEN_QUOTIENT) {
+      ag.limbs_lds_word = (a.num_regs + QUOTIENT_STAGE) * QUOTIENT_THREADS;
+      hipLaunchKernelGGL((k_q_gen_shared<K>), q_grid(a), block, q_interp_lds_bytes(a) + limbs, s, ag, g, accumulate, *guest);
+      return;
+    }
+  }
   if (mode == GEN_ROW_CHECK) hipLaunchKernelGGL((k_q_gen<K, true>), q_grid(a), block, limbs, s, ag, g, accumulate, flag);
   else hipLaunchKernelGGL((k_q_gen<K, false>), q_grid(a), block, limbs, s, ag, g, accumulate, flag);
 }
 
 template <u32 FIRST, size_t... I>
-bool launch_generated_unit(std::index_sequence<I...>, hipStream_t s, const QuotientArgs &a, u32 k, u32 g, u32 accumulate, unsigned long long *flag, u32 mode) {
+bool launch_generated_unit(std::index_sequence<I...>, hipStream_t s, const QuotientArgs &a, u32 k, u32 g, u32 accumulate, unsigned long long *flag, u32 mode, const LightGuest *guest) {
   bool hit = false;
-  ((k == FIRST + I ? (launch_generated_one<FIRST + (u32)I>(s, a, g, accumulate, flag, mode), hit = true) : false), ...);
+  ((k == FIRST + I ? (launch_generated_one<FIRST + (u32)I>(s, a, g, accumulate, flag, mode, guest), hit = true) : false), ...);
   return hit;
 }
 
 #define LCP2_DEFINE_GENERATED_UNIT(name, FIRST, COUNT)                                                                                          \
-  bool launch_generated_##name(hipStream_t s, const QuotientArgs &a, u32 k, u32 g, u32 accumulate, unsigned long long *flag, u32 mode) {       \
-    return launch_generated_unit<FIRST>(std::make_index_sequence<COUNT>{}, s, a, k, g, accumulate, flag, mode);                                 \
+  bool launch_generated_##name(hipStream_t s, const QuotientArgs &a, u32 k, u32 g, u32 accumulate, unsigned long long *flag, u32 mode, const LightGuest *guest) { \
+    return launch_generated_unit<FIRST>(std::make_index_sequence<COUNT>{}, s, a, k, g, accumulate, flag, mode, guest);                          \
   }
 
-bool launch_generated_sha(hipStream_t s, const QuotientArgs &a, u32 k, u32 g, u32 accumulate, unsigned long long *flag, u32 mode);
-bool launch_generated_u32a(hipStream_t s, const QuotientArgs &a, u32 k, u32 g, u32 accumulate, unsigned long long *flag, u32 mode);
-bool launch_generated_u32b(hipStream_t s, const QuotientArgs &a, u32 k, u32 g, u32 accumulate, unsigned long long *flag, u32 mode);
-bool launch_generated_reca(hipStream_t s, const QuotientArgs &a, u32 k, u32 g, u32 accumulate, unsigned long long *flag, u32 mode);
-bool launch_generated_recb(hipStream_t s, const QuotientArgs &a, u32 k, u32 g, u32 accumulate, unsigned long long *flag, u32 mode);
+bool launch_generated_sha(hipStream_t s, const QuotientArgs &a, u32 k, u32 g, u32 accumulate, unsigned long long *flag, u32 mode, const LightGuest *guest);
+bool launch_generated_u32a(hipStream_t s, const QuotientArgs &a, u32 k, u32 g, u32 accumulate, unsigned long long *flag, u32 mode, const LightGuest *guest);
+bool launch_generated_u32b(hipStream_t s, const QuotientArgs &a, u32 k, u32 g, u32 accumulate, unsigned long long *flag, u32 mode, const LightGuest *guest);
+bool launch_generated_reca(hipStream_t s, const QuotientArgs &a, u32 k, u32 g, u32 accumulate, unsigned long long *flag, u32 mode, const LightGuest *guest);
+bool launch_generated_recb(hipStream_t s, const QuotientArgs &a, u32 k, u32 g, u32 accumulate, unsigned long long *flag, u32 mode, const LightGuest *guest);
 
 }
diff --git a/eth-lc-plonky2_amd/csrc/kernels_quotient.hip b/eth-lc-plonky2_amd/csrc/kernels_quotient.hip
--- a/eth-lc-plonky2_amd/csrc/kernels_quotient.hip
+++ b/eth-lc-plonky2_amd/csrc/kernels_quotient.hip
@@ -1,7 +1,7 @@
 #include <algorithm>
 #include "gate_program.hpp"
 #include "kernels_gates.hpp"
-#include "light_gates.hpp"
+#include "light_list.hpp"
 
 namespace lcp2 {
 
@@ -111,20 +111,8 @@
 struct QPoseidon {
   static __device__ __forceinline__ void run(const QuotientArgs &a, const GateDev &, u64 i, u64 *lds, u32 T, u32 tid, QEmit &emit) { q_poseidon_native(a, i, lds, T, tid, emit); }
 };
-struct QArithmetic {
-  static __device__ __forceinline__ void run(const QuotientArgs &a, const GateDev &G, u64 i, u64 *, u32, u32, QEmit &emit) { q_arith_base_walk<true, false>(a, i, G.num_constraints, 0, emit, emit); }
-};
-struct QBaseSum2 {
-  static __device__ __forceinline__ void run(const QuotientArgs &a, const GateDev &G, u64 i, u64 *, u32, u32, QEmit &emit) { q_arith_base_walk<false, true>(a, i, 0, G.num_constraints - 1, emit, emit); }
-};
-__device__ __forceinline__ void q_pair_values(const QuotientArgs &a, u32 gA, u32 gB, const GateDev &GA, const GateDev &GB, u64 i, u64 valA[QUOTIENT_MAX_CH], u64 valB[QUOTIENT_MAX_CH]) {
-  QEmit eA, eB;
-  q_emit_begin(a, GA, eA); q_emit_begin(a, GB, eB);
-  q_arith_base_walk<true, true>(a, i, GA.num_constraints, GB.num_constraints - 1, eA, eB);
-  q_gate_finish(a, gA, GA, i, eA, valA); q_gate_finish(a, gB, GB, i, eB, valB);
-}
 #else
-struct QPoseidon; struct QArithmetic; struct QBaseSum2;
+struct QPoseidon;
 #endif
 struct QArithBasePair;
 template <>
@@ -267,60 +255,29 @@
     if (c < CH) a.out[(u64)c * a.N + ig] = gl_mul(res[c], zhi);
 }
 
-constexpr u32 LIGHT_NO_PAIR = ~0u;
-struct LightGates { u32 count; u32 g[8]; u32 pair_a, pair_b; };
 template <bool CHECK>
 __global__ __launch_bounds__(QUOTIENT_THREADS, 2) void k_q_light(QuotientArgs a, LightGates L, u32 accumulate, unsigned long long *flag) {
 #if defined(__HIP_DEVICE_COMPILE__)
   extern __shared__ __attribute__((aligned(16))) u64 lds[];
-  const u32 T = QUOTIENT_THREADS, tid = threadIdx.x;
   u64 i;
   if (!q_point<CHECK>(a, i)) return;
   u64 sum[QUOTIENT_MAX_CH];
-#pragma unroll
-  for (u32 c = 0; c < QUOTIENT_MAX_CH; c++) sum[c] = 0;
-  const u32 ka = L.pair_a, kb = L.pair_b;
-  const bool pair = ka != LIGHT_NO_PAIR;
-  if (pair) {
-    const GateDev GA = q_load_gate(a, L.g[ka]), GB = q_load_gate(a, L.g[kb]);
-    if (q_wave_holds<CHECK>(a, GA, i) || q_wave_holds<CHECK>(a, GB, i)) {
-      u64 va[QUOTIENT_MAX_CH], vb[QUOTIENT_MAX_CH];
-      q_pair_values(a, L.g[ka], L.g[kb], GA, GB, i, va, vb);
-#pragma unroll
-      for (u32 c = 0; c < QUOTIENT_MAX_CH; c++)
-        if (c < a.num_challenges) sum[c] = gl_add(va[c], vb[c]);
-    }
-  }
-  for (u32 k = 0; k < L.count; k++) {
-    if (pair && (k == ka || k == kb)) continue;
-    const u32 g = L.g[k];
-    const GateDev G = q_load_gate(a, g);
-    if (!q_wave_holds<CHECK>(a, G, i)) continue;
-    u64 val[QUOTIENT_MAX_CH];
-    switch (G.flags & LCP2_GATE_NATIVE_MASK) {
-      case LCP2_GATE_NATIVE_ARITHMETIC: q_gate_value<QArithmetic>(a, g, G, i, lds, T, tid, val); break;
-      case LCP2_GATE_NATIVE_BASE_SUM2: q_gate_value<QBaseSum2>(a, g, G, i, lds, T, tid, val); break;
-      default: q_gate_value<QInterpreted>(a, g, G, i, lds, T, tid, val); break;
-    }
-#pragma unroll
-    for (u32 c = 0; c < QUOTIENT_MAX_CH; c++)
-      if (c < a.num_challenges) sum[c] = gl_add(sum[c], val[c]);
-  }
+  q_light_sum<CHECK>(a, L, i, lds, QUOTIENT_THREADS, threadIdx.x, sum);
   q_gate_store<CHECK>(a, i, sum, accumulate, flag);
 #endif
 }
 
-static bool launch_generated(hipStream_t s, const QuotientArgs &a, u32 k, u32 g, u32 accumulate, unsigned long long *flag, u32 mode) {
-  return launch_generated_sha(s, a, k, g, accumulate, flag, mode) || launch_generated_u32a(s, a, k, g, accumulate, flag, mode) ||
-         launch_generated_u32b(s, a, k, g, accumulate, flag, mode) || launch_generated_reca(s, a, k, g, accumulate, flag, mode) ||
-         launch_generated_recb(s, a, k, g, accumulate, flag, mode);
+static bool launch_generated(hipStream_t s, const QuotientArgs &a, u32 k, u32 g, u32 accumulate, unsigned long long *flag, u32 mode, const LightGuest *guest = nullptr) {
+  return launch_generated_sha(s, a, k, g, accumulate, flag, mode, guest) || launch_generated_u32a(s, a, k, g, accumulate, flag, mode, guest) ||
+         launch_generated_u32b(s, a, k, g, accumulate, flag, mode, guest) || launch_generated_reca(s, a, k, g, accumulate, flag, mode, guest) ||
+         launch_generated_recb(s, a, k, g, accumulate, flag, mode, guest);
 }
 namespace {
 template <bool CHECK>
-void launch_gate(hipStream_t s, const QuotientArgs &a, const GateDev &G, u32 g, u32 accumulate, unsigned long long *flag) {
+void launch_gate(hipStream_t s, const QuotientArgs &a, const GateDev &G, u32 g, u32 accumulate, unsigned long long *flag, const LightGuest *guest = nullptr) {
   const u32 kind = G.flags & LCP2_GATE_NATIVE_MASK;
   if (kind & 0x8000u) {
-    launch_generated(s, a, (kind >> 8) & 0x7Fu, g, accumulate, flag, CHECK ? GEN_ROW_CHECK : GEN_QUOTIENT);
+    launch_generated(s, a, (kind >> 8) & 0x7Fu, g, accumulate, flag, CHECK ? GEN_ROW_CHECK : GEN_QUOTIENT, guest);
     return;
   }
   const size_t stage = (size_t)QUOTIENT_STAGE * QUOTIENT_THREADS * sizeof(u64);
@@ -331,34 +288,95 @@
   return k == 0 || k == LCP2_GATE_NATIVE_ARITHMETIC || k == LCP2_GATE_NATIVE_BASE_SUM2;
 }
 bool pairable(u32 g) { return g < (1u << 16); }
+const LightGates LIGHT_NONE{0, {}, LIGHT_NO_PAIR, LIGHT_NO_PAIR};
+void light_push(LightGates &L, const GateDev &G, u32 g) {
+  const u32 kind = G.flags & LCP2_GATE_NATIVE_MASK;
+  if (kind == LCP2_GATE_NATIVE_ARITHMETIC && L.pair_a == LIGHT_NO_PAIR && pairable(g)) L.pair_a = L.count;
+  if (kind == LCP2_GATE_NATIVE_BASE_SUM2 && L.pair_b == LIGHT_NO_PAIR && pairable(g)) L.pair_b = L.count;
+  L.g[L.count++] = g;
+}
+void light_seal(LightGates &L) {
+  if (L.pair_a == LIGHT_NO_PAIR || L.pair_b == LIGHT_NO_PAIR) L.pair_a = L.pair_b = LIGHT_NO_PAIR;
+}
+struct SharedWalk { const QuotientTiers *t; u64 *planes; };
+bool guest_of(const QuotientArgs &a, const std::vector<GateDev> &host_gates, const SharedWalk &sw, u32 h, LightGuest &guest) {
+  guest = LightGuest{};
+  const QuotientTiers &t = *sw.t;
+  for (size_t b = 0; b < t.light_host.size(); b++) {
+    if (t.light_host[b] != (int)h || guest.lists == Q_GUEST_LISTS) continue;
+    LightGates L = LIGHT_NONE;
+    u32 others = 0;
+    for (u32 g = 0; g < host_gates.size(); g++) {
+      if (host_gates[g].num_constraints == 0 || t.bundle_of[g] != (int)b) continue;
+      if (is_light(host_gates[g])) light_push(L, host_gates[g], g); else others++;
+    }
+    light_seal(L);
+    guest.L[guest.lists] = L;
+    guest.out[guest.lists] = sw.planes + (u64)b * a.num_challenges * a.N;
+    guest.accumulate[guest.lists] = others ? 1u : 0u;
+    guest.lists++;
+  }
+  return guest.lists != 0;
+}
 template <bool CHECK>
-u32 launch_gates(hipStream_t s, const QuotientArgs &a, const std::vector<GateDev> &host_gates, unsigned long long *flag, const int *tier = nullptr, int want = -1) {
+u32 launch_gates(hipStream_t s, const QuotientArgs &a, const std::vector<GateDev> &host_gates, unsigned long long *flag, const int *tier = nullptr, int want = -1,
+                 const SharedWalk *sw = nullptr) {
   u32 launched = 0;
-  const LightGates none{0, {}, LIGHT_NO_PAIR, LIGHT_NO_PAIR};
-  LightGates L = none;
+  LightGates L = LIGHT_NONE;
+  const bool rides = sw && want >= 0 && sw->t->light_host[want] >= 0;
   auto flush = [&] {
-    if (!L.count) return;
-    if (L.pair_a == LIGHT_NO_PAIR || L.pair_b == LIGHT_NO_PAIR) L.pair_a = L.pair_b = LIGHT_NO_PAIR;
+    if (!L.count || rides) return;
+    light_seal(L);
     hipLaunchKernelGGL((k_q_light<CHECK>), q_grid(a), dim3(QUOTIENT_THREADS), q_interp_lds_bytes(a), s, a, L, launched ? 1u : 0u, flag);
     launched++;
-    L = none;
+    L = LIGHT_NONE;
   };
   for (u32 g = 0; g < host_gates.size(); g++) {
     if (host_gates[g].num_constraints == 0 || (tier && tier[g] != want)) continue;
     if (is_light(host_gates[g])) {
-      const u32 kind = host_gates[g].flags & LCP2_GATE_NATIVE_MASK;
-      if (kind == LCP2_GATE_NATIVE_ARITHMETIC && L.pair_a == LIGHT_NO_PAIR && pairable(g)) L.pair_a = L.count;
-      if (kind == LCP2_GATE_NATIVE_BASE_SUM2 && L.pair_b == LIGHT_NO_PAIR && pairable(g)) L.pair_b = L.count;
-      L.g[L.count++] = g;
+      if (rides) continue;
+      light_push(L, host_gates[g], g);
       if (L.count == 8) flush();
       continue;
     }
-    launch_gate<CHECK>(s, a, host_gates[g], g, launched ? 1u : 0u, flag);
+    LightGuest guest;
+    const bool hosts = sw && guest_of(a, host_gates, *sw, g, guest);
+    launch_gate<CHECK>(s, a, host_gates[g], g, launched ? 1u : 0u, flag, hosts ? &guest : nullptr);
     launched++;
   }
   flush();
   return launched;
 }
+}
+
+std::vector<int> plan_shared_walk(const std::vector<GateDev> &gates, const std::vector<int> &bundle_of, u32 num_bundles, u32 num_regs, u32 refused) {
+  std::vector<int> host(num_bundles, -1);
+  std::vector<u32> load(gates.size(), 0);
+  const size_t lds = (size_t)(num_regs + QUOTIENT_STAGE) * QUOTIENT_THREADS * sizeof(u64) + Q_LIMB_WORDS32 * 4;
+  auto program = [&](u32 g) -> int {
+    const u32 kind = gates[g].flags & LCP2_GATE_NATIVE_MASK;
+    if (!(kind & 0x8000u) || gates[g].num_constraints == 0) return -1;
+    const u32 k = (kind >> 8) & 0x7Fu;
+    if (k >= QUOTIENT_GENERATED_GATES || !Q_GUEST_HOSTS[k] || ((refused >> k) & 1)) return -1;
+    const u32 groups = Q_GENERATED_HOST_WAVES[k] * 256 / QUOTIENT_THREADS;
+    if (lds * groups > Q_LDS_BYTES_PER_CU) return -1;
+    return (int)k;
+  };
+  for (u32 b = 0; b < num_bundles; b++) {
+    u32 lights = 0, others = 0;
+    for (u32 g = 0; g < gates.size(); g++)
+      if (bundle_of[g] == (int)b && gates[g].num_constraints) (is_light(gates[g]) ? lights : others)++;
+    if (lights == 0 || lights > 8) continue;
+    int best = -1, best_k = -1;
+    for (u32 g = 0; g < gates.size(); g++) {
+      const int k = bundle_of[g] >= (int)b || (bundle_of[g] >= 0 && others == 0) ? program(g) : -1;
+      if (k < 0 || load[g] == Q_GUEST_LISTS) continue;
+      const bool better = best < 0 || (best_k != 0 && (k == 0 || Q_GENERATED_COST[k] < Q_GENERATED_COST[best_k]));
+      if (better) { best = (int)g; best_k = k; }
+    }
+    if (best >= 0) { host[b] = best; load[best]++; }
+  }
+  return host;
 }
 
 void launch_quotient(hipStream_t s, const QuotientArgs &a, const std::vector<GateDev> &host_gates) {
@@ -372,10 +390,12 @@
   return launch_gates<false>(s, a, host_gates, nullptr, t.bundle_of.data(), -1);
 }
 void launch_quotient_half_tier(hipStream_t s, const QuotientArgs &a, const std::vector<GateDev> &host_gates, const QuotientTiers &t, u64 *planes) {
+  const SharedWalk sw{&t, planes};
+  const bool shared = t.light_host.size() == t.bundles.size();
   for (size_t b = 0; b < t.bundles.size(); b++) {
     QuotientArgs ab = a;
     ab.out = planes + (u64)b * a.num_challenges * a.N;
-    launch_gates<false>(s, ab, host_gates, nullptr, t.bundle_of.data(), (int)b);
+    launch_gates<false>(s, ab, host_gates, nullptr, t.bundle_of.data(), (int)b, shared ? &sw : nullptr);
   }
 }
 
diff --git a/eth-lc-plonky2_amd/csrc/light_list.hpp b/eth-lc-plonky2_amd/csrc/light_list.hpp
--- /dev/null
+++ b/eth-lc-plonky2_amd/csrc/light_list.hpp
@@ -0,0 +1,82 @@
+#pragma once
+#include "quotient_common.hpp"
+#include "light_gates.hpp"
+
+namespace lcp2 {
+
+constexpr u32 LIGHT_NO_PAIR = ~0u;
+struct LightGates { u32 count; u32 g[8]; u32 pair_a, pair_b; };
+
+constexpr u32 Q_GUEST_LISTS = 2;
+struct LightGuest { u32 lists; LightGates L[Q_GUEST_LISTS]; u64 *out[Q_GUEST_LISTS]; u32 accumulate[Q_GUEST_LISTS]; };
+struct QNoGuest {};
+
+#if defined(__HIP_DEVICE_COMPILE__)
+struct QArithmetic {
+  static __device__ __forceinline__ void run(const QuotientArgs &a, const GateDev &G, u64 i, u64 *, u32, u32, QEmit &emit) { q_arith_base_walk<true, false>(a, i, G.num_constraints, 0, emit, emit); }
+};
+struct QBaseSum2 {
+  static __device__ __forceinline__ void run(const QuotientArgs &a, const GateDev &G, u64 i, u64 *, u32, u32, QEmit &emit) { q_arith_base_walk<false, true>(a, i, 0, G.num_constraints - 1, emit, emit); }
+};
+__device__ __forceinline__ void q_pair_values(const QuotientArgs &a, u32 gA, u32 gB, const GateDev &GA, const GateDev &GB, u64 i, u64 valA[QUOTIENT_MAX_CH], u64 valB[QUOTIENT_MAX_CH]) {
+  QEmit eA, eB;
+  q_emit_begin(a, GA, eA); q_emit_begin(a, GB, eB);
+  q_arith_base_walk<true, true>(a, i, GA.num_constraints, GB.num_constraints - 1, eA, eB);
+  q_gate_finish(a, gA, GA, i, eA, valA); q_gate_finish(a, gB, GB, i, eB, valB);
+}
+template <bool CHECK>
+__device__ __forceinline__ void q_light_sum(const QuotientArgs &a, const LightGates &L, u64 i, u64 *lds, u32 T, u32 tid, u64 (&sum)[QUOTIENT_MAX_CH]) {
+#pragma unroll
+  for (u32 c = 0; c < QUOTIENT_MAX_CH; c++) sum[c] = 0;
+  const u32 ka = L.pair_a, kb = L.pair_b;
+  const bool pair = ka != LIGHT_NO_PAIR;
+  if (pair) {
+    const GateDev GA = q_load_gate(a, L.g[ka]), GB = q_load_gate(a, L.g[kb]);
+    if (q_wave_holds<CHECK>(a, GA, i) || q_wave_holds<CHECK>(a, GB, i)) {
+      u64 va[QUOTIENT_MAX_CH], vb[QUOTIENT_MAX_CH];
+      q_pair_values(a, L.g[ka], L.g[kb], GA, GB, i, va, vb);
+#pragma unroll
+      for (u32 c = 0; c < QUOTIENT_MAX_CH; c++)
+        if (c < a.num_challenges) sum[c] = gl_add(va[c], vb[c]);
+    }
+  }
+  for (u32 k = 0; k < L.count; k++) {
+    if (pair && (k == ka || k == kb)) continue;
+    const u32 g = L.g[k];
+    const GateDev G = q_load_gate(a, g);
+    if (!q_wave_holds<CHECK>(a, G, i)) continue;
+    u64 val[QUOTIENT_MAX_CH];
+    switch (G.flags & LCP2_GATE_NATIVE_MASK) {
+      case LCP2_GATE_NATIVE_ARITHMETIC: q_gate_value<QArithmetic>(a, g, G, i, lds, T, tid, val); break;
+      case LCP2_GATE_NATIVE_BASE_SUM2: q_gate_value<QBaseSum2>(a, g, G, i, lds, T, tid, val); break;
+      default: q_gate_value<QInterpreted>(a, g, G, i, lds, T, tid, val); break;
+    }
+#pragma unroll
+    for (u32 c = 0; c < QUOTIENT_MAX_CH; c++)
+      if (c < a.num_challenges) sum[c] = gl_add(sum[c], val[c]);
+  }
+}
+__device__ __forceinline__ void q_guest_ride(const QuotientArgs &, const QNoGuest &, u64, u64 *, u32, u32, u64 (&)[QUOTIENT_MAX_CH]) {}
+__device__ __forceinline__ void q_guest_ride(const QuotientArgs &a, const LightGuest &guest, u64 i, u64 *lds, u32 T, u32 tid, u64 (&val)[QUOTIENT_MAX_CH]) {
+  for (u32 l = 0; l < guest.lists; l++) {
+    u64 sum[QUOTIENT_MAX_CH];
+    q_light_sum<false>(a, guest.L[l], i, lds, T, tid, sum);
+    if (guest.out[l] == a.out) {
+#pragma unroll
+      for (u32 c = 0; c < QUOTIENT_MAX_CH; c++)
+        if (c < a.num_challenges) val[c] = gl_add(val[c], sum[c]);
+    } else {
+      u64 *out = guest.out[l];
+      const u64 ig = a.leaf0 + i;
+      const u32 accumulate = guest.accumulate[l];
+#pragma unroll
+      for (u32 c = 0; c < QUOTIENT_MAX_CH; c++)
+        if (c < a.num_challenges) out[(u64)c * a.N + ig] = accumulate ? gl_add(out[(u64)c * a.N + ig], sum[c]) : sum[c];
+    }
+  }
+}
+#else
+struct QArithmetic; struct QBaseSum2;
+#endif
+
+}
diff --git a/eth-lc-plonky2_amd/csrc/prover_build.hip b/eth-lc-plonky2_amd/csrc/prover_build.hip
--- a/eth-lc-plonky2_amd/csrc/prover_build.hip
+++ b/eth-lc-plonky2_amd/csrc/prover_build.hip
@@ -271,6 +271,12 @@
   {
     const char *sw = getenv("LCP2_QUOTIENT_TIERS");
     if (!c->sharded() && !(sw && sw[0] == '0' && !sw[1])) form_bundles(c.get());
+    {
+      const char *walk = getenv("LCP2_K6_SHARED_WALK");
+      const u32 nb = (u32)c->tiers.bundles.size();
+      if (walk && walk[0] == '0' && !walk[1]) c->tiers.light_host.assign(nb, -1);
+      else c->tiers.light_host = plan_shared_walk(c->dev_gates, c->tiers.bundle_of, nb, c->dev_regs, 0);
+    }
     if (c->tiers.on()) {
       std::vector<u64> masks(c->gates.size(), 0);
       for (const QuotientBundle &B : c->tiers.bundles)
@@ -385,6 +391,35 @@
   *degree = program_degree(code, 0, num_instructions, registers_only.regs);
   return LCP2_OK;
 }
+static void shared_walk_of_gates(const std::vector<int> &light_host, const std::vector<int> &bundle_of, const std::vector<GateDev> &gates, int32_t *hosts) {
+  for (size_t g = 0; g < gates.size(); g++) {
+    const u32 kind = gates[g].flags & LCP2_GATE_NATIVE_MASK;
+    const bool light = kind == 0 || kind == LCP2_GATE_NATIVE_ARITHMETIC || kind == LCP2_GATE_NATIVE_BASE_SUM2;
+    const int b = bundle_of[g];
+    hosts[g] = (light && gates[g].num_constraints && b >= 0 && (size_t)b < light_host.size()) ? light_host[b] : -1;
+  }
+}
+extern "C" int lcp2_shared_walk_plan(const lcp2_gate *gates, uint32_t num_gates, const int32_t *bundles, uint32_t num_regs, uint32_t refused, int32_t *hosts) {
+  if (!gates || !bundles || !hosts || num_regs > 64) return LCP2_E_INVALID;
+  std::vector<GateDev> dev(num_gates);
+  memcpy(dev.data(), gates, (size_t)num_gates * sizeof(lcp2_gate));
+  std::vector<int> bundle_of(bundles, bundles + num_gates);
+  u32 nb = 0;
+  for (int b : bundle_of) {
+    if (b < -1 || b >= (int)num_gates) return LCP2_E_INVALID;
+    nb = std::max(nb, (u32)(b + 1));
+  }
+  shared_walk_of_gates(plan_shared_walk(dev, bundle_of, nb, std::max(num_regs, 1u), refused), bundle_of, dev, hosts);
+  return LCP2_OK;
+}
+extern "C" int lcp2_circuit_shared_walk(const lcp2_circuit *c, uint32_t num_gates, int32_t *hosts) {
+  if (!c || !hosts || num_gates != c->gates.size()) return LCP2_E_INVALID;
+  std::vector<GateDev> dev(num_gates);
+  memcpy(dev.data(), c->gates.data(), (size_t)num_gates * sizeof(lcp2_gate));
+  shared_walk_of_gates(c->tiers.light_host, c->tiers.bundle_of, dev, hosts);
+  return LCP2_OK;
+}
+
 extern "C" int lcp2_circuit_gate_tiers(const lcp2_circuit *c, uint32_t num_gates, uint32_t *degrees, int32_t *bundles) {
   if (!c || num_gates != c->gates.size()) return LCP2_E_INVALID;
   for (uint32_t g = 0; g < num_gates; g++) {
diff --git a/eth-lc-plonky2_amd/csrc/prover_kernels.hpp b/eth-lc-plonky2_amd/csrc/prover_kernels.hpp
--- a/eth-lc-plonky2_amd/csrc/prover_kernels.hpp
+++ b/eth-lc-plonky2_amd/csrc/prover_kernels.hpp
@@ -113,7 +113,13 @@
   std::vector<QuotientBundle> bundles;
   std::vector<int> bundle_of;
   bool on() const { return !bundles.empty(); }
+  std::vector<int> light_host;
 };
+constexpr bool Q_GUEST_HOSTS[QUOTIENT_GENERATED_GATES] = {true, false, false, false, false, false, false, true, true, true, true, false, true, false, false, false, false};
+constexpr u32 Q_GENERATED_COST[QUOTIENT_GENERATED_GATES] = {213, 395, 405, 318, 520, 855, 903, 1015, 924, 390, 74, 384, 473, 140, 156, 462, 228};
+constexpr u32 Q_GENERATED_HOST_WAVES[QUOTIENT_GENERATED_GATES] = {4, 3, 3, 2, 4, 4, 4, 4, 4, 3, 3, 4, 4, 4, 4, 4, 4};
+constexpr u32 Q_LDS_BYTES_PER_CU = 160 * 1024;
+std::vector<int> plan_shared_walk(const std::vector<GateDev> &gates, const std::vector<int> &bundle_of, u32 num_bundles, u32 num_regs, u32 refused);
 u32 launch_quotient_full_tier(hipStream_t s, const QuotientArgs &a, const std::vector<GateDev> &host_gates, const QuotientTiers &t);
 void launch_quotient_half_tier(hipStream_t s, const QuotientArgs &a, const std::vector<GateDev> &host_gates, const QuotientTiers &t, u64 *planes);
 void launch_tier_combine(hipStream_t s, const QuotientArgs &a, const QuotientTiers &t, const u64 *planes, u32 accumulate);
diff --git a/eth-lc-plonky2_amd/csrc/quotient_common.hpp b/eth-lc-plonky2_amd/csrc/quotient_common.hpp
--- a/eth-lc-plonky2_amd/csrc/quotient_common.hpp
+++ b/eth-lc-plonky2_amd/csrc/quotient_common.hpp
@@ -165,6 +165,12 @@
 
 namespace lcp2 {
 static_assert(Q_GENERATED_COUNT == QUOTIENT_GENERATED_GATES, "prover_kernels.hpp and generated_gates.hpp disagree");
+constexpr bool q_host_waves_agree() {
+  for (u32 k = 0; k < Q_GENERATED_COUNT; k++)
+    if (Q_GENERATED_HOST_WAVES[k] != Q_GENERATED_WAVES[k]) return false;
+  return true;
+}
+static_assert(q_host_waves_agree(), "prover_kernels.hpp Q_GENERATED_HOST_WAVES and generated_gates.hpp Q_GENERATED_WAVES disagree");
 #if defined(__HIP_DEVICE_COMPILE__)
 template <u32 K> __device__ __forceinline__ void q_generated(const QuotientArgs &a, u64 i, QEmit &emit);
 #endif
diff --git a/include/lcp2.h b/include/lcp2.h
--- a/include/lcp2.h
+++ b/include/lcp2.h
@@ -335,6 +335,8 @@
 int lcp2_last_challenges(const lcp2_circuit *c, uint64_t out[97]);
 int lcp2_gate_program_degree(const uint32_t *code, size_t num_instructions, uint32_t num_regs, uint32_t *degree);
 int lcp2_circuit_gate_tiers(const lcp2_circuit *c, uint32_t num_gates, uint32_t *degrees, int32_t *bundles);
+int lcp2_shared_walk_plan(const lcp2_gate *gates, uint32_t num_gates, const int32_t *bundles, uint32_t num_regs, uint32_t refused, int32_t *hosts);
+int lcp2_circuit_shared_walk(const lcp2_circuit *c, uint32_t num_gates, int32_t *hosts);
 
 typedef enum {
   LCP2_K_INTT = 0,
```

Result: no change. 9403 (median of 2 runs) (+0.1%).
